# UZ-SLAMLab/DefSLAM

Measured on AMD Instinct MI355X. Metric: SfT GN iters/sec (500-node mesh, 1k matches), higher is better.
Workload: dtype f64

## Files before the change

### defslam_amd/_lib.py

```python
from __future__ import annotations

import ctypes as C
import os

_HERE = os.path.dirname(os.path.abspath(__file__))
LIB_PATH = os.path.join(_HERE, "lib", "libdefslam_hip.so")
LAB_LIB_PATH = os.path.join(_HERE, "lib", "libdefslam_hip_lab.so")

DSH_OK = 0
DSH_TRACE_STRIDE = 8
DSH_MAX_ITERS = 64

c_double_p = C.POINTER(C.c_double)
c_float_p = C.POINTER(C.c_float)
c_i32_p = C.POINTER(C.c_int32)
c_u8_p = C.POINTER(C.c_uint8)


class SftFrameC(C.Structure):
    _fields_ = [
        ("Tcw", c_float_p),
        ("K", C.c_double * 4),
        ("n_frame", C.c_int32),
        ("M", C.c_int32),
        ("obs_nodes", c_i32_p),
        ("obs_bary", c_double_p),
        ("obs_uv", c_double_p),
        ("obs_invsig2", c_double_p),
        ("xyz", c_double_p),
        ("reg_lap", C.c_double),
        ("reg_inex", C.c_double),
        ("reg_temp", C.c_double),
        ("neighbour_layers", C.c_int32),
        ("max_iters", C.c_int32),
    ]


class SftResultC(C.Structure):
    _fields_ = [
        ("Tcw", c_float_p),
        ("pose7", c_double_p),
        ("xyz", c_double_p),
        ("chi2_obs", c_double_p),
        ("outlier", c_u8_p),
        ("mappoint_xyz", c_float_p),
        ("rep_error", C.c_double),
        ("inliers", C.c_int32),
        ("iters", C.c_int32),
        ("trials", C.c_int32),
        ("dim", C.c_int32),
        ("half_bandwidth", C.c_int32),
        ("status", C.c_int32),
        ("trace", c_double_p),
    ]


class SchwarpProblemC(C.Structure):
    pass


class BbsC(C.Structure):
    _fields_ = [("umin", C.c_double), ("umax", C.c_double), ("nptsu", C.c_int32), ("vmin", C.c_double), ("vmax", C.c_double),
                ("nptsv", C.c_int32), ("valdim", C.c_int32)]


SchwarpProblemC._fields_ = [("bbs", BbsC), ("P", C.c_int32), ("kp1", C.c_void_p), ("kp2", C.c_void_p), ("invsig", C.c_void_p), ("fx_slot", C.c_double),
                            ("fy_slot", C.c_double), ("lam", C.c_double), ("fx", C.c_float), ("fy", C.c_float), ("max_iters", C.c_int32), ("x", C.c_void_p),
                            ("diff", C.c_void_p), ("drop", C.c_void_p), ("info", C.c_int32 * 2), ("costs", C.c_double * 2), ("init_lambda", C.c_double), ("init_ok", C.c_int32)]



class SchwarpStoreC(C.Structure):
    _fields_ = [("point_id", C.c_void_p), ("idx2", C.c_void_p), ("tag", C.c_int32)]


class TrackFrameC(C.Structure):
    _fields_ = [("Tcw", c_float_p), ("Ow", C.c_float * 3), ("K", C.c_float * 4), ("bounds", C.c_float * 4), ("grid_cols", C.c_int32),
                ("grid_rows", C.c_int32), ("levels", C.c_int32), ("scale_factors", c_float_p), ("log_scale_factor", C.c_float), ("N", C.c_int32),
                ("kp", c_float_p), ("octave", c_i32_p), ("desc", c_u8_p), ("state", c_u8_p)]


class TrackProblemC(C.Structure):
    _fields_ = [("frame", TrackFrameC), ("mode", C.c_int32), ("th", C.c_float), ("Q", C.c_int32), ("xyz", c_float_p), ("octave", c_i32_p),
                ("normal", c_float_p), ("max_distance", c_float_p), ("desc", c_u8_p), ("skip", c_u8_p), ("match", c_i32_p), ("in_view", c_u8_p),
                ("level", c_i32_p), ("uv", c_float_p), ("view_cos", c_float_p), ("nmatches", C.c_int32), ("rescans", C.c_int32)]


DSH_TRACK_FRAME = 0
DSH_TRACK_LOCAL = 1


class MpKeyFrameC(C.Structure):
    _fields_ = [("Ow", C.c_float * 3), ("N", C.c_int32), ("desc", c_u8_p), ("octave", c_i32_p), ("levels", C.c_int32),
                ("scale_factors", c_float_p), ("bad", C.c_int32)]


DSH_MP_DESCRIPTOR = 1
DSH_MP_NORMAL_DEPTH = 2
DSH_MP_NO_OBS = 1
DSH_MP_NO_GOOD_DESC = 2
DSH_MP_MAX_OBS = 65535


class MpdbDescC(C.Structure):
    _fields_ = [("ctx", C.c_void_p), ("point_capacity", C.c_int32), ("keyframe_capacity", C.c_int32), ("observation_capacity", C.c_int64)]


DSH_MPDB_POSITION = 1
DSH_MPDB_NORMAL_DEPTH = 2
DSH_MPDB_DESCRIPTOR = 4


class TrackCloseCountsC(C.Structure):
    _fields_ = [(n, C.c_int32) for n in ("matches_inliers", "matches_outliers", "to_match_local", "observed", "inliers", "outliers",
                                         "local_map_points", "n_moved")]


DIFFPROP_FIELDS = ["I1u", "I1v", "I2u", "I2v", "J12a", "J12b", "J12c", "J12d", "J21a", "J21b", "J21c", "J21d",
                   "H12uux", "H12uuy", "H12uvx", "H12uvy", "H12vvx", "H12vvy"]


EXPORTED_SYMBOLS = [
    "dsh_create", "dsh_destroy", "dsh_last_error", "dsh_stream", "dsh_synchronize",
    "dsh_template_build", "dsh_template_set", "dsh_template_dims", "dsh_template_get", "dsh_template_embed",
    "dsh_sft_solve", "dsh_sft_batch_upload", "dsh_sft_batch_run", "dsh_sft_batch_download",
    "dsh_sft_batch_counts", "dsh_sft_batch_problem_info",
    "dsh_bbs_eval", "dsh_bbs_coloc", "dsh_normals_estimate", "dsh_schwarp_eval", "dsh_schwarp_fit", "dsh_schwarp_fit_batch",
    "dsh_sfn_estimate", "dsh_bbs_bending", "dsh_warp_initialize", "dsh_search_by_schwarp",
    "dsh_template_embed_device", "dsh_scale_min_median", "dsh_optimize_horn", "dsh_surface_register",
    "dsh_comm_unique_id", "dsh_comm_create", "dsh_comm_destroy", "dsh_sft_shared_solve", "dsh_sft_shared_solve_group", "dsh_sft_connected_solve", "dsh_sft_connected_solve_group",
    "dsh_diffdb_create", "dsh_diffdb_destroy", "dsh_diffdb_clear", "dsh_diffdb_count", "dsh_diffdb_append", "dsh_schwarp_fit_batch_store",
    "dsh_normals_estimate_db", "dsh_sfn_estimate_db",
    "dsh_search_by_projection_batch", "dsh_search_by_projection_frame", "dsh_search_by_projection_local",
    "dsh_kfdb_create", "dsh_kfdb_destroy", "dsh_kfdb_clear", "dsh_kfdb_add", "dsh_kfdb_set_bad", "dsh_kfdb_count", "dsh_mappoint_update",
    "dsh_mpdb_create", "dsh_mpdb_destroy", "dsh_mpdb_clear", "dsh_mpdb_point_count", "dsh_mpdb_keyframe_count", "dsh_mpdb_add_points",
    "dsh_mpdb_update_points", "dsh_mpdb_set_points_bad", "dsh_mpdb_add_observations", "dsh_mpdb_erase_observations", "dsh_mpdb_add_keyframe",
    "dsh_mpdb_set_keyframe_point", "dsh_mpdb_set_keyframe_parent", "dsh_mpdb_set_keyframe_bad",
    "dsh_local_map_update", "dsh_local_map_points", "dsh_local_map_search",
    "dsh_trackstate_set_embedding", "dsh_trackstate_clear_embedding", "dsh_trackstate_set_counters", "dsh_trackstate_get",
    "dsh_trackstate_seed_local_points", "dsh_trackstate_repose", "dsh_trackstate_cull", "dsh_track_close_frame",
]
DSH_COMM_ID_BYTES = 128

LAB_SYMBOLS = ["dsh_lab_set_option", "dsh_lab_sft_run_timed", "dsh_lab_sft_assemble_timed", "dsh_lab_sft_phase_ms", "dsh_lab_sft_step_trace",
               "dsh_lab_sft_system", "dsh_lab_sft_solver_info", "dsh_lab_sft_wave_check", "dsh_lab_sft_dump", "dsh_lab_sft_rounds_timed",
               "dsh_lab_sft_factor_check"]

_lib = None
_lab = None


def load() -> C.CDLL:
    global _lib
    if _lib is None:
        _lib = _bind(LIB_PATH, lab=False)
    return _lib


def load_lab() -> C.CDLL:
    global _lab
    if _lab is None:
        _lab = _bind(LAB_LIB_PATH, lab=True)
    return _lab


def _bind(path: str, lab: bool) -> C.CDLL:
    if not os.path.exists(path):
        raise OSError(f"{path} is missing: run `python -c 'import __graft_entry__ as g; g.build()'` "
                      f"(or `make -C defslam_amd/csrc`). There is no CPU fallback.")
    L = C.CDLL(path)
    vp = C.c_void_p
    L.dsh_create.argtypes = [C.POINTER(vp), C.c_int]
    L.dsh_destroy.argtypes = [vp]
    L.dsh_last_error.argtypes = [vp]
    L.dsh_last_error.restype = C.c_char_p
    L.dsh_stream.argtypes = [vp]
    L.dsh_stream.restype = vp
    L.dsh_synchronize.argtypes = [vp]
    L.dsh_template_build.argtypes = [vp, C.c_int, c_double_p, C.c_int, c_i32_p]
    L.dsh_template_set.argtypes = [vp, C.c_int, c_double_p, c_u8_p, c_i32_p, c_i32_p, c_double_p, c_double_p, C.c_int, c_i32_p,
                                   c_double_p, C.c_double]
    L.dsh_template_dims.argtypes = [vp, c_i32_p, c_i32_p, c_i32_p]
    L.dsh_template_get.argtypes = [vp, c_u8_p, c_i32_p, c_i32_p, c_double_p, c_double_p, c_i32_p, c_double_p, c_double_p]
    L.dsh_template_embed.argtypes = [vp, C.c_int, c_float_p, c_i32_p, c_i32_p, c_float_p]
    L.dsh_sft_solve.argtypes = [vp, C.POINTER(SftFrameC), C.POINTER(SftResultC)]
    L.dsh_sft_batch_upload.argtypes = [vp, C.c_int, C.POINTER(SftFrameC)]
    L.dsh_sft_batch_run.argtypes = [vp]
    L.dsh_sft_batch_download.argtypes = [vp, C.c_int, C.POINTER(SftResultC)]
    L.dsh_sft_batch_counts.argtypes = [vp, C.POINTER(C.c_int64), C.POINTER(C.c_int64)]
    L.dsh_sft_batch_problem_info.argtypes = [vp, C.c_int, C.POINTER(C.c_int64), c_i32_p]
    L.dsh_bbs_eval.argtypes = [vp, C.POINTER(BbsC), c_double_p, c_double_p, c_double_p, C.c_int, C.c_int, C.c_int, c_double_p, c_u8_p]
    L.dsh_bbs_coloc.argtypes = [vp, C.POINTER(BbsC), c_double_p, c_double_p, C.c_int, C.c_int, C.c_int, c_i32_p, c_double_p, c_i32_p]
    L.dsh_normals_estimate.argtypes = [vp, C.c_int, c_i32_p, c_float_p, c_u8_p, c_float_p, c_u8_p, c_float_p, c_u8_p, c_float_p,
                                       c_double_p, c_double_p, c_i32_p, c_float_p, c_float_p, c_u8_p, c_i32_p]
    L.dsh_schwarp_eval.argtypes = [vp, C.POINTER(BbsC), C.c_int, c_float_p, c_float_p, c_float_p, C.c_double, C.c_double, C.c_double, c_double_p,
                                   c_double_p, c_double_p]
    L.dsh_schwarp_fit.argtypes = [vp, C.POINTER(BbsC), C.c_int, c_float_p, c_float_p, c_float_p, C.c_double, C.c_double, C.c_double, C.c_float,
                                  C.c_float, C.c_int, c_double_p, c_float_p, c_u8_p, c_i32_p, c_double_p]
    L.dsh_schwarp_fit_batch.argtypes = [vp, C.c_int, C.POINTER(SchwarpProblemC)]
    L.dsh_diffdb_create.argtypes = [vp, C.c_int64, C.POINTER(vp)]
    L.dsh_diffdb_destroy.argtypes = [vp]
    L.dsh_diffdb_clear.argtypes = [vp]
    L.dsh_diffdb_count.argtypes = [vp]
    L.dsh_diffdb_count.restype = C.c_int64
    L.dsh_diffdb_append.argtypes = [vp, C.c_int, c_float_p, c_i32_p, c_i32_p, c_i32_p]
    L.dsh_schwarp_fit_batch_store.argtypes = [vp, C.c_int, C.POINTER(SchwarpProblemC), C.POINTER(SchwarpStoreC), vp]
    L.dsh_normals_estimate_db.argtypes = [vp, vp, C.c_int, c_i32_p, c_float_p, c_u8_p, c_float_p, c_double_p, c_double_p, c_i32_p, c_float_p, c_i32_p,
                                          C.c_int32, c_i32_p, c_i32_p, c_i32_p, c_i32_p, c_float_p, c_u8_p]
    L.dsh_sfn_estimate.argtypes = [vp, C.POINTER(BbsC), C.c_int, c_double_p, c_double_p, c_float_p, C.c_double, C.c_double, C.c_int, c_double_p, c_double_p,
                                   c_double_p, c_double_p, c_float_p, c_i32_p]
    L.dsh_sfn_estimate_db.argtypes = [vp, C.POINTER(BbsC), vp, C.c_int, c_i32_p, c_double_p, c_double_p, C.c_double, C.c_double, C.c_int, c_double_p, c_double_p,
                                      c_double_p, c_double_p, c_float_p, c_i32_p]
    L.dsh_bbs_bending.argtypes = [C.POINTER(BbsC), C.c_double, c_double_p]
    L.dsh_search_by_schwarp.argtypes = [vp, C.POINTER(BbsC), c_double_p, C.c_int, c_float_p, c_u8_p, c_float_p, c_float_p, C.c_int, C.c_int, C.c_int, c_float_p,
                                        c_u8_p, c_u8_p, C.c_float, C.c_int, c_i32_p, c_i32_p]
    L.dsh_warp_initialize.argtypes = [vp, C.POINTER(BbsC), C.c_int, c_float_p, c_float_p, C.c_double, c_double_p, c_i32_p]
    c_i64_p = C.POINTER(C.c_int64)
    L.dsh_template_embed_device.argtypes = [vp, C.c_int, c_float_p, c_i32_p, c_i32_p, c_float_p]
    L.dsh_scale_min_median.argtypes = [vp, C.c_int, c_float_p, c_float_p, c_double_p, C.c_int64, c_float_p, c_i64_p, c_i32_p]
    L.dsh_optimize_horn.argtypes = [vp, C.c_int, c_float_p, c_float_p, c_double_p, C.c_double, C.c_double, c_i32_p, c_double_p]
    L.dsh_surface_register.argtypes = [vp, C.c_int, c_float_p, c_float_p, c_double_p, C.c_int64, c_float_p, C.c_double, C.c_int, c_i32_p, c_double_p,
                                       c_double_p, c_float_p, c_double_p]
    L.dsh_comm_unique_id.argtypes = [vp]
    L.dsh_comm_create.argtypes = [vp, C.c_int, C.c_int, vp, C.POINTER(vp)]
    L.dsh_comm_destroy.argtypes = [vp]
    L.dsh_sft_shared_solve.argtypes = [vp, vp, C.POINTER(SftFrameC), C.POINTER(SftResultC)]
    L.dsh_sft_shared_solve_group.argtypes = [C.c_int, C.POINTER(vp), C.POINTER(SftFrameC), C.POINTER(SftResultC)]
    L.dsh_sft_connected_solve.argtypes = [vp, vp, C.POINTER(SftFrameC), C.POINTER(SftResultC)]
    L.dsh_sft_connected_solve_group.argtypes = [vp, vp, C.POINTER(SftFrameC), C.POINTER(SftResultC)]
    L.dsh_search_by_projection_batch.argtypes = [vp, C.c_int, C.POINTER(TrackProblemC)]
    L.dsh_search_by_projection_frame.argtypes = [vp, C.POINTER(TrackFrameC), C.c_int, c_float_p, c_i32_p, c_u8_p, C.c_float, c_i32_p, c_i32_p]
    L.dsh_search_by_projection_local.argtypes = [vp, C.POINTER(TrackFrameC), C.c_int, c_float_p, c_float_p, c_float_p, c_u8_p, c_u8_p, C.c_float,
                                                 c_i32_p, c_u8_p, c_i32_p, c_i32_p]
    L.dsh_kfdb_create.argtypes = [vp, C.c_int32, C.POINTER(vp)]
    L.dsh_kfdb_destroy.argtypes = [vp]
    L.dsh_kfdb_clear.argtypes = [vp]
    L.dsh_kfdb_add.argtypes = [vp, C.POINTER(MpKeyFrameC), c_i32_p]
    L.dsh_kfdb_set_bad.argtypes = [vp, C.c_int32, C.c_int32]
    L.dsh_kfdb_count.argtypes = [vp]
    L.dsh_mappoint_update.argtypes = [vp, vp, C.c_int, c_float_p, c_i32_p, c_i32_p, c_i32_p, c_i32_p, C.c_int32, c_u8_p, c_i32_p, c_float_p,
                                      c_float_p, c_float_p, c_i32_p]
    i32 = C.c_int32
    L.dsh_mpdb_create.argtypes = [C.POINTER(MpdbDescC), C.POINTER(vp)]
    L.dsh_mpdb_destroy.argtypes = [vp]
    L.dsh_mpdb_clear.argtypes = [vp]
    L.dsh_mpdb_point_count.argtypes = [vp]
    L.dsh_mpdb_keyframe_count.argtypes = [vp]
    L.dsh_mpdb_add_points.argtypes = [vp, C.c_int, c_float_p, c_float_p, c_float_p, c_u8_p, c_u8_p, c_i32_p]
    L.dsh_mpdb_update_points.argtypes = [vp, C.c_int, c_i32_p, i32, c_float_p, c_float_p, c_float_p, c_u8_p]
    L.dsh_mpdb_set_points_bad.argtypes = [vp, C.c_int, c_i32_p, c_u8_p]
    L.dsh_mpdb_add_observations.argtypes = [vp, C.c_int, c_i32_p, c_i32_p]
    L.dsh_mpdb_erase_observations.argtypes = [vp, C.c_int, c_i32_p, c_i32_p]
    L.dsh_mpdb_add_keyframe.argtypes = [vp, i32, c_i32_p, i32, i32, c_i32_p]
    L.dsh_mpdb_set_keyframe_point.argtypes = [vp, i32, i32, i32]
    L.dsh_mpdb_set_keyframe_parent.argtypes = [vp, i32, i32]
    L.dsh_mpdb_set_keyframe_bad.argtypes = [vp, i32, i32]
    L.dsh_local_map_update.argtypes = [vp, C.c_int, c_i32_p, c_u8_p, i32, c_i32_p, c_i32_p, c_i32_p, c_i32_p, c_i32_p, c_i32_p]
    L.dsh_local_map_points.argtypes = [vp, i32, c_i32_p, c_i32_p]
    L.dsh_local_map_search.argtypes = [vp, C.POINTER(TrackFrameC), C.c_float, i32, c_i32_p, c_i32_p, c_u8_p, c_i32_p, c_float_p, c_float_p, c_i32_p]
    L.dsh_trackstate_set_embedding.argtypes = [vp, C.c_int, c_i32_p, c_i32_p, c_double_p]
    L.dsh_trackstate_clear_embedding.argtypes = [vp]
    L.dsh_trackstate_set_counters.argtypes = [vp, C.c_int, c_i32_p, c_i32_p, c_i32_p]
    L.dsh_trackstate_get.argtypes = [vp, C.c_int, c_i32_p, c_i32_p, c_i32_p, c_i32_p, c_float_p]
    L.dsh_trackstate_seed_local_points.argtypes = [vp, C.c_int, c_i32_p]
    L.dsh_trackstate_repose.argtypes = [vp, C.c_int, c_double_p, c_i32_p]
    L.dsh_trackstate_cull.argtypes = [vp, C.c_int, c_i32_p, c_i32_p, i32, c_u8_p]
    L.dsh_track_close_frame.argtypes = [vp, C.POINTER(TrackFrameC), C.c_int, c_i32_p, c_u8_p, C.c_int, c_double_p, i32, C.POINTER(TrackCloseCountsC)]
    for name in EXPORTED_SYMBOLS:
        fn = getattr(L, name)
        if name not in ("dsh_last_error", "dsh_stream"):
            fn.restype = C.c_int
    if lab:
        L.dsh_lab_set_option.argtypes = [vp, C.c_char_p, C.c_int]
        L.dsh_lab_sft_run_timed.argtypes = [vp, C.c_int, c_double_p]
        L.dsh_lab_sft_assemble_timed.argtypes = [vp, C.c_int, c_double_p]
        L.dsh_lab_sft_phase_ms.argtypes = [vp, C.c_int, c_double_p]
        L.dsh_lab_sft_step_trace.argtypes = [vp, C.c_int, c_double_p]
        L.dsh_lab_sft_system.argtypes = [vp, C.c_int, C.c_int32, c_double_p, c_double_p, c_double_p]
        L.dsh_lab_sft_solver_info.argtypes = [vp, C.c_int, c_i32_p]
        L.dsh_lab_sft_wave_check.argtypes = [vp, C.c_double, C.c_int, C.c_int, c_double_p, c_double_p, c_i32_p, c_double_p]
        L.dsh_lab_sft_dump.argtypes = [vp, C.c_int, C.c_int, C.c_int64, c_double_p]
        L.dsh_lab_sft_rounds_timed.argtypes = [vp, c_double_p, c_i32_p]
        L.dsh_lab_sft_factor_check.argtypes = [vp, c_double_p, c_u8_p, C.c_int, c_double_p, c_i32_p]
        for name in LAB_SYMBOLS:
            getattr(L, name).restype = C.c_int
    return L


class HipEvents:

    def __init__(self):
        self._hip = C.CDLL("libamdhip64.so")
        self._hip.hipEventCreate.argtypes = [C.POINTER(C.c_void_p)]
        self._hip.hipEventRecord.argtypes = [C.c_void_p, C.c_void_p]
        self._hip.hipEventSynchronize.argtypes = [C.c_void_p]
        self._hip.hipEventElapsedTime.argtypes = [C.POINTER(C.c_float), C.c_void_p, C.c_void_p]
        self._hip.hipEventDestroy.argtypes = [C.c_void_p]
        self.e0, self.e1 = C.c_void_p(), C.c_void_p()
        for e in (self.e0, self.e1):
            if self._hip.hipEventCreate(C.byref(e)) != 0:
                raise OSError("hipEventCreate failed")

    def start(self, stream: int):
        if self._hip.hipEventRecord(self.e0, C.c_void_p(stream)) != 0:
            raise OSError("hipEventRecord failed")

    def stop_ms(self, stream: int) -> float:
        ms = C.c_float()
        if (self._hip.hipEventRecord(self.e1, C.c_void_p(stream)) != 0 or self._hip.hipEventSynchronize(self.e1) != 0
                or self._hip.hipEventElapsedTime(C.byref(ms), self.e0, self.e1) != 0):
            raise OSError("HIP event timing failed")
        return float(ms.value)

    def close(self):
        for e in (self.e0, self.e1):
            if e:
                self._hip.hipEventDestroy(e)
        self.e0 = self.e1 = None


HIP_DEVICE_ATTRIBUTE_MULTIPROCESSOR_COUNT = 63


def device_cus(device: int = 0) -> int:
    hip = C.CDLL("libamdhip64.so")
    hip.hipDeviceGetAttribute.argtypes = [C.POINTER(C.c_int), C.c_int, C.c_int]
    n = C.c_int(0)
    if hip.hipDeviceGetAttribute(C.byref(n), HIP_DEVICE_ATTRIBUTE_MULTIPROCESSOR_COUNT, int(device)) != 0 or n.value <= 0:
        raise OSError("hipDeviceGetAttribute(hipDeviceAttributeMultiprocessorCount) failed")
    return int(n.value)
```

### defslam_amd/csrc/dsh_api.cpp

```cpp
#include <hip/hip_runtime.h>

#include <algorithm>
#include <cmath>
#include <cstdio>
#include <cstdlib>
#include <cstring>
#include <dlfcn.h>

#include <memory>
#include <mutex>
#include <string>
#include <vector>

#include "../../include/defslam_hip.h"
#include "dsh_ctx.h"
#include "dsh_template.h"
#include "sft_pack.h"
#include "sft_problem.h"

#include "mapping_launch.h"

#ifdef DSH_LAB
#include "../../include/defslam_hip_debug.h"
#endif

struct LdsMarks { size_t lm[2] = {0, 0}, sc = 0, spec[2] = {0, 0}, cn = 0, b[2] = {0, 0}, tail = 0; };
static LdsMarks g_lds_marks[64];
static std::mutex g_lds_mu;
#define LDS_MARKS(c) (g_lds_marks[(c)->device & 63])
#define LDS_LOCK() std::lock_guard<std::mutex> lds_lock__(g_lds_mu)

namespace {

constexpr int kNB = 32;
constexpr int kTS = 16, kBT = 8, kWB = 16;

using dsh::Tcw_from_pose7;

struct Packed {
  SftDev h{};
  dsh::SftGraph* g = nullptr;
  dsh::SftFramePack f;
};

}

struct dsh_ctx : dsh_ctx_base {
  dsh::TemplateHost tmpl;
  char* d_tmpl = nullptr;
  size_t d_tmpl_bytes = 0;
  struct {
    const double *xyz0, *nbr_w, *nbr_sumw, *k0;
    const int32_t *nbr_ptr, *nbr_idx;
  } dt{};
  std::vector<std::unique_ptr<dsh::SftGraph>> graphs;
  uint64_t upload_serial = 0;
  int B = 0;
  std::vector<Packed> packed;
  char* d_batch = nullptr;
  size_t d_batch_cap = 0;
  SftDev* d_probs = nullptr;
  std::vector<SftDev> h_probs;
  HostBuf stage;
  hipEvent_t stage_free = nullptr;
  bool stage_busy = false;
  HostBuf results;
  size_t ro_bytes = 0;
  size_t res_off = 0, res_bytes = 0;
  struct ResOffs { size_t xyz, chi2, trace, mp, outl; };
  std::vector<ResOffs> res_offs;
  int max_kd = 0;
  size_t jl_doubles = 0;
  size_t xyz_doubles = 0;
  int nw = 8;
  int spec_k = 1;
  int spec_nh = 0;
  char* d_sync = nullptr;
  size_t sync_bytes = 0;
  int spec_hint = 12;
  int max_iters_batch = 0;
  SftSpec* d_spec = nullptr;
  size_t spec_bytes = 0;
  HostBuf spec_done;
  SftSc* d_sc = nullptr;
  int force_waves = 0;
  bool force_split = false;
  bool rounds_mode = false;
  SftRun* d_runs = nullptr;
  int* d_counters = nullptr;
  int* d_linlist = nullptr;
  int rounds_hint = 24;
  static constexpr int kMaxSub = 4;
  hipStream_t sub_stream[kMaxSub] = {nullptr, nullptr, nullptr, nullptr};
  hipEvent_t sub_event[kMaxSub] = {nullptr, nullptr, nullptr, nullptr};
  int n_sub = 1;
  std::vector<hipEvent_t>* phase_events = nullptr;
  std::vector<int> phase_ids;
  int num_cus = 256;
  bool ran = false;
  struct { int waves = 0; int dataflow = 1; int wide_off = 0; int speculate = 0; int split = 2; int rounds = 1; int streams = 0; int helpers = -1; int tail = -1; int owner_waves = 8; int helpers_wbt = 12; } opt;
  bool any_split = false;
};

dsh_ctx_base* dsh_base(dsh_ctx* ctx) { return static_cast<dsh_ctx_base*>(ctx); }

namespace {

void drop_graphs(dsh_ctx* c) {
  if (!c->host_only && c->stream) (void)hipStreamSynchronize(c->stream);
  for (auto& g : c->graphs)
    if (g->d_base) (void)hipFree(g->d_base);
  c->graphs.clear();
  c->packed.clear();
}

int upload_template(dsh_ctx* c) {
  c->B = 0;
  c->ran = false;
  drop_graphs(c);
  if (c->host_only) return DSH_OK;
  const dsh::TemplateHost& t = c->tmpl;
  Arena a;
  const size_t o_xyz0 = a.take(sizeof(double) * 3 * t.n);
  const size_t o_ptr = a.take(sizeof(int32_t) * (t.n + 1));
  const size_t o_idx = a.take(sizeof(int32_t) * t.nbr_idx.size());
  const size_t o_w = a.take(sizeof(double) * t.nbr_w.size());
  const size_t o_sw = a.take(sizeof(double) * t.n);
  const size_t o_k0 = a.take(sizeof(double) * t.n);
  if (c->d_tmpl) { (void)hipFree(c->d_tmpl); c->d_tmpl = nullptr; }
  HIPCHK(c, hipMalloc((void**)&c->d_tmpl, a.size));
  c->d_tmpl_bytes = a.size;
  std::vector<char> st(a.size, 0);
  std::memcpy(&st[o_xyz0], t.xyz0.data(), sizeof(double) * 3 * t.n);
  std::memcpy(&st[o_ptr], t.nbr_ptr.data(), sizeof(int32_t) * (t.n + 1));
  std::memcpy(&st[o_idx], t.nbr_idx.data(), sizeof(int32_t) * t.nbr_idx.size());
  std::memcpy(&st[o_w], t.nbr_w.data(), sizeof(double) * t.nbr_w.size());
  std::memcpy(&st[o_sw], t.nbr_sumw.data(), sizeof(double) * t.n);
  std::memcpy(&st[o_k0], t.k0.data(), sizeof(double) * t.n);
  HIPCHK(c, hipMemcpy(c->d_tmpl, st.data(), a.size, hipMemcpyHostToDevice));
  c->dt.xyz0 = (const double*)(c->d_tmpl + o_xyz0);
  c->dt.nbr_ptr = (const int32_t*)(c->d_tmpl + o_ptr);
  c->dt.nbr_idx = (const int32_t*)(c->d_tmpl + o_idx);
  c->dt.nbr_w = (const double*)(c->d_tmpl + o_w);
  c->dt.nbr_sumw = (const double*)(c->d_tmpl + o_sw);
  c->dt.k0 = (const double*)(c->d_tmpl + o_k0);
  c->B = 0;
  c->ran = false;
  return DSH_OK;
}

template <class T>
size_t reserve(Arena& a, const std::vector<T>& v) { return a.take(sizeof(T) * v.size()); }
template <class T>
void put(char* st, size_t off, const std::vector<T>& v) {
  if (!v.empty()) std::memcpy(st + off, v.data(), sizeof(T) * v.size());
}

int graph_for(dsh_ctx* c, const std::vector<uint8_t>& opt, dsh::SftGraph** out, std::string& err) {
  uint64_t h = 1469598103934665603ull;
  for (uint8_t b : opt) { h ^= b; h *= 1099511628211ull; }
  for (auto& g : c->graphs)
    if (g->opt_hash == h && g->opt == opt) { g->last_use = c->upload_serial; *out = g.get(); return DSH_OK; }
  if (c->graphs.size() >= 64) {
    if (!c->host_only && c->stream) (void)hipStreamSynchronize(c->stream);
    auto& gs = c->graphs;
    for (size_t i = 0; i < gs.size();) {
      if (gs[i]->last_use != c->upload_serial) {
        if (gs[i]->d_base) (void)hipFree(gs[i]->d_base);
        gs.erase(gs.begin() + i);
      } else {
        i++;
      }
    }
  }
  std::unique_ptr<dsh::SftGraph> g(new dsh::SftGraph());
  const int rc = dsh::build_graph(c->tmpl, opt, *g, err);
  if (rc != DSH_OK) return rc;
  g->last_use = c->upload_serial;
  if (!c->host_only) {
    Arena a;
    auto& o = g->o;
    o.act = reserve(a, g->act); o.actnode = reserve(a, g->actnode); o.star_node = reserve(a, g->star_node); o.star_sL = reserve(a, g->star_sL);
    o.str_nodes = reserve(a, g->str_nodes); o.str_L0 = reserve(a, g->str_L0); o.off_ptr = reserve(a, g->off_ptr); o.off_rc = reserve(a, g->off_rc);
    o.sh_ptr = reserve(a, g->sh_ptr); o.sh_rec = reserve(a, g->sh_rec); o.sh_cf = reserve(a, g->sh_cf); o.tmask = reserve(a, g->tmask);
    o.hgather = reserve(a, g->hgather);
    o.hgatherT = reserve(a, g->hgatherT);
    std::vector<char> st(a.size, 0);
    put(st.data(), o.act, g->act); put(st.data(), o.actnode, g->actnode); put(st.data(), o.star_node, g->star_node); put(st.data(), o.star_sL, g->star_sL);
    put(st.data(), o.str_nodes, g->str_nodes); put(st.data(), o.str_L0, g->str_L0); put(st.data(), o.off_ptr, g->off_ptr); put(st.data(), o.off_rc, g->off_rc);
    put(st.data(), o.sh_ptr, g->sh_ptr); put(st.data(), o.sh_rec, g->sh_rec); put(st.data(), o.sh_cf, g->sh_cf); put(st.data(), o.tmask, g->tmask);
    put(st.data(), o.hgather, g->hgather);
    put(st.data(), o.hgatherT, g->hgatherT);
    if (hipMalloc((void**)&g->d_base, a.size) != hipSuccess) { err = "out of device memory (graph)"; return DSH_ERR_HIP; }
    g->d_bytes = a.size;
    if (hipMemcpy(g->d_base, st.data(), a.size, hipMemcpyHostToDevice) != hipSuccess) { (void)hipFree(g->d_base); err = "graph upload failed"; return DSH_ERR_HIP; }
  }
  *out = g.get();
  c->graphs.push_back(std::move(g));
  return DSH_OK;
}

int pack_problem(dsh_ctx* c, const dsh_sft_frame& f, bool wide_off, Packed& P, std::string& err) {
  const dsh::TemplateHost& t = c->tmpl;
  std::vector<uint8_t> viewed, opt;
  int rc = dsh::frame_active_set(t, f, viewed, opt, err);
  if (rc != DSH_OK) return rc;
  rc = graph_for(c, opt, &P.g, err);
  if (rc != DSH_OK) return rc;
  const dsh::SftGraph& g = *P.g;
  rc = dsh::pack_frame(t, g, f, viewed, P.f, err);
  if (rc != DSH_OK) return rc;
  SftDev& h = P.h;
  h = SftDev{};
  h.n = t.n; h.nA = g.nA; h.Dn = 3 * g.nA; h.kd = g.kd; h.ldh = h.kd + 1;
  h.tile_mode = (h.kd <= kTS * kBT) ? 1 : ((h.kd <= kTS * kWB && !wide_off) ? 2 : 0);
  h.wbt = h.tile_mode == 1 ? kBT : (h.tile_mode == 2 ? (h.kd + kTS - 1) / kTS : 0);
  h.tpr = h.tile_mode ? h.wbt + 1 : 0;
  h.M = f.M; h.V = P.f.V; h.S = g.S; h.Es = g.Es; h.noff = g.noff; h.max_iters = f.max_iters; h.mode = 0;
  h.fx = f.K[0]; h.fy = f.K[1]; h.cx = f.K[2]; h.cy = f.K[3];
  h.w_ref = f.reg_temp / std::pow(t.median_L, 2);
  h.w_curv = f.reg_lap / (double)g.nA;
  h.w_str = g.Es > 0 ? f.reg_inex / (double)g.Es : 0.0;
  const float deltaMono = (float)std::sqrt(5.991);
  h.hub_delta = (double)deltaMono;
  h.hub_dsqr = h.hub_delta * h.hub_delta;
  return DSH_OK;
}

int run_rounds_enqueue(dsh_ctx* c);
int run_rounds(dsh_ctx* c) {
  const int rc = run_rounds_enqueue(c);
  if (rc != DSH_OK)
    for (int s = 0; s < c->n_sub; s++) if (c->sub_stream[s]) (void)hipStreamSynchronize(c->sub_stream[s]);
  return rc;
}
int run_rounds_enqueue(dsh_ctx* c) {
  const int B = c->B, S = c->n_sub;
  int b0[dsh_ctx::kMaxSub + 1];
  for (int s = 0; s <= S; s++) b0[s] = (int)((long long)B * s / S);
  int tail_below = -1;
  if (S == 1 && c->opt.tail != 0) {
    if (c->opt.tail > 0) tail_below = c->opt.tail * c->num_cus;
    else tail_below = std::min(4 * c->num_cus, std::max(2 * c->num_cus, (int)((long long)3 * B / 4)));
  }
  auto launch = [&](int s, int phase) {
    const bool ev = c->phase_events && S == 1;
    if (ev) { hipEvent_t e; if (hipEventCreate(&e) == hipSuccess) { (void)hipEventRecord(e, c->stream); c->phase_events->push_back(e); c->phase_ids.push_back(phase); } }
    hipError_t r;
    {
      LDS_LOCK();
      if (phase == SFTB_PH_TAIL) r = sftb_tail_launch(c->d_probs + b0[s], c->d_runs + b0[s], c->d_counters + 16 * s, b0[s + 1] - b0[s], c->max_kd, c->jl_doubles, &LDS_MARKS(c).tail, c->num_cus, tail_below, c->sub_stream[s]);
      else r = sftb_launch(c->d_probs + b0[s], c->d_runs + b0[s], c->d_counters + 16 * s, c->d_linlist + b0[s], b0[s + 1] - b0[s], phase, c->jl_doubles, c->xyz_doubles, LDS_MARKS(c).b,
                           c->num_cus, tail_below, c->sub_stream[s]);
    }
    if (ev) { hipEvent_t e; if (hipEventCreate(&e) == hipSuccess) { (void)hipEventRecord(e, c->stream); c->phase_events->push_back(e); } }
    return r;
  };
  if (S > 1) {
    HIPCHK(c, hipEventRecord(c->sub_event[0], c->stream));
    for (int s = 1; s < S; s++) HIPCHK(c, hipStreamWaitEvent(c->sub_stream[s], c->sub_event[0], 0));
  }
  for (int s = 0; s < S; s++) HIPCHK(c, launch(s, SFTB_PH_INIT));
  const int worst = std::max(1, c->max_iters_batch) * 10 + 1;
  int rounds = 0, group = std::max(1, std::min(worst, c->rounds_hint));
  if (tail_below >= B) group = 0;
  HIPCHK(c, c->spec_done.ensure(64 * dsh_ctx::kMaxSub, true));
  int rc = DSH_OK;
  while (true) {
    for (int i = 0; i < group && rounds < worst; i++, rounds++)
      for (int s = 0; s < S; s++) {
        HIPCHK(c, launch(s, SFTB_PH_LIN));
        HIPCHK(c, launch(s, SFTB_PH_FACTOR));
        HIPCHK(c, launch(s, SFTB_PH_TRIAL));
      }
    if (tail_below >= 0) HIPCHK(c, launch(0, SFTB_PH_TAIL));
    for (int s = 0; s < S; s++) HIPCHK(c, hipMemcpyAsync(c->spec_done.p + 64 * s, c->d_counters + 16 * s, 8 * sizeof(int), hipMemcpyDeviceToHost, c->sub_stream[s]));
    for (int s = 0; s < S; s++) HIPCHK(c, hipStreamSynchronize(c->sub_stream[s]));
    int done = 0;
    for (int s = 0; s < S; s++) done += *reinterpret_cast<const int*>(c->spec_done.p + 64 * s);
    const int* c0 = reinterpret_cast<const int*>(c->spec_done.p);
    if (done >= B) { c->rounds_hint = (tail_below >= 0 && c0[6]) ? std::max(1, c0[7]) : rounds; break; }
    if (rounds >= worst) { rc = dsh_fail(c, DSH_ERR_STATE, "batched rounds: a problem did not terminate within its trial budget"); break; }
    group = 2;
  }
  return rc;
}

int run_once(dsh_ctx* c) {
  if (c->rounds_mode) return run_rounds(c);
  if (c->spec_k <= 1) {
    LDS_LOCK();
    HIPCHK(c, sft_lm_launch(c->d_probs, c->B, c->max_kd, c->jl_doubles, c->nw, LDS_MARKS(c).lm, c->stream));
    return DSH_OK;
  }
  const int K = c->spec_k, B = c->B;
  HIPCHK(c, hipMemsetAsync(c->d_spec, 0, c->spec_bytes, c->stream));
  const int rounds_per_iter = (10 + K - 1) / K;
  const int worst = c->max_iters_batch * rounds_per_iter;
  auto launch = [&](int phase) { LDS_LOCK(); return sft_spec_launch(c->d_probs, c->d_spec, B, K, phase, c->spec_nh, c->opt.owner_waves, c->max_kd, c->jl_doubles, LDS_MARKS(c).spec, c->stream); };
  if (c->spec_nh > 0) HIPCHK(c, hipMemsetAsync(c->d_sync, 0, c->sync_bytes, c->stream));
  HIPCHK(c, launch(SFT_SPEC_INIT));
  int rounds = 0, group = std::max(2, std::min(worst, c->spec_hint));
  HIPCHK(c, c->spec_done.ensure(sizeof(SftSpec) * (size_t)B, true));
  while (true) {
    for (int i = 0; i < group && rounds < worst; i++, rounds++) {
      HIPCHK(c, launch(SFT_SPEC_LIN));
      if (c->any_split) {
        HIPCHK(c, launch(SFT_SPEC_FACTOR));
        HIPCHK(c, launch(SFT_SPEC_SOLVE));
      }
      HIPCHK(c, launch(SFT_SPEC_TRIAL));
    }
    HIPCHK(c, launch(SFT_SPEC_LIN));
    HIPCHK(c, hipMemcpyAsync(c->spec_done.p, c->d_spec, sizeof(SftSpec) * (size_t)B, hipMemcpyDeviceToHost, c->stream));
    HIPCHK(c, hipStreamSynchronize(c->stream));
    const SftSpec* sp = reinterpret_cast<const SftSpec*>(c->spec_done.p);
    bool all_done = true;
    int needed = 0;
    for (int b = 0; b < B; b++) { all_done = all_done && sp[b].done; needed = std::max(needed, sp[b].launches); }
    if (all_done) { c->spec_hint = needed; break; }
    if (rounds >= worst) return dsh_fail(c, DSH_ERR_STATE, "speculative trials: a problem did not terminate within its launch budget");
    group = 2;
  }
  return DSH_OK;
}

}

extern "C" {

int dsh_create(dsh_ctx** out, int device) {
  if (!out) return DSH_ERR_ARG;
  *out = nullptr;
  if (device == -1) {
    dsh_ctx* hc = new dsh_ctx();
    hc->device = -1;
    hc->host_only = true;
    *out = hc;
    return DSH_OK;
  }
  int count = 0;
  if (hipGetDeviceCount(&count) != hipSuccess || count <= 0) return DSH_ERR_NO_DEVICE;
  if (device < 0 || device >= count) return DSH_ERR_ARG;
  dsh_ctx* c = new dsh_ctx();
  c->device = device;
  if (hipSetDevice(device) != hipSuccess || hipStreamCreateWithFlags(&c->stream, hipStreamNonBlocking) != hipSuccess) {
    delete c;
    return DSH_ERR_HIP;
  }
  if (hipEventCreateWithFlags(&c->stage_free, hipEventDisableTiming) != hipSuccess) {
    (void)hipStreamDestroy(c->stream);
    delete c;
    return DSH_ERR_HIP;
  }
  int cus = 0;
  if (hipDeviceGetAttribute(&cus, hipDeviceAttributeMultiprocessorCount, device) == hipSuccess && cus > 0) c->num_cus = cus;
  c->sub_stream[0] = c->stream;
  if (hipEventCreateWithFlags(&c->sub_event[0], hipEventDisableTiming) != hipSuccess) c->sub_event[0] = nullptr;
  *out = c;
  return DSH_OK;
}

int dsh_destroy(dsh_ctx* c) {
  if (!c) return DSH_ERR_ARG;
  dsh_detach_stores(c);
  if (c->host_only) { c->stage.release(); c->results.release(); delete c; return DSH_OK; }
  (void)hipSetDevice(c->device);
  drop_graphs(c);
  for (int i = 1; i < dsh_ctx::kMaxSub; i++) if (c->sub_stream[i]) { (void)hipStreamSynchronize(c->sub_stream[i]); (void)hipStreamDestroy(c->sub_stream[i]); }
  for (int i = 0; i < dsh_ctx::kMaxSub; i++) if (c->sub_event[i]) (void)hipEventDestroy(c->sub_event[i]);
  if (c->stream) { (void)hipStreamSynchronize(c->stream); (void)hipStreamDestroy(c->stream); }
  if (c->stage_free) (void)hipEventDestroy(c->stage_free);
  c->stage.release();
  c->results.release();
  c->spec_done.release();
  if (c->d_tmpl) (void)hipFree(c->d_tmpl);
  c->scratch.release();
  c->pin_in.release();
  c->pin_out.release();
  if (c->d_batch) (void)hipFree(c->d_batch);
  if (c->d_sc) (void)hipFree(c->d_sc);
  delete c;
  return DSH_OK;
}

const char* dsh_last_error(const dsh_ctx* c) { return c ? c->err.c_str() : "null context"; }
void* dsh_stream(dsh_ctx* c) { return c ? (void*)c->stream : nullptr; }
int dsh_synchronize(dsh_ctx* c) {
  if (const int rc = dsh_enter(c, "dsh_synchronize")) return rc;
  HIPCHK(c, hipStreamSynchronize(c->stream));
  return DSH_OK;
}

int dsh_template_build(dsh_ctx* c, int n, const double* xyz0, int F, const int32_t* facets) {
  if (!c || n <= 0 || F <= 0 || !xyz0 || !facets) return dsh_fail(c, DSH_ERR_ARG, "dsh_template_build: bad argument");
  for (int i = 0; i < 3 * F; i++)
    if (facets[i] < 0 || facets[i] >= n) return dsh_fail(c, DSH_ERR_ARG, "dsh_template_build: facet index out of range");
  if (!c->host_only) (void)hipSetDevice(c->device);
  c->tmpl.build(n, xyz0, F, facets);
  return upload_template(c);
}

int dsh_template_set(dsh_ctx* c, int n, const double* xyz0, const uint8_t* boundary, const int32_t* rp, const int32_t* col, const double* w,
                     const double* k0, int E, const int32_t* en, const double* eL, double median_L) {
  if (!c || n <= 0 || E < 0 || !xyz0 || !boundary || !rp || !col || !w || !k0 || !en || !eL) return dsh_fail(c, DSH_ERR_ARG, "dsh_template_set: bad argument");
  if (rp[0] != 0) return dsh_fail(c, DSH_ERR_ARG, "dsh_template_set: nbr_rowptr[0] != 0");
  for (int i = 0; i < n; i++)
    if (rp[i + 1] < rp[i]) return dsh_fail(c, DSH_ERR_ARG, "dsh_template_set: nbr_rowptr is not non-decreasing");
  for (int p = 0; p < rp[n]; p++)
    if (col[p] < 0 || col[p] >= n) return dsh_fail(c, DSH_ERR_ARG, "dsh_template_set: neighbour index out of range");
  for (int e = 0; e < E; e++) {
    if (en[2 * e] < 0 || en[2 * e] >= n || en[2 * e + 1] < 0 || en[2 * e + 1] >= n) return dsh_fail(c, DSH_ERR_ARG, "dsh_template_set: edge node out of range");
    if (!(eL[e] > 0.0)) return dsh_fail(c, DSH_ERR_ARG, "dsh_template_set: edge rest length must be positive");
  }
  if (!(median_L > 0.0)) return dsh_fail(c, DSH_ERR_ARG, "dsh_template_set: median edge length must be positive");
  if (!c->host_only) (void)hipSetDevice(c->device);
  c->tmpl.set(n, xyz0, boundary, rp, col, w, k0, E, en, eL, median_L);
  return upload_template(c);
}

int dsh_template_dims(const dsh_ctx* c, int32_t* n, int32_t* E, int32_t* nnz) {
  if (!c || !c->tmpl.valid) return DSH_ERR_STATE;
  if (n) *n = c->tmpl.n;
  if (E) *E = c->tmpl.E;
  if (nnz) *nnz = (int32_t)c->tmpl.nbr_idx.size();
  return DSH_OK;
}

int dsh_template_get(const dsh_ctx* c, uint8_t* boundary, int32_t* rp, int32_t* col, double* w, double* k0, int32_t* en, double* eL, double* med) {
  if (!c || !c->tmpl.valid) return DSH_ERR_STATE;
  const dsh::TemplateHost& t = c->tmpl;
  if (boundary) std::memcpy(boundary, t.boundary.data(), t.n);
  if (rp) std::memcpy(rp, t.nbr_ptr.data(), sizeof(int32_t) * (t.n + 1));
  if (col) std::memcpy(col, t.nbr_idx.data(), sizeof(int32_t) * t.nbr_idx.size());
  if (w) std::memcpy(w, t.nbr_w.data(), sizeof(double) * t.nbr_w.size());
  if (k0) std::memcpy(k0, t.k0.data(), sizeof(double) * t.n);
  if (en) std::memcpy(en, t.edge_nodes.data(), sizeof(int32_t) * 2 * t.E);
  if (eL) std::memcpy(eL, t.edge_L0.data(), sizeof(double) * t.E);
  if (med) *med = t.median_L;
  return DSH_OK;
}

int dsh_template_embed(const dsh_ctx* c, int P, const float* pts, int32_t* facet_id, int32_t* nodes, float* bary) {
  if (!c || !c->tmpl.valid || c->tmpl.F <= 0) return DSH_ERR_STATE;
  if (P < 0 || !pts || !facet_id || !nodes || !bary) return DSH_ERR_ARG;
  c->tmpl.embed(P, pts, facet_id, nodes, bary);
  return DSH_OK;
}

int dsh_template_embed_device(dsh_ctx* c, int P, const float* pts, int32_t* facet_id, int32_t* nodes, float* bary) {
  if (!c) return DSH_ERR_ARG;
  if (!c->tmpl.valid || c->tmpl.F <= 0) return dsh_fail(c, DSH_ERR_STATE, "dsh_template_embed_device: needs a template built from facets");
  if (P < 0 || (P > 0 && (!pts || !facet_id || !nodes || !bary))) return dsh_fail(c, DSH_ERR_ARG, "dsh_template_embed_device: bad argument");
  if (c->host_only) return dsh_fail(c, DSH_ERR_NO_DEVICE, "dsh_template_embed_device: host-only context, no GPU (dsh_template_embed is the host routine)");
  if (P == 0) return DSH_OK;
  if (const int rc = dsh_enter(c, "dsh_template_embed_device")) return rc;
  const dsh::TemplateHost& t = c->tmpl;
  hipStream_t st = c->stream;
  struct Item { const void* src; size_t bytes; void* dev; };
  Item in[5] = {{pts, 12 * (size_t)P, nullptr}, {t.xyz0.data(), 24 * (size_t)t.n, nullptr}, {t.facets.data(), 12 * (size_t)t.F, nullptr},
                {t.nf_ptr.data(), 4 * (size_t)(t.n + 1), nullptr}, {t.nf_idx.data(), 4 * t.nf_idx.size(), nullptr}};
  for (Item& it : in) {
    if (c->scratch.take(it.bytes, &it.dev) != hipSuccess) return dsh_fail(c, DSH_ERR_HIP, "dsh_template_embed_device: out of device memory");
    if (it.bytes && hipMemcpyAsync(it.dev, it.src, it.bytes, hipMemcpyHostToDevice, st) != hipSuccess)
      return dsh_fail(c, DSH_ERR_HIP, "dsh_template_embed_device: upload failed");
  }
  void *d_fid = nullptr, *d_nodes = nullptr, *d_bary = nullptr;
  if (c->scratch.take(4 * (size_t)P, &d_fid) != hipSuccess || c->scratch.take(12 * (size_t)P, &d_nodes) != hipSuccess ||
      c->scratch.take(12 * (size_t)P, &d_bary) != hipSuccess)
    return dsh_fail(c, DSH_ERR_HIP, "dsh_template_embed_device: out of device memory");
  hipError_t e = reg_embed(P, static_cast<const float*>(in[0].dev), t.n, static_cast<const double*>(in[1].dev), static_cast<const int32_t*>(in[2].dev),
                           static_cast<const int32_t*>(in[3].dev), static_cast<const int32_t*>(in[4].dev), static_cast<int32_t*>(d_fid),
                           static_cast<int32_t*>(d_nodes), static_cast<float*>(d_bary), st);
  if (e == hipSuccess) e = hipMemcpyAsync(facet_id, d_fid, 4 * (size_t)P, hipMemcpyDeviceToHost, st);
  if (e == hipSuccess) e = hipMemcpyAsync(nodes, d_nodes, 12 * (size_t)P, hipMemcpyDeviceToHost, st);
  if (e == hipSuccess) e = hipMemcpyAsync(bary, d_bary, 12 * (size_t)P, hipMemcpyDeviceToHost, st);
  if (e == hipSuccess) e = hipStreamSynchronize(st);
  if (e != hipSuccess) return dsh_fail(c, DSH_ERR_HIP, std::string("dsh_template_embed_device: ") + hipGetErrorString(e));
  return DSH_OK;
}

int dsh_sft_batch_upload(dsh_ctx* c, int B, const dsh_sft_frame* frames) {
  if (!c || B <= 0 || !frames) return dsh_fail(c, DSH_ERR_ARG, "dsh_sft_batch_upload: bad argument");
  if (!c->tmpl.valid) return dsh_fail(c, DSH_ERR_STATE, "dsh_sft_batch_upload: no template");
  if (!c->host_only) (void)hipSetDevice(c->device);
  c->B = 0;
  c->ran = false;
  c->upload_serial++;
  if ((int)c->packed.size() != B) c->packed.resize(B);
  for (int b = 0; b < B; b++) {
    std::string e;
    const int rc = pack_problem(c, frames[b], c->opt.wide_off != 0, c->packed[b], e);
    if (rc != DSH_OK) return dsh_fail(c, rc, "problem " + std::to_string(b) + ": " + e);
  }
  int nw = 8;
  {
    bool all_tiles = true;
    for (int b = 0; b < B; b++) all_tiles = all_tiles && c->packed[b].h.tile_mode == 1;
    if (all_tiles && 2 * B > c->num_cus) nw = 4;
    if ((c->opt.waves == 4 && all_tiles) || c->opt.waves == 8) nw = c->opt.waves;
    if (c->force_waves == 8) nw = 8;
    c->rounds_mode = all_tiles && nw == 4 && c->opt.waves == 0 && c->opt.rounds != 0 && !c->host_only;
    c->n_sub = 1;
    if (c->rounds_mode) {
      const int want = c->opt.streams > 0 ? c->opt.streams : 1;
      while (c->n_sub < want && c->n_sub < dsh_ctx::kMaxSub && B / (c->n_sub + 1) >= 16 * c->num_cus) c->n_sub++;
      if (c->opt.streams > 0) c->n_sub = std::min(std::min(c->opt.streams, (int)dsh_ctx::kMaxSub), std::max(1, B / 64));
      for (int i = 1; i < c->n_sub; i++)
        if (!c->sub_stream[i] && hipStreamCreateWithFlags(&c->sub_stream[i], hipStreamNonBlocking) != hipSuccess) c->sub_stream[i] = nullptr;
      for (int i = 0; i < c->n_sub; i++) if (!c->sub_stream[i] || !c->sub_event[0]) c->n_sub = 1;
    }
  }
  int K = 1;
  if (nw == 8 && !c->force_waves && !c->host_only) {
    K = (4 * B <= c->num_cus) ? 4 : ((3 * B <= c->num_cus) ? 3 : ((2 * B <= c->num_cus) ? 2 : 1));
    {
      bool wide = c->opt.split != 0 && c->opt.helpers != 0;
      for (int b = 0; b < B; b++) {
        const SftDev& hh = c->packed[b].h;
        const int sT = (hh.kd + kTS - 1) / kTS, sp = kTS * sT;
        const int c0 = ((hh.Dn - sp) / 2 / kTS) * kTS, n1 = hh.Dn - sp - c0;
        wide = wide && hh.tile_mode == 2 && sT >= c->opt.helpers_wbt && sT >= 2 && c0 >= 4 * kTS && n1 >= 4 * kTS;
      }
      if (wide && K == 4 && (long long)B * 4 * 2 * 3 > c->num_cus && (long long)B * 2 * 2 * 3 <= c->num_cus) K = 2;
    }
    if (c->opt.speculate >= 1 && c->opt.speculate <= SFT_SPEC_MAXK) K = c->opt.speculate;
    for (int b = 0; b < B; b++) if (c->packed[b].f.max_iters < 1) K = 1;
  }
  size_t jl_doubles = 0, xyz_doubles = 0;
  int max_kd = 0;
  const size_t lds_budget = ((((nw == 4 && !c->rounds_mode) || SFT_WAVES_PER_EU >= 4) ? 75 : 155) * 1024) / 8;
  for (int b = 0; b < B; b++) {
    SftDev& hh = c->packed[b].h;
    if ((c->force_split && hh.tile_mode == 1) ||
        (K > 1 && hh.tile_mode == 1 && c->opt.split >= 2 && 20 * B <= c->num_cus && hh.kd > kTS && hh.Dn >= 8 * kTS * ((hh.kd + kTS - 1) / kTS))) {
      hh.tile_mode = 2;
      hh.wbt = (hh.kd + kTS - 1) / kTS;
      hh.tpr = hh.wbt + 1;
    }
    hh.mode = (hh.mode & ~2) | ((hh.tile_mode == 1 && c->opt.dataflow) ? 2 : 0);
    hh.split = 0;
    if ((c->force_split || (K > 1 && c->opt.split)) && hh.tile_mode == 2) {
      const int sT = hh.wbt, sp = kTS * sT;
      const int c0 = ((hh.Dn - sp) / 2 / kTS) * kTS, n1 = hh.Dn - sp - c0;
      if (sT >= 2 && c0 >= 4 * kTS && n1 >= 4 * kTS) {
        const int n1p = ((n1 + kTS - 1) / kTS) * kTS;
        hh.split = 1; hh.sp_c0 = c0; hh.sp_s = sp; hh.sp_n1p = n1p; hh.sp_pad = n1p - n1;
        SftPart& p0 = hh.part[0]; SftPart& p1 = hh.part[1]; SftPart& p2 = hh.part[2];
        p0 = SftPart{}; p1 = SftPart{}; p2 = SftPart{};
        p0.nS = c0 / kTS; p0.nT = p0.nS + sT; p0.tpr = hh.tpr; p0.wbt = hh.wbt; p0.b_base = 0; p0.b_sign = 1; p0.b_lo = 0; p0.b_hi = c0 + sp;
        p1.nS = n1p / kTS; p1.nT = p1.nS + sT; p1.tpr = hh.tpr; p1.wbt = hh.wbt; p1.b_base = hh.Dn - 1 + hh.sp_pad; p1.b_sign = -1; p1.b_lo = hh.sp_pad; p1.b_hi = n1p;
        p2.nS = sT; p2.nT = sT; p2.wbt = sT - 1; p2.tpr = sT;
        hh.sp_xl = sT * p2.tpr * kTS * kTS + 8 * kTS * sT + 64;
        hh.part[3] = p2;
      }
    }
    size_t used = 0;
    const size_t need1 = ((3 * (size_t)hh.n + 1) & ~(size_t)1) + (((size_t)hh.M + 1) & ~(size_t)1) + 4 * (size_t)hh.S, need2 = need1 + 6 * (size_t)hh.nA + 4 * (size_t)hh.Es;
    const size_t need3 = need2 + 5 * (size_t)hh.M;
    hh.lds_class = (c->rounds_mode && used + need3 <= lds_budget) ? 3 : (used + need2 <= lds_budget) ? 2 : ((used + need1 <= lds_budget) ? 1 : 0);
    used += hh.lds_class == 3 ? need3 : hh.lds_class == 2 ? need2 : (hh.lds_class == 1 ? need1 : 0);
    jl_doubles = std::max(jl_doubles, used);
    if (hh.lds_class >= 1) xyz_doubles = std::max(xyz_doubles, ((3 * (size_t)hh.n + 1) & ~(size_t)1));
    max_kd = std::max(max_kd, hh.tile_mode == 2 ? std::max(hh.kd, kTS * kBT + 1) : hh.kd);
  }
  if (c->host_only) {
    c->h_probs.resize(B);
    for (int b = 0; b < B; b++) c->h_probs[b] = c->packed[b].h;
    c->B = B;
    c->nw = nw;
    return DSH_OK;
  }
  Arena a;
  const size_t o_tab = a.take(sizeof(SftDev) * B * K);
  struct Offs { size_t obs_nodes, obs_bary, obs_uv, obs_w, ob_ptr, ob_m, ob_c, viewed, xyz_init, pose_init; };
  std::vector<Offs> ro(B);
  for (int b = 0; b < B; b++) {
    dsh::SftFramePack& F = c->packed[b].f;
    Offs& o = ro[b];
    o.obs_nodes = reserve(a, F.obs_nodes); o.obs_bary = reserve(a, F.obs_bary); o.obs_uv = reserve(a, F.obs_uv); o.obs_w = reserve(a, F.obs_w);
    o.ob_ptr = reserve(a, F.ob_ptr); o.ob_m = reserve(a, F.ob_m); o.ob_c = reserve(a, F.ob_c); o.viewed = reserve(a, F.viewed);
    o.xyz_init = reserve(a, F.xyz_init);
    o.pose_init = a.take(8 * 8);
  }
  c->ro_bytes = a.size;
  c->res_off = a.size;
  (void)a.take(sizeof(SftResHdr) * (size_t)B);
  c->res_offs.resize(B);
  for (int b = 0; b < B; b++) {
    const SftDev& h = c->packed[b].h;
    dsh_ctx::ResOffs& r = c->res_offs[b];
    r.xyz = a.take(8 * 3 * (size_t)h.n) - c->res_off; r.chi2 = a.take(8 * (size_t)h.M) - c->res_off;
    r.trace = a.take(8 * DSH_TRACE_STRIDE * DSH_MAX_ITERS) - c->res_off;
    r.mp = a.take(4 * 3 * (size_t)h.M) - c->res_off; r.outl = a.take((size_t)h.M) - c->res_off;
  }
  c->res_bytes = a.size - c->res_off;
  struct POffs { size_t Hb, Lb, Lt, LbT, Lbord, Linv, x, xchg, Pf, PfB, sync; };
  struct WOffs { size_t bak, camrec, wtv, Anode, Jstar, Jstr, Hc, Hb, Hbord, Hcn, Lb, Lbord, Lc, Linv, Lt, LbT, x, dbg, sx0, sx1, shadow_xyz, shadow_chi2, shadow_hdr; POffs part[4]; };
  std::vector<WOffs> wo((size_t)B * K);
  const size_t ws_off = a.size;
  const size_t o_spec = a.take(sizeof(SftSpec) * (size_t)B * K);
  const size_t o_runs = a.take(c->rounds_mode ? sizeof(SftRun) * (size_t)B + 64 * dsh_ctx::kMaxSub + sizeof(int) * (size_t)B : 0);
  int nh = 0;
  {
    bool any = false;
    for (int b = 0; b < B; b++) any = any || (c->packed[b].h.split != 0 && c->packed[b].h.wbt >= c->opt.helpers_wbt);
    for (int b = 0; b < B; b++)
      if (c->packed[b].h.split && std::max(c->packed[b].h.part[0].nT, c->packed[b].h.part[1].nT) >= 60000) any = false;
    if (any && K > 1 && !c->force_split) {
      while (nh < 3 && (long long)B * K * 2 * (2 + nh) <= c->num_cus) nh++;
      if (nh == 1) nh = 0;
      if (c->opt.helpers >= 0) nh = c->opt.helpers;
    }
  }
  size_t sync_total = 0;
  if (nh > 0)
    for (int e = 0; e < B * K; e++) {
      const SftDev& h = c->packed[e % B].h;
      if (h.split) for (int g = 0; g < 2; g++) sync_total += Arena::round((size_t)4 * (16 + h.part[g].nT));
    }
  const size_t o_sync = a.take(sync_total);
  size_t sync_used = 0;
  for (int e = 0; e < B * K; e++) {
    const int b = e % B, lane = e / B;
    const SftDev& h = c->packed[b].h;
    const size_t Dnp = (size_t)((h.Dn + kNB - 1) / kNB) * kNB;
    WOffs& w = wo[e];
    w.sx0 = a.take(K > 1 ? 8 * 3 * (size_t)h.n : 0); w.sx1 = a.take(K > 1 ? 8 * 3 * (size_t)h.n : 0);
    w.shadow_xyz = a.take(lane ? 8 * 3 * (size_t)h.n : 0); w.shadow_chi2 = a.take(lane ? 8 * (size_t)h.M : 0); w.shadow_hdr = a.take(lane ? sizeof(SftResHdr) : 0);
    w.bak = a.take(8 * 3 * (size_t)h.n);
    w.camrec = a.take(8 * (size_t)h.M * SFT_CAM_STRIDE);
    w.wtv = a.take(h.lds_class >= 1 ? 0 : 8 * ((size_t)h.M + 1)); w.Jstar = a.take(h.lds_class >= 1 ? 0 : 8 * 4 * (size_t)h.S);
    w.Anode = a.take(h.lds_class >= 2 ? 0 : 8 * 6 * (size_t)h.nA); w.Jstr = a.take(h.lds_class >= 2 ? 0 : 8 * 4 * (size_t)h.Es);
    const size_t band_elems = h.tile_mode ? (Dnp / kTS + SFT_H_PAD_TILE_ROWS) * (size_t)h.tpr * kTS * kTS : Dnp * (size_t)h.ldh;
    const size_t bord_elems = (SFT_BORDER + 1) * Dnp + SFT_H_PAD_BORDER;
    w.Hc = a.take(h.tile_mode == 1 ? 8 * c->packed[b].g->hc_elems() : 0);
    w.Hb = a.take(h.tile_mode == 1 ? 0 : 8 * band_elems); w.Hbord = a.take(8 * bord_elems); w.Hcn = a.take(8 * 56);
    w.Lb = a.take(8 * band_elems); w.Lbord = a.take(8 * bord_elems); w.Lc = a.take(8 * 56);
    w.Linv = a.take(8 * (Dnp / kTS) * (size_t)kTS * kTS);
    w.Lt = a.take(h.tile_mode == 2 ? 8 * band_elems : 0); w.LbT = a.take(h.tile_mode == 2 ? 8 * (Dnp / kTS) * (size_t)kTS * kTS : 0);
    w.x = a.take(8 * (Dnp + 8)); w.dbg = a.take(1024);
    if (h.split)
      for (int g = 0; g < 4; g++) {
        const SftPart& q = h.part[g];
        const size_t tiles = 8 * (size_t)q.nT * q.tpr * kTS * kTS, col = 8 * (size_t)q.nT * kTS * kTS;
        POffs& po = w.part[g];
        po.Hb = a.take(g < 2 && lane == 0 ? tiles : 0);
        po.Lb = a.take(tiles); po.Lt = a.take(tiles); po.LbT = a.take(col); po.Linv = a.take(col);
        po.Lbord = a.take(8 * 8 * (size_t)kTS * q.nT); po.x = a.take(8 * ((size_t)kTS * q.nT + 8)); po.xchg = a.take(8 * (size_t)h.sp_xl);
        const bool helped = nh > 0 && g < 2;
        po.Pf = a.take(helped ? tiles : 0); po.PfB = a.take(helped ? col : 0);
        po.sync = o_sync + sync_used;
        if (helped) sync_used += Arena::round((size_t)4 * (16 + q.nT));
      }
  }
  if (sft_lm_kernel_lds_bytes(max_kd, jl_doubles) > 160 * 1024 || max_kd + kNB + SFT_BORDER > SFT_NT)
    return dsh_fail(c, DSH_ERR_ARG, "half-bandwidth too large for the LDS panel / workgroup");
  bool fresh_arena = false;
  if (a.size > c->d_batch_cap) {
    HIPCHK(c, hipStreamSynchronize(c->stream));
    if (c->d_batch) { (void)hipFree(c->d_batch); c->d_batch = nullptr; c->d_batch_cap = 0; }
    HIPCHK(c, hipMalloc((void**)&c->d_batch, a.size));
    c->d_batch_cap = a.size;
    fresh_arena = true;
  }
  if (c->stage_busy) { HIPCHK(c, hipEventSynchronize(c->stage_free)); c->stage_busy = false; }
  HIPCHK(c, c->stage.ensure(c->ro_bytes, true));
  char* st = c->stage.p;
  char* base = c->d_batch;
  c->h_probs.resize((size_t)B * K);
  SftResHdr* d_hdr = (SftResHdr*)(base + c->res_off);
  int max_iters = 0;
  for (int e = 0; e < B * K; e++) {
    const int b = e % B, lane = e / B;
    Packed& P = c->packed[b];
    const dsh::SftFramePack& F = P.f;
    const dsh::SftGraph& g = *P.g;
    const Offs& o = ro[b];
    if (lane == 0) {
      put(st, o.obs_nodes, F.obs_nodes); put(st, o.obs_bary, F.obs_bary); put(st, o.obs_uv, F.obs_uv); put(st, o.obs_w, F.obs_w);
      put(st, o.ob_ptr, F.ob_ptr); put(st, o.ob_m, F.ob_m); put(st, o.ob_c, F.ob_c); put(st, o.viewed, F.viewed); put(st, o.xyz_init, F.xyz_init);
      std::memcpy(st + o.pose_init, F.pose_init, 7 * sizeof(double));
    }
    SftDev h = P.h;
    const WOffs& w = wo[e];
    const dsh_ctx::ResOffs& r = c->res_offs[b];
    max_iters = std::max(max_iters, F.max_iters);
    char* rbase = base + c->res_off;
    const char* gb = g.d_base;
    h.xyz0 = c->dt.xyz0; h.nbr_ptr = c->dt.nbr_ptr; h.nbr_idx = c->dt.nbr_idx; h.nbr_w = c->dt.nbr_w; h.nbr_sumw = c->dt.nbr_sumw; h.k0 = c->dt.k0;
    h.act = (const int32_t*)(gb + g.o.act); h.actnode = (const int32_t*)(gb + g.o.actnode); h.star_node = (const int32_t*)(gb + g.o.star_node);
    h.star_sL = (const double*)(gb + g.o.star_sL); h.str_nodes = (const int32_t*)(gb + g.o.str_nodes); h.str_L0 = (const double*)(gb + g.o.str_L0);
    h.off_ptr = (const int32_t*)(gb + g.o.off_ptr); h.off_rc = (const int32_t*)(gb + g.o.off_rc); h.sh_ptr = (const int32_t*)(gb + g.o.sh_ptr);
    h.sh_rec = (const uint32_t*)(gb + g.o.sh_rec); h.sh_cf = (const double*)(gb + g.o.sh_cf); h.tmask = (const int32_t*)(gb + g.o.tmask);
    h.hgather = (const uint32_t*)(gb + g.o.hgather);
    h.hgatherT = (const uint32_t*)(gb + g.o.hgatherT);
    h.obs_nodes = (const int32_t*)(base + o.obs_nodes); h.obs_bary = (const double*)(base + o.obs_bary);
    h.obs_uv = (const double*)(base + o.obs_uv); h.obs_w = (const double*)(base + o.obs_w);
    h.ob_ptr = (const int32_t*)(base + o.ob_ptr); h.ob_m = (const int32_t*)(base + o.ob_m); h.ob_c = (const double*)(base + o.ob_c);
    h.viewed = (const uint8_t*)(base + o.viewed);
    h.xyz_init = (const double*)(base + o.xyz_init); h.pose_init = (const double*)(base + o.pose_init);
    h.res = d_hdr + b; h.pose = d_hdr[b].pose;
    h.xyz = (double*)(rbase + r.xyz); h.chi2_obs = (double*)(rbase + r.chi2); h.trace = (double*)(rbase + r.trace);
    h.mappoint = (float*)(rbase + r.mp); h.outlier = (uint8_t*)(rbase + r.outl);
    h.xyz_bak = (double*)(base + w.bak);
    h.camrec = (double*)(base + w.camrec); h.wtv = (double*)(base + w.wtv); h.Anode = (double*)(base + w.Anode);
    h.Jstar = (double*)(base + w.Jstar); h.Jstr = (double*)(base + w.Jstr);
    h.Hc = (double*)(base + w.Hc); h.Hb = (double*)(base + w.Hb); h.Hbord = (double*)(base + w.Hbord); h.Hcorner = (double*)(base + w.Hcn);
    h.Lb = (double*)(base + w.Lb); h.Lbord = (double*)(base + w.Lbord); h.Lcorner = (double*)(base + w.Lc); h.Linv = (double*)(base + w.Linv);
    h.Lt = (double*)(base + w.Lt); h.LbT = (double*)(base + w.LbT);
    h.x = (double*)(base + w.x); h.dbg = (double*)(base + w.dbg);
    h.spec_xyz[0] = (double*)(base + w.sx0); h.spec_xyz[1] = (double*)(base + w.sx1);
    if (h.split)
      for (int g = 0; g < 4; g++) {
        const POffs& po = w.part[g];
        SftPart& q = h.part[g];
        q.Hb = g < 2 ? (double*)(base + (lane ? wo[b].part[g].Hb : po.Hb)) : (double*)(base + po.xchg);
        q.Lb = (double*)(base + po.Lb); q.Lt = (double*)(base + po.Lt); q.LbT = (double*)(base + po.LbT); q.Linv = (double*)(base + po.Linv);
        q.Lbord = (double*)(base + po.Lbord); q.x = (double*)(base + po.x); q.xchg = (double*)(base + po.xchg);
        const bool helped = nh > 0 && g < 2;
        q.Pf = helped ? (double*)(base + po.Pf) : nullptr; q.PfB = helped ? (double*)(base + po.PfB) : nullptr;
        q.sync = helped ? (int32_t*)(base + po.sync) : nullptr;
      }
    if (lane) {
      h.xyz = (double*)(base + w.shadow_xyz); h.chi2_obs = (double*)(base + w.shadow_chi2);
      h.res = (SftResHdr*)(base + w.shadow_hdr); h.pose = ((SftResHdr*)(base + w.shadow_hdr))->pose;
      h.trace = nullptr; h.mappoint = nullptr; h.outlier = nullptr;
      if (h.tile_mode == 1 || h.split) {
        const SftDev& h0 = c->h_probs[b];
        h.Hc = h0.Hc; h.Hbord = h0.Hbord; h.Hcorner = h0.Hcorner;
      }
    }
    c->h_probs[e] = h;
  }
  std::memcpy(st + o_tab, c->h_probs.data(), sizeof(SftDev) * B * K);
  HIPCHK(c, hipMemcpyAsync(base, st, c->ro_bytes, hipMemcpyHostToDevice, c->stream));
  HIPCHK(c, hipEventRecord(c->stage_free, c->stream));
  c->stage_busy = true;
  if (fresh_arena) HIPCHK(c, hipMemsetAsync(base + ws_off, 0, a.size - ws_off, c->stream));
  HIPCHK(c, hipMemsetAsync(base + c->res_off, 0, c->res_bytes, c->stream));
  c->d_probs = (SftDev*)(base + o_tab);
  c->d_spec = (SftSpec*)(base + o_spec);
  c->d_runs = (SftRun*)(base + o_runs);
  c->d_counters = (int*)(base + o_runs + sizeof(SftRun) * (size_t)B);
  c->d_linlist = c->d_counters + 16 * dsh_ctx::kMaxSub;
  c->spec_bytes = sizeof(SftSpec) * (size_t)B * K;
  c->spec_k = K;
  c->spec_nh = nh;
  c->d_sync = base + o_sync;
  c->sync_bytes = sync_total;
  c->any_split = false;
  for (int b = 0; b < B; b++) c->any_split = c->any_split || c->packed[b].h.split != 0;
  c->max_iters_batch = max_iters;
  c->B = B;
  c->max_kd = max_kd;
  c->jl_doubles = jl_doubles;
  c->xyz_doubles = xyz_doubles;
  c->nw = nw;
  return DSH_OK;
}

int dsh_sft_batch_run(dsh_ctx* c) {
  if (!c) return DSH_ERR_ARG;
  if (const int rc = dsh_enter(c, "dsh_sft_batch_run")) return rc;
  if (c->B <= 0) return dsh_fail(c, DSH_ERR_STATE, "dsh_sft_batch_run: nothing uploaded");
  const int rc = run_once(c);
  if (rc != DSH_OK) return rc;
  c->ran = true;
  return DSH_OK;
}

int dsh_sft_batch_counts(dsh_ctx* c, int64_t* iters, int64_t* trials) {
  if (!c || c->B <= 0 || !c->ran) return DSH_ERR_STATE;
  if (const int rc = dsh_enter(c, "dsh_sft_batch_counts")) return rc;
  const size_t bytes = sizeof(SftResHdr) * (size_t)c->B;
  HIPCHK(c, c->results.ensure(std::max(bytes, c->results.cap), true));
  HIPCHK(c, hipMemcpyAsync(c->results.p, c->d_batch + c->res_off, bytes, hipMemcpyDeviceToHost, c->stream));
  HIPCHK(c, hipStreamSynchronize(c->stream));
  const SftResHdr* hd = reinterpret_cast<const SftResHdr*>(c->results.p);
  int64_t it = 0, tr = 0;
  for (int b = 0; b < c->B; b++) { it += hd[b].iters; tr += hd[b].trials; }
  if (iters) *iters = it;
  if (trials) *trials = tr;
  return DSH_OK;
}

int dsh_sft_batch_problem_info(dsh_ctx* c, int b, int64_t* bytes, int32_t* counts) {
  if (!c || b < 0 || b >= c->B) return DSH_ERR_ARG;
  const Packed& P = c->packed[b];
  const SftDev& h = P.h;
  const int64_t M = h.M, n = h.n, C = P.g->n_curv_ref, E = h.Es, V = h.V;
  const int64_t reads = 60 * M + 24 * n + 88 + 92 * C + 16 * E + 28 * V;
  const int64_t writes = 8 * (30 * M + 21 * C + 6 * E + 9 * V) + 8 * (2 * M + C + E + 3 * V) + 8 * M;
  if (bytes) *bytes = reads + writes;
  if (counts) { counts[0] = h.M; counts[1] = h.nA; counts[2] = P.g->n_curv_ref; counts[3] = h.Es; counts[4] = h.V; counts[5] = 6 + h.Dn; counts[6] = h.kd; counts[7] = c->rounds_mode ? 1 : c->nw; counts[8] = P.g->noff; }
  return DSH_OK;
}

int dsh_sft_batch_download(dsh_ctx* c, int B, dsh_sft_result* res) {
  if (!c || !res || B != c->B) return dsh_fail(c, DSH_ERR_ARG, "dsh_sft_batch_download: bad argument");
  if (const int rc = dsh_enter(c, "dsh_sft_batch_download")) return rc;
  if (!c->ran) return dsh_fail(c, DSH_ERR_STATE, "dsh_sft_batch_download: no run");
  HIPCHK(c, c->results.ensure(c->res_bytes, true));
  HIPCHK(c, hipMemcpyAsync(c->results.p, c->d_batch + c->res_off, c->res_bytes, hipMemcpyDeviceToHost, c->stream));
  HIPCHK(c, hipStreamSynchronize(c->stream));
  const char* rb = c->results.p;
  const SftResHdr* hd = reinterpret_cast<const SftResHdr*>(rb);
  for (int b = 0; b < B; b++) {
    const SftDev& h = c->h_probs[b];
    const Packed& P = c->packed[b];
    const dsh_ctx::ResOffs& o = c->res_offs[b];
    dsh_sft_result& r = res[b];
    r.rep_error = hd[b].rep_error;
    r.inliers = hd[b].inliers;
    r.iters = hd[b].iters;
    r.trials = hd[b].trials;
    r.status = hd[b].status;
    r.dim = 6 + h.Dn;
    r.half_bandwidth = h.kd;
    if (r.chi2_obs) std::memcpy(r.chi2_obs, rb + o.chi2, 8 * (size_t)h.M);
    if (r.outlier) std::memcpy(r.outlier, rb + o.outl, (size_t)h.M);
    if (r.xyz) std::memcpy(r.xyz, rb + o.xyz, 8 * 3 * (size_t)h.n);
    if (r.pose7) std::memcpy(r.pose7, hd[b].pose, 8 * 7);
    if (r.Tcw) Tcw_from_pose7(hd[b].pose, r.Tcw);
    if (r.mappoint_xyz) std::memcpy(r.mappoint_xyz, rb + o.mp, 4 * 3 * (size_t)h.M);
    if (r.trace) {
      const size_t rows = (size_t)std::max(P.f.max_iters, 0), done = std::min(rows, (size_t)std::max(hd[b].iters, 0));
      std::memcpy(r.trace, rb + o.trace, 8 * DSH_TRACE_STRIDE * done);
      std::memset(r.trace + DSH_TRACE_STRIDE * done, 0, 8 * DSH_TRACE_STRIDE * (rows - done));
    }
  }
  return DSH_OK;
}

int dsh_sft_solve(dsh_ctx* c, const dsh_sft_frame* frame, dsh_sft_result* result) {
  if (!c || !frame || !result) return dsh_fail(c, DSH_ERR_ARG, "dsh_sft_solve: bad argument");
  int rc = dsh_sft_batch_upload(c, 1, frame);
  if (rc != DSH_OK) return rc;
  rc = dsh_sft_batch_run(c);
  if (rc != DSH_OK) return rc;
  return dsh_sft_batch_download(c, 1, result);
}

namespace {
struct RcclUniqueId { char internal[128]; };
struct Rccl {
  void* lib = nullptr;
  int (*GetUniqueId)(RcclUniqueId*) = nullptr;
  int (*CommInitRank)(void**, int, RcclUniqueId, int) = nullptr;
  int (*AllReduce)(const void*, void*, size_t, int, int, void*, hipStream_t) = nullptr;
  int (*CommDestroy)(void*) = nullptr;
  const char* (*GetErrorString)(int) = nullptr;
  bool load(std::string& err) {
    if (lib) return true;
    for (const char* name : {"librccl.so.1", "librccl.so", "/opt/rocm/lib/librccl.so.1"}) {
      lib = dlopen(name, RTLD_NOW | RTLD_GLOBAL);
      if (lib) break;
    }
    if (!lib) { err = std::string("RCCL not found: ") + dlerror(); return false; }
    GetUniqueId = reinterpret_cast<decltype(GetUniqueId)>(dlsym(lib, "ncclGetUniqueId"));
    CommInitRank = reinterpret_cast<decltype(CommInitRank)>(dlsym(lib, "ncclCommInitRank"));
    AllReduce = reinterpret_cast<decltype(AllReduce)>(dlsym(lib, "ncclAllReduce"));
    CommDestroy = reinterpret_cast<decltype(CommDestroy)>(dlsym(lib, "ncclCommDestroy"));
    GetErrorString = reinterpret_cast<decltype(GetErrorString)>(dlsym(lib, "ncclGetErrorString"));
    if (!GetUniqueId || !CommInitRank || !AllReduce || !CommDestroy) { err = "RCCL symbols missing"; lib = nullptr; return false; }
    return true;
  }
};
Rccl g_rccl;
constexpr int kNcclDouble = 8, kNcclSum = 0;
}

struct dsh_comm {
  int nranks = 1, rank = 0;
  void* comm = nullptr;
  dsh_ctx* ctx = nullptr;
};

namespace {

struct ScRank { dsh_ctx* c; };

struct ScReducer {
  dsh_comm* comm = nullptr;
  SftSc** d_ptrs = nullptr;
  int reduce(std::vector<ScRank>& R, std::string& err) {
    if (comm) {
      dsh_ctx* c = R[0].c;
      const int rc = g_rccl.AllReduce(c->d_sc->send, c->d_sc->recv, SFT_SC_XCHG, kNcclDouble, kNcclSum, comm->comm, c->stream);
      if (rc != 0) { err = std::string("ncclAllReduce: ") + (g_rccl.GetErrorString ? g_rccl.GetErrorString(rc) : "error"); return DSH_ERR_HIP; }
      return DSH_OK;
    }
    for (auto& r : R)
      if (hipStreamSynchronize(r.c->stream) != hipSuccess) { err = "stream synchronise failed"; return DSH_ERR_HIP; }
    if (sft_sc_local_reduce(d_ptrs, (int)R.size(), R[0].c->stream) != hipSuccess || hipStreamSynchronize(R[0].c->stream) != hipSuccess) { err = "local reduce failed"; return DSH_ERR_HIP; }
    return DSH_OK;
  }
};

int sc_phase(std::vector<ScRank>& R, int phase, std::string& err) {
  for (auto& r : R) {
    dsh_ctx* c = r.c;
    (void)hipSetDevice(c->device);
    LDS_LOCK();
    if (sft_sc_launch(c->d_probs, c->d_sc, 1, phase, c->max_kd, c->jl_doubles, &LDS_MARKS(c).sc, c->stream) != hipSuccess) { err = "phase kernel launch failed"; return DSH_ERR_HIP; }
  }
  return DSH_OK;
}

int sc_solve(std::vector<ScRank>& R, ScReducer& red, int rank0, int nranks, const dsh_sft_frame* frames, dsh_sft_result* results, std::string& err) {
  const int G = (int)R.size();
  if (nranks > SFT_SC_XCHG - 13) { err = "too many ranks for the exchange vector"; return DSH_ERR_ARG; }
  int local_rc = DSH_OK;
  std::string local_err;
  for (int g = 0; g < G; g++) {
    dsh_ctx* c = R[g].c;
    if (c->host_only) { err = "host-only context, no GPU (there is no CPU fallback)"; return DSH_ERR_NO_DEVICE; }
    (void)hipSetDevice(c->device);
    if (!c->d_sc && hipMalloc((void**)&c->d_sc, sizeof(SftSc)) != hipSuccess) { err = "out of device memory"; return DSH_ERR_HIP; }
    SftSc init{};
    init.rank = rank0 + g;
    init.nranks = nranks;
    int rc = frames[g].max_iters < 1 ? DSH_ERR_ARG : DSH_OK;
    if (rc != DSH_OK && local_rc == DSH_OK) { local_rc = rc; local_err = "max_iters must be >= 1"; }
    if (rc == DSH_OK) {
      c->force_waves = 8;
      rc = dsh_sft_batch_upload(c, 1, &frames[g]);
      c->force_waves = 0;
      if (rc != DSH_OK && local_rc == DSH_OK) { local_rc = rc; local_err = c->err; }
    }
    if (rc == DSH_OK && c->packed[0].h.tile_mode != 1) {
      rc = DSH_ERR_ARG;
      if (local_rc == DSH_OK) { local_rc = rc; local_err = "the shared-camera mode needs a template with half-bandwidth <= 128 (register-window solver); dsh_sft_connected_solve takes wider ones"; }
    }
    if (rc == DSH_OK) {
      init.send[0] = (double)c->packed[0].h.nA;
      init.send[1] = (double)c->packed[0].h.Es;
    }
    init.send[2] = rc == DSH_OK ? 0.0 : 1.0;
    if (hipMemcpyAsync(c->d_sc, &init, sizeof(SftSc), hipMemcpyHostToDevice, c->stream) != hipSuccess) { err = "state upload failed"; return DSH_ERR_HIP; }
  }
  int rc = red.reduce(R, err);
  if (rc != DSH_OK) return rc;
  {
    double tot3[3];
    dsh_ctx* c = R[0].c;
    if (hipMemcpyAsync(tot3, c->d_sc->recv, sizeof(tot3), hipMemcpyDeviceToHost, c->stream) != hipSuccess || hipStreamSynchronize(c->stream) != hipSuccess) { err = "read-back failed"; return DSH_ERR_HIP; }
    if (tot3[2] != 0.0) {
      if (local_rc != DSH_OK) { err = local_err; return local_rc; }
      err = "another rank failed to set its patch up";
      return DSH_ERR_STATE;
    }
  }
  for (int g = 0; g < G; g++) {
    dsh_ctx* c = R[g].c;
    double tot[2];
    if (hipMemcpyAsync(tot, c->d_sc->recv, sizeof(tot), hipMemcpyDeviceToHost, c->stream) != hipSuccess || hipStreamSynchronize(c->stream) != hipSuccess) { err = "read-back failed"; return DSH_ERR_HIP; }
    SftDev& h = c->h_probs[0];
    h.w_curv = frames[g].reg_lap / tot[0];
    h.w_str = tot[1] > 0 ? frames[g].reg_inex / tot[1] : 0.0;
    if (hipMemcpyAsync(c->d_probs, &h, sizeof(SftDev), hipMemcpyHostToDevice, c->stream) != hipSuccess || hipStreamSynchronize(c->stream) != hipSuccess) { err = "problem record upload failed"; return DSH_ERR_HIP; }
  }
  for (int guard = 0; guard < DSH_MAX_ITERS + 1; guard++) {
    if ((rc = sc_phase(R, SFT_SC_LIN, err)) != DSH_OK || (rc = red.reduce(R, err)) != DSH_OK) return rc;
    int again = 0, done = 0;
    do {
      if ((rc = sc_phase(R, SFT_SC_FAC, err)) != DSH_OK || (rc = red.reduce(R, err)) != DSH_OK) return rc;
      if ((rc = sc_phase(R, SFT_SC_SOL, err)) != DSH_OK || (rc = red.reduce(R, err)) != DSH_OK) return rc;
      if ((rc = sc_phase(R, SFT_SC_CTL, err)) != DSH_OK) return rc;
      int32_t flags[2];
      dsh_ctx* c = R[0].c;
      if (hipMemcpyAsync(flags, &c->d_sc->again, sizeof(flags), hipMemcpyDeviceToHost, c->stream) != hipSuccess || hipStreamSynchronize(c->stream) != hipSuccess) { err = "flag read-back failed"; return DSH_ERR_HIP; }
      again = flags[0];
      done = flags[1];
    } while (again);
    if (done) break;
  }
  for (int g = 0; g < G; g++) {
    R[g].c->ran = true;
    rc = dsh_sft_batch_download(R[g].c, 1, &results[g]);
    if (rc != DSH_OK) { err = R[g].c->err; return rc; }
  }
  return DSH_OK;
}

}

int dsh_comm_unique_id(void* id) {
  std::string err;
  if (!id || !g_rccl.load(err)) return DSH_ERR_HIP;
  return g_rccl.GetUniqueId(static_cast<RcclUniqueId*>(id)) == 0 ? DSH_OK : DSH_ERR_HIP;
}

int dsh_comm_create(dsh_ctx* c, int nranks, int rank, const void* id, dsh_comm** out) {
  if (!c || !out || !id || nranks < 1 || rank < 0 || rank >= nranks) return dsh_fail(c, DSH_ERR_ARG, "dsh_comm_create: bad argument");
  *out = nullptr;
  if (const int rc = dsh_enter(c, "dsh_comm_create")) return rc;
  std::string err;
  if (!g_rccl.load(err)) return dsh_fail(c, DSH_ERR_HIP, "dsh_comm_create: " + err);
  RcclUniqueId uid;
  std::memcpy(&uid, id, sizeof(uid));
  std::unique_ptr<dsh_comm> cm(new dsh_comm());
  cm->nranks = nranks; cm->rank = rank; cm->ctx = c;
  const int rc = g_rccl.CommInitRank(&cm->comm, nranks, uid, rank);
  if (rc != 0) return dsh_fail(c, DSH_ERR_HIP, std::string("ncclCommInitRank: ") + (g_rccl.GetErrorString ? g_rccl.GetErrorString(rc) : "error"));
  *out = cm.release();
  return DSH_OK;
}

int dsh_comm_destroy(dsh_comm* cm) {
  if (!cm) return DSH_ERR_ARG;
  if (cm->comm && g_rccl.CommDestroy) (void)g_rccl.CommDestroy(cm->comm);
  delete cm;
  return DSH_OK;
}

int dsh_sft_shared_solve(dsh_ctx* c, dsh_comm* cm, const dsh_sft_frame* frame, dsh_sft_result* result) {
  if (!c || !cm || !frame || !result || cm->ctx != c) return dsh_fail(c, DSH_ERR_ARG, "dsh_sft_shared_solve: bad argument");
  std::vector<ScRank> R{ScRank{c}};
  ScReducer red;
  red.comm = cm;
  std::string err;
  const int rc = sc_solve(R, red, cm->rank, cm->nranks, frame, result, err);
  return rc == DSH_OK ? rc : dsh_fail(c, rc, "dsh_sft_shared_solve: " + err);
}

int dsh_sft_shared_solve_group(int G, dsh_ctx* const* ctxs, const dsh_sft_frame* frames, dsh_sft_result* results) {
  if (G < 1 || !ctxs || !frames || !results) return DSH_ERR_ARG;
  for (int g = 0; g < G; g++)
    if (!ctxs[g]) return DSH_ERR_ARG;
  dsh_ctx* c0 = ctxs[0];
  std::vector<ScRank> R;
  for (int g = 0; g < G; g++) R.push_back(ScRank{ctxs[g]});
  for (int g = 0; g < G; g++) {
    if (ctxs[g]->host_only) return dsh_fail(c0, DSH_ERR_NO_DEVICE, "dsh_sft_shared_solve_group: host-only context, no GPU (there is no CPU fallback)");
    (void)hipSetDevice(ctxs[g]->device);
    if (!ctxs[g]->d_sc && hipMalloc((void**)&ctxs[g]->d_sc, sizeof(SftSc)) != hipSuccess) return dsh_fail(c0, DSH_ERR_HIP, "dsh_sft_shared_solve_group: out of device memory");
  }
  std::vector<SftSc*> ptrs;
  for (int g = 0; g < G; g++) ptrs.push_back(ctxs[g]->d_sc);
  ScReducer red;
  (void)hipSetDevice(c0->device);
  if (hipMalloc((void**)&red.d_ptrs, sizeof(SftSc*) * G) != hipSuccess) return dsh_fail(c0, DSH_ERR_HIP, "dsh_sft_shared_solve_group: out of device memory");
  int rc = DSH_OK;
  std::string err;
  if (hipMemcpy(red.d_ptrs, ptrs.data(), sizeof(SftSc*) * G, hipMemcpyHostToDevice) != hipSuccess) { rc = DSH_ERR_HIP; err = "pointer table upload failed"; }
  if (rc == DSH_OK) rc = sc_solve(R, red, 0, G, frames, results, err);
  (void)hipFree(red.d_ptrs);
  return rc == DSH_OK ? rc : dsh_fail(c0, rc, "dsh_sft_shared_solve_group: " + err);
}


namespace {

int cn_allreduce(std::vector<ScRank>& R, dsh_comm* comm, double* const* send, double* const* recv, int n, std::string& err) {
  if (comm) {
    dsh_ctx* c = R[0].c;
    const int rc = g_rccl.AllReduce(send[0], recv[0], (size_t)n, kNcclDouble, kNcclSum, comm->comm, c->stream);
    if (rc != 0) { err = std::string("ncclAllReduce: ") + (g_rccl.GetErrorString ? g_rccl.GetErrorString(rc) : "error"); return DSH_ERR_HIP; }
    return DSH_OK;
  }
  for (auto& r : R)
    if (hipStreamSynchronize(r.c->stream) != hipSuccess) { err = "stream synchronise failed"; return DSH_ERR_HIP; }
  if (sft_vec_sum2(send[0], send[1], recv[0], recv[1], n, R[0].c->stream) != hipSuccess || hipStreamSynchronize(R[0].c->stream) != hipSuccess) { err = "local reduce failed"; return DSH_ERR_HIP; }
  return DSH_OK;
}

int cn_phase(std::vector<ScRank>& R, int phase, std::string& err) {
  for (auto& r : R) {
    dsh_ctx* c = r.c;
    (void)hipSetDevice(c->device);
    LDS_LOCK();
    if (sft_cn_launch(c->d_probs, c->d_sc, phase, c->max_kd, c->jl_doubles, &LDS_MARKS(c).cn, c->stream) != hipSuccess) { err = "phase kernel launch failed"; return DSH_ERR_HIP; }
  }
  return DSH_OK;
}

int cn_solve(std::vector<ScRank>& R, dsh_comm* comm, int rank0, const dsh_sft_frame* frame, dsh_sft_result* results, std::string& err) {
  const int G = (int)R.size();
  int local_rc = DSH_OK;
  std::string local_err;
  for (int g = 0; g < G; g++) {
    dsh_ctx* c = R[g].c;
    if (c->host_only) { err = "host-only context, no GPU (there is no CPU fallback)"; return DSH_ERR_NO_DEVICE; }
    (void)hipSetDevice(c->device);
    if (!c->d_sc && hipMalloc((void**)&c->d_sc, sizeof(SftSc)) != hipSuccess) { err = "out of device memory"; return DSH_ERR_HIP; }
    int rc = frame->max_iters < 1 ? DSH_ERR_ARG : DSH_OK;
    if (rc != DSH_OK && local_rc == DSH_OK) { local_rc = rc; local_err = "max_iters must be >= 1"; }
    if (rc == DSH_OK) {
      c->force_waves = 8;
      c->force_split = true;
      rc = dsh_sft_batch_upload(c, 1, frame);
      c->force_waves = 0;
      c->force_split = false;
      if (rc != DSH_OK && local_rc == DSH_OK) { local_rc = rc; local_err = c->err; }
    }
    if (rc == DSH_OK && !c->packed[0].h.split) {
      rc = DSH_ERR_ARG;
      if (local_rc == DSH_OK) { local_rc = rc; local_err = "the connected-mesh mode needs a band of at most 256 that is long enough to cut (two parts of four tile columns next to a separator of one bandwidth)"; }
    }
    SftSc init{};
    init.rank = rank0 + g;
    init.nranks = 2;
    init.send[0] = rc == DSH_OK ? 0.0 : 1.0;
    if (hipMemcpyAsync(c->d_sc, &init, sizeof(SftSc), hipMemcpyHostToDevice, c->stream) != hipSuccess) { err = "state upload failed"; return DSH_ERR_HIP; }
  }
  {
    double* snd[2]; double* rcv[2];
    for (int g = 0; g < G; g++) { snd[g] = R[g].c->d_sc->send; rcv[g] = R[g].c->d_sc->recv; }
    int rc = cn_allreduce(R, comm, snd, rcv, 4, err);
    if (rc != DSH_OK) return rc;
    double bad = 0.0;
    dsh_ctx* c = R[0].c;
    if (hipMemcpyAsync(&bad, c->d_sc->recv, sizeof(bad), hipMemcpyDeviceToHost, c->stream) != hipSuccess || hipStreamSynchronize(c->stream) != hipSuccess) { err = "read-back failed"; return DSH_ERR_HIP; }
    if (bad != 0.0) {
      if (local_rc != DSH_OK) { err = local_err; return local_rc; }
      err = "the other rank failed to set the problem up";
      return DSH_ERR_STATE;
    }
  }
  int rc;
  double* xs[2]; double* xr[2]; double* vx[2];
  int xl = 0, nx = 0;
  for (int g = 0; g < G; g++) {
    const SftDev& h = R[g].c->h_probs[0];
    xs[g] = h.part[rank0 + g].xchg; xr[g] = h.part[2].xchg; vx[g] = h.x;
    xl = h.sp_xl;
    nx = ((h.Dn + kNB - 1) / kNB) * kNB + 6;
  }
  for (int guard = 0; guard < DSH_MAX_ITERS + 1; guard++) {
    if ((rc = cn_phase(R, SFT_CN_LIN, err)) != DSH_OK) return rc;
    int again = 0, done = 0;
    do {
      if ((rc = cn_phase(R, SFT_CN_FAC, err)) != DSH_OK || (rc = cn_allreduce(R, comm, xs, xr, xl, err)) != DSH_OK) return rc;
      if ((rc = cn_phase(R, SFT_CN_SOL, err)) != DSH_OK || (rc = cn_allreduce(R, comm, vx, vx, nx, err)) != DSH_OK) return rc;
      if ((rc = cn_phase(R, SFT_CN_CTL, err)) != DSH_OK) return rc;
      int32_t flags[2];
      dsh_ctx* c = R[0].c;
      if (hipMemcpyAsync(flags, &c->d_sc->again, sizeof(flags), hipMemcpyDeviceToHost, c->stream) != hipSuccess || hipStreamSynchronize(c->stream) != hipSuccess) { err = "flag read-back failed"; return DSH_ERR_HIP; }
      again = flags[0];
      done = flags[1];
    } while (again);
    if (done) break;
  }
  for (int g = 0; g < G; g++) {
    R[g].c->ran = true;
    rc = dsh_sft_batch_download(R[g].c, 1, &results[g]);
    if (rc != DSH_OK) { err = R[g].c->err; return rc; }
  }
  return DSH_OK;
}

}

int dsh_sft_connected_solve(dsh_ctx* c, dsh_comm* cm, const dsh_sft_frame* frame, dsh_sft_result* result) {
  if (!c || !cm || !frame || !result || cm->ctx != c) return dsh_fail(c, DSH_ERR_ARG, "dsh_sft_connected_solve: bad argument");
  if (cm->nranks != 2) return dsh_fail(c, DSH_ERR_ARG, "dsh_sft_connected_solve: the cut has two parts: the communicator must have exactly two ranks");
  std::vector<ScRank> R{ScRank{c}};
  std::string err;
  const int rc = cn_solve(R, cm, cm->rank, frame, result, err);
  return rc == DSH_OK ? rc : dsh_fail(c, rc, "dsh_sft_connected_solve: " + err);
}

int dsh_sft_connected_solve_group(dsh_ctx* c0, dsh_ctx* c1, const dsh_sft_frame* frame, dsh_sft_result* results) {
  if (!c0 || !c1 || c0 == c1 || !frame || !results) return DSH_ERR_ARG;
  std::vector<ScRank> R{ScRank{c0}, ScRank{c1}};
  std::string err;
  const int rc = cn_solve(R, nullptr, 0, frame, results, err);
  return rc == DSH_OK ? rc : dsh_fail(c0, rc, "dsh_sft_connected_solve_group: " + err);
}

#ifdef DSH_LAB
namespace {
struct EventPair {
  hipEvent_t e0 = nullptr, e1 = nullptr;
  hipError_t create() { hipError_t e = hipEventCreate(&e0); return e != hipSuccess ? e : hipEventCreate(&e1); }
  ~EventPair() { if (e0) (void)hipEventDestroy(e0); if (e1) (void)hipEventDestroy(e1); }
};
}

int dsh_lab_set_option(dsh_ctx* c, const char* name, int value) {
  if (!c || !name) return DSH_ERR_ARG;
  const std::string k(name);
  if (k == "waves") { if (value != 0 && value != 4 && value != 8) return dsh_fail(c, DSH_ERR_ARG, "dsh_lab_set_option: waves is 0 (automatic), 4 or 8"); c->opt.waves = value; }
  else if (k == "dataflow") c->opt.dataflow = value != 0;
  else if (k == "wide_off") c->opt.wide_off = value != 0;
  else if (k == "rounds") c->opt.rounds = value != 0;
  else if (k == "streams") { if (value < 0 || value > dsh_ctx::kMaxSub) return dsh_fail(c, DSH_ERR_ARG, "dsh_lab_set_option: streams is 0 (automatic) or 1..4 sub-batches"); c->opt.streams = value; }
  else if (k == "split") { if (value < 0 || value > 2) return dsh_fail(c, DSH_ERR_ARG, "dsh_lab_set_option: split is 0 (off), 1 (wide bands only) or 2 (every band long enough)"); c->opt.split = value; }
  else if (k == "helpers_wbt") { if (value < 1 || value > 16) return dsh_fail(c, DSH_ERR_ARG, "dsh_lab_set_option: helpers_wbt is 1..16 (tiles of half-bandwidth from which parts get helper workgroups)"); c->opt.helpers_wbt = value; }
  else if (k == "owner_waves") { if (value != 8 && value != 16) return dsh_fail(c, DSH_ERR_ARG, "dsh_lab_set_option: owner_waves is 8 or 16 (wavefronts of a FACTOR workgroup with helpers)"); c->opt.owner_waves = value; }
  else if (k == "helpers") { if (value < -1 || value > 3) return dsh_fail(c, DSH_ERR_ARG, "dsh_lab_set_option: helpers is -1 (automatic) or 0..3 workgroups per part"); c->opt.helpers = value; }
  else if (k == "tail") { if (value < -1 || value > 8) return dsh_fail(c, DSH_ERR_ARG, "dsh_lab_set_option: tail is -1 (automatic), 0 (rounds to the end) or the number of problems per CU from which downwards the last problems go to the tail kernel"); c->opt.tail = value; }
  else if (k == "speculate") { if (value < 0 || value > SFT_SPEC_MAXK) return dsh_fail(c, DSH_ERR_ARG, "dsh_lab_set_option: speculate is 0 (automatic) or 1..4 lanes"); c->opt.speculate = value; }
  else return dsh_fail(c, DSH_ERR_ARG, "dsh_lab_set_option: unknown option " + k);
  return DSH_OK;
}

int dsh_lab_sft_solver_info(dsh_ctx* c, int b, int32_t* out8) {
  if (!c || !out8 || b < 0 || b >= c->B) return dsh_fail(c, DSH_ERR_ARG, "dsh_lab_sft_solver_info: bad argument");
  const SftDev& h = c->h_probs[b];
  out8[0] = h.split; out8[1] = h.sp_c0; out8[2] = h.sp_s; out8[3] = h.sp_n1p; out8[4] = h.sp_pad; out8[5] = c->spec_k; out8[6] = h.tile_mode; out8[7] = c->nw;
  return DSH_OK;
}

int dsh_lab_sft_run_timed(dsh_ctx* c, int launches, double* total_ms) {
  if (!c || launches <= 0 || !total_ms) return dsh_fail(c, DSH_ERR_ARG, "dsh_lab_sft_run_timed: bad argument");
  if (const int rc = dsh_enter(c, "dsh_lab_sft_run_timed")) return rc;
  if (c->B <= 0) return dsh_fail(c, DSH_ERR_STATE, "dsh_lab_sft_run_timed: nothing uploaded");
  EventPair ev;
  HIPCHK(c, ev.create());
  HIPCHK(c, hipEventRecord(ev.e0, c->stream));
  for (int i = 0; i < launches; i++) { const int rc = run_once(c); if (rc != DSH_OK) return rc; }
  HIPCHK(c, hipEventRecord(ev.e1, c->stream));
  HIPCHK(c, hipEventSynchronize(ev.e1));
  float ms = 0.f;
  HIPCHK(c, hipEventElapsedTime(&ms, ev.e0, ev.e1));
  *total_ms = (double)ms;
  c->ran = true;
  return DSH_OK;
}

int dsh_lab_sft_assemble_timed(dsh_ctx* c, int launches, double* total_ms) {
  if (!c || launches <= 0 || !total_ms) return dsh_fail(c, DSH_ERR_ARG, "dsh_lab_sft_assemble_timed: bad argument");
  if (const int rc = dsh_enter(c, "dsh_lab_sft_assemble_timed")) return rc;
  if (c->B <= 0 || !c->ran) return dsh_fail(c, DSH_ERR_STATE, "dsh_lab_sft_assemble_timed: needs an uploaded batch that has run once");
  EventPair ev;
  HIPCHK(c, ev.create());
  HIPCHK(c, hipEventRecord(ev.e0, c->stream));
  for (int i = 0; i < launches; i++) HIPCHK(c, sft_assembly_launch(c->d_probs, c->B, c->max_kd, c->jl_doubles, c->rounds_mode ? 8 : c->nw, c->stream));
  HIPCHK(c, hipEventRecord(ev.e1, c->stream));
  HIPCHK(c, hipEventSynchronize(ev.e1));
  float ms = 0.f;
  HIPCHK(c, hipEventElapsedTime(&ms, ev.e0, ev.e1));
  *total_ms = ms;
  c->ran = false;
  return DSH_OK;
}

int dsh_lab_sft_wave_check(dsh_ctx* c, double rel, int launches, int only, double* x_ref, double* x_new, int32_t* ok2, double* ms2) {
  if (!c || launches <= 0 || !ms2) return dsh_fail(c, DSH_ERR_ARG, "dsh_lab_sft_wave_check: bad argument");
  if (const int rc = dsh_enter(c, "dsh_lab_sft_wave_check")) return rc;
  if (c->B <= 0 || !c->ran) return dsh_fail(c, DSH_ERR_STATE, "dsh_lab_sft_wave_check: needs an uploaded batch that has run once");
  for (int b = 0; b < c->B; b++)
    if (c->h_probs[b].tile_mode != 1) return dsh_fail(c, DSH_ERR_STATE, "dsh_lab_sft_wave_check: register-window problems (half-bandwidth <= 128) only");
  HIPCHK(c, sft_assembly_launch(c->d_probs, c->B, c->max_kd, c->jl_doubles, c->rounds_mode ? 8 : c->nw, c->stream));
  EventPair ev;
  HIPCHK(c, ev.create());
  for (int which = 0; which < 2; which++) {
    if (only == 2 - which) continue;
    HIPCHK(c, sft_wave_lab_launch(c->d_probs, c->B, which, rel, c->max_kd, c->jl_doubles, c->stream));
    HIPCHK(c, hipEventRecord(ev.e0, c->stream));
    for (int i = 0; i < launches; i++) HIPCHK(c, sft_wave_lab_launch(c->d_probs, c->B, which, rel, c->max_kd, c->jl_doubles, c->stream));
    HIPCHK(c, hipEventRecord(ev.e1, c->stream));
    HIPCHK(c, hipEventSynchronize(ev.e1));
    float ms = 0.f;
    HIPCHK(c, hipEventElapsedTime(&ms, ev.e0, ev.e1));
    ms2[which] = (double)ms / launches;
    double* dst = which == 0 ? x_ref : x_new;
    size_t off = 0;
    for (int b = 0; b < c->B; b++) {
      const SftDev& h = c->h_probs[b];
      const size_t Dnp = (size_t)((h.Dn + kNB - 1) / kNB) * kNB;
      if (dst) HIPCHK(c, hipMemcpy(dst + off, h.x, 8 * (Dnp + 6), hipMemcpyDeviceToHost));
      off += Dnp + 6;
      double flag = 0.0;
      if (ok2) { HIPCHK(c, hipMemcpy(&flag, h.dbg + 2, 8, hipMemcpyDeviceToHost)); ok2[2 * b + which] = (int32_t)flag; }
    }
  }
  return DSH_OK;
}

int dsh_lab_sft_factor_check(dsh_ctx* c, const double* lambda, const uint8_t* factor, int grid, double* x, int32_t* ok) {
  if (!c || !lambda || grid < 0) return dsh_fail(c, DSH_ERR_ARG, "dsh_lab_sft_factor_check: bad argument");
  if (const int rc = dsh_enter(c, "dsh_lab_sft_factor_check")) return rc;
  if (c->B <= 0 || !c->ran) return dsh_fail(c, DSH_ERR_STATE, "dsh_lab_sft_factor_check: needs an uploaded batch that has run once");
  for (int b = 0; b < c->B; b++)
    if (c->h_probs[b].tile_mode != 1) return dsh_fail(c, DSH_ERR_STATE, "dsh_lab_sft_factor_check: register-window problems (half-bandwidth <= 128) only");
  const int B = c->B;
  struct OwnedDevBuf { void* p = nullptr; ~OwnedDevBuf() { if (p) (void)hipFree(p); } } runs, counters;
  HIPCHK(c, hipMalloc(&runs.p, sizeof(SftRun) * (size_t)B));
  HIPCHK(c, hipMalloc(&counters.p, 16 * sizeof(int)));
  std::vector<SftRun> h_runs(B);
  for (int b = 0; b < B; b++) {
    SftRun& R = h_runs[b];
    std::memset(&R, 0, sizeof(R));
    R.lambda = lambda[b];
    R.state = (!factor || factor[b]) ? SFTB_TRIAL : SFTB_DONE;
    R.fact_ok = -1;
  }
  HIPCHK(c, sft_assembly_launch(c->d_probs, B, c->max_kd, c->jl_doubles, c->rounds_mode ? 8 : c->nw, c->stream));
  for (int b = 0; b < B; b++) HIPCHK(c, hipMemcpyAsync(c->h_probs[b].dbg + 1, &lambda[b], sizeof(double), hipMemcpyHostToDevice, c->stream));
  HIPCHK(c, hipMemcpyAsync(runs.p, h_runs.data(), sizeof(SftRun) * (size_t)B, hipMemcpyHostToDevice, c->stream));
  HIPCHK(c, hipMemsetAsync(counters.p, 0, 16 * sizeof(int), c->stream));
  HIPCHK(c, sftb_factor_lab_launch(c->d_probs, (SftRun*)runs.p, (int*)counters.p, B, grid ? grid : std::min(B, 4 * c->num_cus), c->stream));
  HIPCHK(c, hipStreamSynchronize(c->stream));
  HIPCHK(c, hipMemcpy(h_runs.data(), runs.p, sizeof(SftRun) * (size_t)B, hipMemcpyDeviceToHost));
  size_t off = 0;
  for (int b = 0; b < B; b++) {
    const SftDev& h = c->h_probs[b];
    const size_t Dnp = (size_t)((h.Dn + kNB - 1) / kNB) * kNB;
    if (x) HIPCHK(c, hipMemcpy(x + off, h.x, 8 * (Dnp + 6), hipMemcpyDeviceToHost));
    off += Dnp + 6;
    if (ok) ok[b] = h_runs[b].fact_ok;
  }
  return DSH_OK;
}

int dsh_lab_sft_rounds_timed(dsh_ctx* c, double* ms4, int32_t* rounds) {
  if (!c || !ms4) return dsh_fail(c, DSH_ERR_ARG, "dsh_lab_sft_rounds_timed: bad argument");
  if (const int rc = dsh_enter(c, "dsh_lab_sft_rounds_timed")) return rc;
  if (c->B <= 0 || !c->rounds_mode) return dsh_fail(c, DSH_ERR_STATE, "dsh_lab_sft_rounds_timed: needs an uploaded batch that runs as rounds of phase kernels");
  std::vector<hipEvent_t> ev;
  c->phase_events = &ev;
  c->phase_ids.clear();
  const int rc = run_rounds(c);
  c->phase_events = nullptr;
  (void)hipStreamSynchronize(c->stream);
  for (int i = 0; i < 7; i++) ms4[i] = 0.0;
  { int32_t cnt[16] = {0}; if (hipMemcpy(cnt, c->d_counters, sizeof(cnt), hipMemcpyDeviceToHost) == hipSuccess) { ms4[5] = (double)cnt[8]; ms4[6] = (double)cnt[9]; } }
  int n_trial = 0;
  for (size_t i = 0; i + 1 < ev.size(); i += 2) {
    float ms = 0.f;
    (void)hipEventElapsedTime(&ms, ev[i], ev[i + 1]);
    const int ph = c->phase_ids[i / 2];
    ms4[ph == SFTB_PH_INIT ? 0 : ph == SFTB_PH_LIN ? 1 : ph == SFTB_PH_FACTOR ? 2 : ph == SFTB_PH_TRIAL ? 3 : 4] += ms;
    n_trial += ph == SFTB_PH_TRIAL;
  }
  if (rounds) *rounds = n_trial;
  for (hipEvent_t e : ev) (void)hipEventDestroy(e);
  if (rc == DSH_OK) c->ran = true;
  return rc;
}

int dsh_lab_sft_dump(dsh_ctx* c, int b, int what, int64_t n, double* out) {
  if (!c || !out || b < 0 || b >= c->B || n <= 0) return dsh_fail(c, DSH_ERR_ARG, "dsh_lab_sft_dump: bad argument");
  if (const int rc = dsh_enter(c, "dsh_lab_sft_dump")) return rc;
  const SftDev& h = c->h_probs[b];
  const double* src = what == 0 ? h.Lb : what == 1 ? h.Linv : what == 2 ? h.Lbord : what == 3 ? h.Hc : what == 4 ? h.Hbord : what == 5 ? h.x : what == 6 ? h.Hcorner :
                      (what == 8 || what == 9) ? (const double*)h.part[what - 8].sync : h.dbg;
  if (!src) return dsh_fail(c, DSH_ERR_STATE, "dsh_lab_sft_dump: the problem has no such buffer");
  HIPCHK(c, hipStreamSynchronize(c->stream));
  HIPCHK(c, hipMemcpy(out, src, 8 * (size_t)n, hipMemcpyDeviceToHost));
  return DSH_OK;
}

int dsh_lab_sft_phase_ms(dsh_ctx* c, int b, double* out8) {
  if (!c || !out8 || b < 0 || b >= c->B) return dsh_fail(c, DSH_ERR_ARG, "dsh_lab_sft_phase_ms: bad argument");
  if (const int rc = dsh_enter(c, "dsh_lab_sft_phase_ms")) return rc;
  if (!c->ran) return dsh_fail(c, DSH_ERR_STATE, "dsh_lab_sft_phase_ms: no run");
#ifndef SFT_PHASE_TIMERS
  return dsh_fail(c, DSH_ERR_STATE, "dsh_lab_sft_phase_ms: this build has no phase timers (make lab EXTRA=-DSFT_PHASE_TIMERS)");
#else
  HIPCHK(c, hipStreamSynchronize(c->stream));
  HIPCHK(c, hipMemcpy(out8, c->h_probs[b].dbg, 8 * sizeof(double), hipMemcpyDeviceToHost));
  for (int i = 0; i < 8; i++) out8[i] *= 1e-5;
  {
    double as[6];
    HIPCHK(c, hipMemcpy(as, c->h_probs[b].dbg + 32, sizeof(as), hipMemcpyDeviceToHost));
    std::fprintf(stderr, "[lab] assembly sections of problem %d, kcycles of wave 0: corner %.0f, diagonal gather %.0f, butterfly+finish %.0f, off-diagonal %.0f, round overhead %.0f; rounds %.0f\n",
                 b, as[0] * 1e-3, as[1] * 1e-3, as[2] * 1e-3, as[3] * 1e-3, as[4] * 1e-3, as[5]);
  }
  return DSH_OK;
#endif
}

int dsh_lab_sft_step_trace(dsh_ctx* c, int b, double* out64) {
  if (!c || !out64 || b < 0 || b >= c->B) return dsh_fail(c, DSH_ERR_ARG, "dsh_lab_sft_step_trace: bad argument");
  if (const int rc = dsh_enter(c, "dsh_lab_sft_step_trace")) return rc;
  if (!c->ran) return dsh_fail(c, DSH_ERR_STATE, "dsh_lab_sft_step_trace: no run");
#ifndef SFT_STEP_TRACE
  return dsh_fail(c, DSH_ERR_STATE, "dsh_lab_sft_step_trace: this build has no step trace (make lab EXTRA=-DSFT_STEP_TRACE)");
#else
  HIPCHK(c, hipStreamSynchronize(c->stream));
  HIPCHK(c, hipMemcpy(out64, c->h_probs[b].dbg + 16, 64 * sizeof(double), hipMemcpyDeviceToHost));
  return DSH_OK;
#endif
}

int dsh_lab_sft_system(dsh_ctx* c, int b, int32_t D, double* H, double* bvec, double* chi2) {
  if (!c || b < 0 || b >= c->B) return dsh_fail(c, DSH_ERR_ARG, "dsh_lab_sft_system: bad argument");
  if (const int rc = dsh_enter(c, "dsh_lab_sft_system")) return rc;
  HIPCHK(c, hipStreamSynchronize(c->stream));
  SftDev h = c->h_probs[b];
  if (D != 6 + h.Dn) return dsh_fail(c, DSH_ERR_ARG, "dsh_lab_sft_system: D mismatch");
  const int32_t mode_saved = h.mode, split_saved = h.split;
  h.mode = 1;
  h.split = 0;
  HIPCHK(c, hipMemcpy(c->d_probs + b, &h, sizeof(SftDev), hipMemcpyHostToDevice));
  { LDS_LOCK(); HIPCHK(c, sft_lm_launch(c->d_probs + b, 1, c->max_kd, c->jl_doubles, c->nw, LDS_MARKS(c).lm, c->stream)); }
  HIPCHK(c, hipStreamSynchronize(c->stream));
  c->ran = false;
  h.mode = mode_saved;
  h.split = split_saved;
  HIPCHK(c, hipMemcpy(c->d_probs + b, &h, sizeof(SftDev), hipMemcpyHostToDevice));
  const size_t Dnp = (size_t)((h.Dn + kNB - 1) / kNB) * kNB;
  const size_t band_elems = h.tile_mode ? (Dnp / kTS) * (size_t)h.tpr * kTS * kTS : Dnp * (size_t)h.ldh;
  std::vector<double> Hb(h.tile_mode == 1 ? 0 : band_elems), Hbord(SFT_BORDER * Dnp), Hc(56);
  auto hidx = [&](int r, int cc) -> size_t {
    const size_t tb = ((size_t)(r >> 4) * h.tpr + ((r >> 4) - (cc >> 4))) * (kTS * kTS);
    if (h.tile_mode == 1) return tb + ((((r & 15) & 3) << 4) + (cc & 15)) * 4 + ((r & 15) >> 2);
    if (h.tile_mode == 2) return tb + ((((cc & 15) & 3) << 4) + (r & 15)) * 4 + ((cc & 15) >> 2);
    return (size_t)r * h.ldh + (cc - r + h.kd);
  };
  const dsh::SftGraph& g = *c->packed[b].g;
  std::vector<double> Hcomp;
  if (h.tile_mode == 1) {
    Hcomp.resize(g.hc_elems());
    HIPCHK(c, hipMemcpy(Hcomp.data(), h.Hc, 8 * Hcomp.size(), hipMemcpyDeviceToHost));
  } else {
    HIPCHK(c, hipMemcpy(Hb.data(), h.Hb, 8 * Hb.size(), hipMemcpyDeviceToHost));
  }
  auto hval = [&](int r, int cc) -> double {
    if (h.tile_mode != 1) return Hb[hidx(r, cc)];
    const int I = r >> 4, d = I - (cc >> 4);
    if (d > kBT) return 0.0;
    const int lane = (((r & 15) & 3) << 4) + (cc & 15), q = (r & 15) >> 2;
    return Hcomp[g.hgather[(((size_t)I * (kBT + 1) + d) * 64 + lane) * 4 + q] / 8];
  };
  HIPCHK(c, hipMemcpy(Hbord.data(), h.Hbord, 8 * Hbord.size(), hipMemcpyDeviceToHost));
  HIPCHK(c, hipMemcpy(Hc.data(), h.Hcorner, 8 * 49, hipMemcpyDeviceToHost));
  if (chi2) HIPCHK(c, hipMemcpy(chi2, h.dbg, 8, hipMemcpyDeviceToHost));
  if (H) {
    std::fill(H, H + (size_t)D * D, 0.0);
    for (int r = 0; r < h.Dn; r++)
      for (int k = 0; k <= h.kd; k++) {
        const int cidx = r - h.kd + k;
        if (cidx < 0) continue;
        const double v = hval(r, cidx);
        H[(size_t)(6 + r) + (size_t)(6 + cidx) * D] = v;
        H[(size_t)(6 + cidx) + (size_t)(6 + r) * D] = v;
      }
    for (int k = 0; k < 6; k++)
      for (int r = 0; r < h.Dn; r++) {
        const double v = Hbord[(size_t)k * Dnp + r];
        H[(size_t)k + (size_t)(6 + r) * D] = v;
        H[(size_t)(6 + r) + (size_t)k * D] = v;
      }
    for (int r = 0; r < 6; r++)
      for (int k = 0; k <= r; k++) {
        H[(size_t)r + (size_t)k * D] = Hc[r * 7 + k];
        H[(size_t)k + (size_t)r * D] = Hc[r * 7 + k];
      }
  }
  if (bvec) {
    for (int r = 0; r < 6; r++) bvec[r] = Hc[42 + r];
    for (int r = 0; r < h.Dn; r++) bvec[6 + r] = Hbord[(size_t)6 * Dnp + r];
  }
  return DSH_OK;
}
#endif

}
```

### defslam_amd/csrc/sft_batch.h

```cpp
#pragma once

#define SFTB_NW 8
#ifndef SFTB_LIN_NW
#define SFTB_LIN_NW 8
#endif
#ifndef SFTB_LIN_WAVES
#define SFTB_LIN_WAVES 2
#endif
#ifndef SFTB_TRIAL_WAVES
#define SFTB_TRIAL_WAVES 2
#endif

__device__ __forceinline__ void sftb_ctl_lds(char* smem, Ctl*& ctl, double*& red, double*& out, double*& panel) {
  ctl = reinterpret_cast<Ctl*>(smem);
  red = reinterpret_cast<double*>(smem + 512);
  out = red + 16 * 27 + 5;
  panel = out + 32;
}

__global__ __launch_bounds__(64 * SFTB_NW, 2) void sftb_init_kernel(const SftDev* __restrict__ probs, SftRun* __restrict__ runs, int* __restrict__ counters, int* __restrict__ lin_list, int tail_below) {
  const SftDev& P = probs[blockIdx.x];
  if (blockIdx.x == 0 && threadIdx.x == 0 && (int)gridDim.x <= tail_below) counters[6] = 1;
  init_state<64 * SFTB_NW>(P);
  if (threadIdx.x == 0) {
    SftRun& R = runs[blockIdx.x];
    R.lambda = -1.0; R.ni = 2.0; R.chi_cur = 0.0; R.chi_ini = 0.0; R.rho = 0.0; R.lambda_start = 0.0;
    R.it = 0; R.qmax = 0; R.nbad = 0; R.accepted = 0; R.all_ok = 1; R.iters = 0; R.trials = 0; R.fact_ok = 1;
    R.state = P.max_iters > 0 ? SFTB_LIN : SFTB_FINISH;
    if (P.max_iters > 0) lin_list[atomicAdd(&counters[2], 1)] = blockIdx.x;
  }
}

template <int NW>
__device__ __forceinline__ void sftb_lin_problem(const SftDev& P, SftRun& R, Ctl* ctl, double* red, double* out, double* panel) {
  constexpr int NT = 64 * NW;
  const int tid = threadIdx.x;
  auto nothing = [] {};
  const double chi0 = linearise<NW, decltype(nothing), true>(P, ctl, red, out, panel, nothing);
  double lambda = R.lambda;
  if (R.it == 0) {
    double mx = 0.0;
    for (int r = tid; r < P.Dn; r += NT) mx = fmax(mx, fabs(h_diag(P, r)));
    if (tid < 6) mx = fmax(mx, fabs(P.Hcorner[tid * 8]));
    mx = block_max(mx, red);
    lambda = 1e-5 * mx;
  }
  if (tid == 0) {
    if (R.it == 0) { R.lambda = lambda; R.ni = 2.0; R.nbad = 0; }
    R.chi_cur = chi0; R.chi_ini = chi0; R.qmax = 0; R.rho = 0.0; R.accepted = 0; R.all_ok = 1; R.lambda_start = lambda;
    R.state = SFTB_TRIAL;
  }
}

__global__ __launch_bounds__(64 * SFTB_LIN_NW, SFTB_LIN_WAVES) void sftb_lin_kernel(const SftDev* __restrict__ probs, SftRun* __restrict__ runs, int* __restrict__ counters,
                                                                                  const int* __restrict__ lin_list, int B, int tail_below) {
  constexpr int NW = SFTB_LIN_NW, NT = 64 * NW;
  extern __shared__ __attribute__((aligned(16))) char smem[];
  __shared__ int next_b;
  Ctl* ctl; double *red, *out, *panel;
  sftb_ctl_lds(smem, ctl, red, out, panel);
  const int tid = threadIdx.x;
  if (counters[6] || B - counters[0] <= tail_below) {
    if (blockIdx.x == 0 && tid == 0) counters[6] = 1;
    return;
  }
  if (blockIdx.x == 0 && tid == 0) counters[7]++;
  auto fetch = [&]() { const int i = atomicAdd(&counters[3], 1); return i < counters[2] ? lin_list[i] : -1; };
  int nxt = -1;
  if (tid == 0) nxt = fetch();
  while (true) {
    if (tid == 0) next_b = nxt;
    __syncthreads();
    const int b = __builtin_amdgcn_readfirstlane(next_b);
    if (b < 0) break;
    if (tid == 0) { nxt = fetch(); atomicAdd(&counters[9], 1); }
    sftb_lin_problem<NW>(probs[b], runs[b], ctl, red, out, panel);
  }
}

__global__ __launch_bounds__(64, 1) void sftb_factor_kernel(const SftDev* __restrict__ probs, SftRun* __restrict__ runs, int* __restrict__ counters, int B) {
  extern __shared__ __attribute__((aligned(16))) char smem[];
  lds_double* lds = to_lds(reinterpret_cast<double*>(smem));
  const int lane = threadIdx.x;
  if (counters[6]) return;
  for (int i = lane; i < WV_LDS_DOUBLES; i += 64) lds[i] = 0.0;
  if (blockIdx.x == 0 && lane == 0) { counters[2] = 0; counters[3] = 0; }
  WvPrev Q;
  Q.Lg = nullptr; Q.Linv = nullptr; Q.x = nullptr; Q.nT = 0; Q.active = 0; Q.xb = 0.0;
  int n_done = 0;
  while (true) {
    int b = 0;
    if (lane == 0) b = atomicAdd(&counters[1], 1);
    b = __builtin_amdgcn_readfirstlane(b);
    if (b >= B) break;
    if (runs[b].state != SFTB_TRIAL) continue;
    const SftDev& P = probs[b];
    const double lambda = runs[b].lambda;
    double xcam;
    const int ok = wv_factor(P, lambda, lambda, lds, Q, xcam);
    if (lane == 0) runs[b].fact_ok = ok;
    Q = wv_prev_of(P, ok, xcam, lane);
    n_done++;
  }
  int lane_now;
  asm volatile("v_mbcnt_lo_u32_b32 %0, -1, 0\n\tv_mbcnt_hi_u32_b32 %0, -1, %0" : "=v"(lane_now));
  if (Q.active) wv_backsub_now(Q, lane_now);
  if (lane_now == 0 && n_done) atomicAdd(&counters[8], n_done);
}

template <int NW>
__device__ __forceinline__ int sftb_trial_problem(const SftDev& P, SftRun& R, Ctl* ctl, double* red, double* out, double* panel, int* counters, int* lin_list, int b) {
  constexpr int NT = 64 * NW;
  const int tid = threadIdx.x;
  const int Dn = P.Dn;
  const int Dnp = ((Dn + NB - 1) / NB) * NB;
  const int ok = R.fact_ok;
  const double lam = R.lambda;
  const bool in_lds = P.lds_class >= 1;
  if (!in_lds)
    for (int i = tid; i < 3 * P.n; i += NT) {
      const double v = P.xyz[i];
      P.xyz_bak[i] = v;
      const int a = P.act[i / 3];
      if (a >= 0) P.xyz[i] = v + P.x[3 * a + (i % 3)];
    }
  if (tid < 7) R.pose_bak[tid] = P.pose[tid];
  __syncthreads();
  if (tid == 0) pose_oplus(P.pose, P.x + Dnp);
  double sc = 0.0;
  for (int r = tid; r < Dn; r += NT) { const double xv = P.x[r]; sc += xv * (lam * xv + P.Hbord[(size_t)6 * Dnp + r]); }
  if (tid < 6) { const double xv = P.x[Dnp + tid]; sc += xv * (lam * xv + P.Hcorner[42 + tid]); }
  __syncthreads();
  block_sum<1>(&sc, red, out);
  const double scale = out[0];
  __syncthreads();
  const auto staged = asm_records<NW, 1>(P, panel);
  const double chi_new = in_lds ? eval_edges<false, 1>(P, ctl, red, out, staged, P.x)
                                : eval_edges<false, 0>(P, ctl, red, out, asm_records<NW, 0>(P, panel));
  if (tid == 0) {
    const double tempChi = ok ? chi_new : DBL_MAX;
    double rho = (R.chi_cur - tempChi);
    rho /= (scale + 1e-3);
    R.rho = rho;
    if (rho > 0 && isfinite(tempChi)) {
      double alpha = 1. - pow((2 * rho - 1), 3);
      alpha = fmin(alpha, 2. / 3.);
      const double sf = fmax(1. / 3., alpha);
      R.lambda = lam * sf; R.ni = 2.0; R.chi_cur = tempChi; R.accepted = 1;
      ctl->stop = 0;
    } else {
      R.lambda = lam * R.ni; R.ni *= 2.0;
      ctl->stop = 1;
    }
    R.qmax++;
    R.all_ok &= ok;
    ctl->qmax = R.qmax;
    ctl->rho = rho;
  }
  __syncthreads();
  if (ctl->stop) {
    if (!in_lds)
      for (int i = tid; i < 3 * P.n; i += NT) P.xyz[i] = P.xyz_bak[i];
    if (tid < 7) P.pose[tid] = R.pose_bak[tid];
  } else if (in_lds) {
    for (int i = tid; i < 3 * P.n; i += NT) P.xyz[i] = staged.xyz_l[i];
  }
  const bool again = (ctl->rho < 0) && (ctl->qmax < 10);
  if (again) return 0;
  __syncthreads();
  if (tid == 0) {
    const int qmax = R.qmax;
    R.trials += qmax;
    R.iters++;
    if (P.trace) {
      double* t = P.trace + R.it * 8;
      t[0] = R.chi_ini; t[1] = R.lambda_start; t[2] = qmax; t[3] = R.chi_cur; t[4] = R.lambda; t[5] = R.rho; t[6] = R.accepted; t[7] = R.all_ok;
    }
    if (!R.all_ok) P.res->status |= 1;
    bool term = (qmax == 10) || (R.rho == 0);
    if (!term) {
      if ((R.chi_ini - R.chi_cur) * 1e3 < R.chi_ini) R.nbad++; else R.nbad = 0;
      term = R.nbad >= 3;
    }
    R.it++;
    if (R.it >= P.max_iters) term = true;
    ctl->nbad = term ? 1 : 0;
    ctl->it = R.iters;
    ctl->accepted = R.trials;
    R.state = term ? SFTB_DONE : SFTB_LIN;
    if (!term && lin_list) lin_list[atomicAdd(&counters[2], 1)] = b;
  }
  __syncthreads();
  if (ctl->nbad) {
    const int iters = ctl->it, trials = ctl->accepted;
    __syncthreads();
    classify<NT>(P, ctl, panel, iters, trials);
    if (tid == 0) atomicAdd(&counters[0], 1);
    return 2;
  }
  return 1;
}

__global__ __launch_bounds__(64 * SFTB_NW, SFTB_TRIAL_WAVES) void sftb_trial_kernel(const SftDev* __restrict__ probs, SftRun* __restrict__ runs, int* __restrict__ counters, int* __restrict__ lin_list) {
  constexpr int NW = SFTB_NW, NT = 64 * NW;
  SftRun& R = runs[blockIdx.x];
  const int st = R.state;
  if (counters[6]) return;
  if (blockIdx.x == 0 && threadIdx.x == 0) counters[1] = 0;
  if (st != SFTB_TRIAL && st != SFTB_FINISH) return;
  extern __shared__ __attribute__((aligned(16))) char smem[];
  const SftDev& P = probs[blockIdx.x];
  Ctl* ctl; double *red, *out, *panel;
  sftb_ctl_lds(smem, ctl, red, out, panel);
  const int tid = threadIdx.x;
  if (st == SFTB_FINISH) {
    classify<NT>(P, ctl, panel, 0, 0);
    if (tid == 0) { R.state = SFTB_DONE; atomicAdd(&counters[0], 1); }
    return;
  }
  (void)sftb_trial_problem<NW>(P, R, ctl, red, out, panel, counters, lin_list, blockIdx.x);
}

__device__ __noinline__ void sftb_solve8(const SftDev& P, unsigned ctl_off, unsigned ws_off, double lambda) {
  typedef __attribute__((address_space(3))) char lds_char;
  Ctl* ctl = reinterpret_cast<Ctl*>((char*)(lds_char*)(size_t)__builtin_amdgcn_readfirstlane(ctl_off));
  double* ws = reinterpret_cast<double*>((char*)(lds_char*)(size_t)__builtin_amdgcn_readfirstlane(ws_off));
  factor_tiles_df8<1>(P, ctl, ws, lambda, true);
  backsub_tiles<8>(P, ctl, ws);
}

__global__ __launch_bounds__(64 * SFTB_NW, SFT_WAVES_PER_EU) void sftb_tail_kernel(const SftDev* __restrict__ probs, SftRun* __restrict__ runs, int* __restrict__ counters, int B, int tail_below) {
  constexpr int NW = SFTB_NW, NT = 64 * NW;
  extern __shared__ __attribute__((aligned(16))) char smem[];
  Ctl* ctl; double *red, *out, *panel;
  sftb_ctl_lds(smem, ctl, red, out, panel);
  const int tid = threadIdx.x;
  if (!counters[6]) {
    if (B - counters[0] > tail_below) return;
    if (blockIdx.x == 0 && tid == 0) counters[6] = 1;
  }
  while (true) {
    __syncthreads();
    if (tid == 0) ctl->it = atomicAdd(&counters[5], 1);
    __syncthreads();
    const int b = __builtin_amdgcn_readfirstlane(ctl->it);
    __syncthreads();
    if (b >= B) break;
    SftRun& R = runs[b];
    const SftDev& P = probs[b];
    int st = R.state;
    if (st == SFTB_FINISH) {
      classify<NT>(P, ctl, panel, 0, 0);
      if (tid == 0) { R.state = SFTB_DONE; atomicAdd(&counters[0], 1); }
      continue;
    }
    while (st == SFTB_LIN || st == SFTB_TRIAL) {
      if (st == SFTB_LIN) {
        sftb_lin_problem<NW>(P, R, ctl, red, out, panel);
        __syncthreads();
      }
      if (tid == 0) ctl->lambda = R.lambda;
      __syncthreads();
      sftb_solve8(P, (unsigned)(size_t)(__attribute__((address_space(3))) char*)(char*)ctl, (unsigned)(size_t)(__attribute__((address_space(3))) char*)(char*)panel, R.lambda);
      if (tid == 0) R.fact_ok = ctl->fact_ok;
      __syncthreads();
      const int r = sftb_trial_problem<NW>(P, R, ctl, red, out, panel, counters, nullptr, b);
      __syncthreads();
      st = r == 0 ? SFTB_TRIAL : (r == 1 ? SFTB_LIN : SFTB_DONE);
    }
  }
}
```

### defslam_amd/csrc/sft_kernels.hip

```cpp
#include <hip/hip_runtime.h>
#include <type_traits>
#include <utility>
#include <algorithm>
#include <cstdio>
#include <cstdlib>
#include <math.h>
#include <float.h>
#define SFT_KERNEL_SOURCE
#include "sft_problem.h"
#include "tile_chol.h"

#define NB 32

#if defined(SFT_PHASE_TIMERS) && defined(DSH_LAB)
#define PH_T0() long long ph_t0__ = wall_clock64()
#define PH_ADD(slot)                                                          \
  do {                                                                        \
    const long long t1__ = wall_clock64();                                    \
    if (threadIdx.x == 0) P.dbg[slot] += (double)(t1__ - ph_t0__);            \
    ph_t0__ = t1__;                                                           \
  } while (0)
#define PH_RESET() ph_t0__ = wall_clock64()
#define AS_T0() long long as_t0__ = clock64()
#define AS_ADD(slot) do { const long long t1__ = clock64(); if (threadIdx.x == 0) P.dbg[slot] += (double)(t1__ - as_t0__); as_t0__ = t1__; } while (0)
// ... 2773 lines not shown
    for (int i = tid; i < 3 * P.n; i += NT) {
      const int a = P.act[i / 3];
      if (a >= 0) P.xyz[i] += P.x[3 * a + (i % 3)];
    }
    if (tid == 0) pose_oplus(P.pose, P.x + Dnp);
    double sc = 0.0;
    const double lam = S.lambda;
    for (int r = tid; r < Dn; r += NT) { const double xv = P.x[r]; sc += xv * (lam * xv + P.Hbord[(size_t)6 * Dnp + r]); }
    if (tid < 6) { const double xv = P.x[Dnp + tid]; sc += xv * (lam * xv + P.Hcorner[42 + tid]); }
    __syncthreads();
    block_sum<1>(&sc, red, out);
    const double scale = out[0];
    __syncthreads();
    const double chi_new = eval_edges<false, 0>(P, ctl, red, out, asm_records<NW, 0>(P, panel));
    if (tid == 0) {
      const int ok = S.fact_ok;
      S.all_ok &= ok;
      const double tempChi = ok ? chi_new : DBL_MAX;
      double rho = (S.chi_cur - tempChi);
      rho /= (scale + 1e-3);
      S.rho = rho;
      if (rho > 0 && isfinite(tempChi)) {
        double alpha = 1. - pow((2 * rho - 1), 3);
        alpha = fmin(alpha, 2. / 3.);
        const double sf = fmax(1. / 3., alpha);
        S.lambda *= sf; S.ni = 2.0; S.chi_cur = tempChi; S.accepted = 1;
        ctl->stop = 0;
      } else {
        S.lambda *= S.ni; S.ni *= 2.0;
        ctl->stop = 1;
      }
      S.qmax++;
    }
    __syncthreads();
    if (ctl->stop) {
      for (int i = tid; i < 3 * P.n; i += NT) P.xyz[i] = P.xyz_bak[i];
      if (tid < 7) P.pose[tid] = S.pose_bak[tid];
    }
    __syncthreads();
    const bool again = (S.rho < 0) && (S.qmax < 10);
    bool finished = false;
    if (!again) {
      if (tid == 0) {
        S.trials += S.qmax;
        S.iters++;
        if (P.trace) {
          double* t = P.trace + S.it * 8;
          t[0] = S.chi_ini; t[1] = S.lambda_start; t[2] = S.qmax; t[3] = S.chi_cur; t[4] = S.lambda; t[5] = S.rho; t[6] = S.accepted; t[7] = S.all_ok;
        }
        if (!S.all_ok) P.res->status |= 1;
        bool term = (S.qmax == 10) || (S.rho == 0);
        if (!term) {
          if ((S.chi_ini - S.chi_cur) * 1e3 < S.chi_ini) S.nbad++; else S.nbad = 0;
          term = S.nbad >= 3;
        }
        S.it++;
        if (S.it >= P.max_iters) term = true;
        S.done = term ? 1 : 0;
        ctl->qmax = term ? 1 : 0;
      }
      __syncthreads();
      finished = ctl->qmax != 0;
    }
    if (tid == 0) S.again = again ? 1 : 0;
    if (finished) classify<NT>(P, ctl, panel, S.iters, S.trials);
  }
}

#include "sft_batch.h"

#ifdef DSH_LAB
template <int NW>
__global__ __launch_bounds__(64 * NW, SFT_WAVES_PER_EU) void sft_assembly_kernel(const SftDev* __restrict__ probs) {
  constexpr int NT = 64 * NW;
  extern __shared__ __attribute__((aligned(16))) char smem[];
  const SftDev& P = probs[blockIdx.x];
  Ctl* ctl = reinterpret_cast<Ctl*>(smem);
  double* red = reinterpret_cast<double*>(smem + 512);
  double* out = red + 16 * 27 + 5;
  double* panel = out + 32;
  const int tid = threadIdx.x;
  for (int i = tid; i < 3 * P.n; i += NT) P.xyz[i] = P.xyz_init[i];
  if (tid < 7) P.pose[tid] = P.pose_init[tid];
  __syncthreads();
  double chi = 0.0;
  switch (P.lds_class) {
    case 3: { const auto jp = asm_records<NW, 3>(P, panel); chi = eval_edges<true, 3>(P, ctl, red, out, jp); assemble<NW, 3>(P, red, out, jp); break; }
    case 2: { const auto jp = asm_records<NW, 2>(P, panel); chi = eval_edges<true, 2>(P, ctl, red, out, jp); assemble<NW, 2>(P, red, out, jp); break; }
    case 1: { const auto jp = asm_records<NW, 1>(P, panel); chi = eval_edges<true, 1>(P, ctl, red, out, jp); assemble<NW, 1>(P, red, out, jp); break; }
    default: { const auto jp = asm_records<NW, 0>(P, panel); chi = eval_edges<true, 0>(P, ctl, red, out, jp); assemble<NW, 0>(P, red, out, jp); break; }
  }
  if (tid == 0) P.dbg[0] = chi;
}

template <int NW>
__device__ __forceinline__ void ref_factor_solve(const SftDev& P, Ctl* ctl, double* panel) {
  tile_factor<NW>(P, ctl, panel);
  backsub_tiles<NW>(P, ctl, panel);
}
template <int NW>
__global__ __launch_bounds__(64 * NW, SFT_WAVES_PER_EU) void sft_ref_solve_kernel(const SftDev* __restrict__ probs, double rel) {
  constexpr int NT = 64 * NW;
  extern __shared__ __attribute__((aligned(16))) char smem[];
  const SftDev& P = probs[blockIdx.x];
  Ctl* ctl = reinterpret_cast<Ctl*>(smem);
  double* red = reinterpret_cast<double*>(smem + 512);
  double* out = red + 16 * 27 + 5;
  double* panel = out + 32;
  const int tid = threadIdx.x;
  double mx = 0.0;
  for (int r = tid; r < P.Dn; r += NT) mx = fmax(mx, fabs(h_diag(P, r)));
  if (tid < 6) mx = fmax(mx, fabs(P.Hcorner[tid * 8]));
  mx = block_max(mx, red);
  if (tid == 0) { ctl->lambda = rel * 1e-5 * mx; P.dbg[1] = ctl->lambda; }
  __syncthreads();
  ref_factor_solve<NW>(P, ctl, panel);
  if (tid == 0) P.dbg[2] = ctl->fact_ok;
}
__global__ __launch_bounds__(64, 1) void sft_wave_solve_kernel(const SftDev* __restrict__ probs) {
  extern __shared__ __attribute__((aligned(16))) char smem[];
  const SftDev& P = probs[blockIdx.x];
  const double lambda = P.dbg[1];
  const int ok = wv_factor_solve(P, lambda, lambda, to_lds(reinterpret_cast<double*>(smem)));
  int lane_now;
  asm volatile("v_mbcnt_lo_u32_b32 %0, -1, 0\n\tv_mbcnt_hi_u32_b32 %0, -1, %0" : "=v"(lane_now));
  if (lane_now == 0) P.dbg[2] = ok;
}
#endif

}


extern "C" size_t sft_lm_kernel_lds_bytes(int kd, size_t jl_doubles) {
  const size_t rows = NB + kd + SFT_BORDER;
  const size_t LDP = rows | 1;
  size_t panel = (size_t)NB * LDP + 2 * NB * NB;
  const size_t backsub = NB + (SFT_NT / NB) * NB + NB * NB;
  if (backsub > panel) panel = backsub;
  const size_t tiles = (size_t)(BT + 2 * (BT + 1) + 3) * TILE_LDS + 3 * SFT_BORDER * TS + 64 + 48 + 128 + 128;
  if (kd <= TS * BT) panel = tiles;
  else if (kd <= TS * WB) panel = std::max(panel, std::max((size_t)2 * WB * TS * TS + TILE_LDS + 704, (size_t)(SFT_WIDE_NEAR + 2) * SFT_WIDE_NEAR * TS * TS + 2 * TILE_LDS + 704 + (size_t)32 * TS * TS + (size_t)(WB - SFT_WIDE_NEAR + 1) * TS * TS));
  if (jl_doubles > panel) panel = jl_doubles;
  return 512 + (16 * 27 + 5 + 32 + panel) * sizeof(double) + 64;
}

#ifdef DSH_LAB
extern "C" hipError_t sft_assembly_launch(const SftDev* d_probs, int B, int max_kd, size_t jl_doubles, int nw, hipStream_t stream) {
  const size_t lds = sft_lm_kernel_lds_bytes(max_kd, jl_doubles);
  const void* fn = nw == 4 ? reinterpret_cast<const void*>(sft_assembly_kernel<4>) : reinterpret_cast<const void*>(sft_assembly_kernel<8>);
  hipError_t e = hipFuncSetAttribute(fn, hipFuncAttributeMaxDynamicSharedMemorySize, (int)lds);
  if (e != hipSuccess) return e;
  if (nw == 4) hipLaunchKernelGGL(sft_assembly_kernel<4>, dim3(B), dim3(256), lds, stream, d_probs);
  else hipLaunchKernelGGL(sft_assembly_kernel<8>, dim3(B), dim3(512), lds, stream, d_probs);
  return hipGetLastError();
}
#endif

extern "C" hipError_t sft_sc_launch(const SftDev* d_probs, SftSc* d_sc, int B, int phase, int max_kd, size_t jl_doubles, size_t* configured, hipStream_t stream) {
  const size_t lds = sft_lm_kernel_lds_bytes(max_kd, jl_doubles);
  if (lds > *configured) {
    hipError_t e = hipFuncSetAttribute(reinterpret_cast<const void*>(sft_sc_kernel<8>), hipFuncAttributeMaxDynamicSharedMemorySize, (int)lds);
    if (e != hipSuccess) return e;
    *configured = lds;
  }
  hipLaunchKernelGGL(sft_sc_kernel<8>, dim3(B), dim3(512), lds, stream, d_probs, d_sc, phase);
  return hipGetLastError();
}

extern "C" hipError_t sft_cn_launch(const SftDev* d_probs, SftSc* d_sc, int phase, int max_kd, size_t jl_doubles, size_t* configured, hipStream_t stream) {
  const size_t lds = sft_lm_kernel_lds_bytes(max_kd, jl_doubles);
  if (lds > *configured) {
    hipError_t e = hipFuncSetAttribute(reinterpret_cast<const void*>(sft_cn_kernel<8>), hipFuncAttributeMaxDynamicSharedMemorySize, (int)lds);
    if (e != hipSuccess) return e;
    *configured = lds;
  }
  hipLaunchKernelGGL(sft_cn_kernel<8>, dim3(1), dim3(512), lds, stream, d_probs, d_sc, phase);
  return hipGetLastError();
}

extern "C" hipError_t sftb_tail_launch(const SftDev* d_probs, SftRun* d_runs, int* d_counters, int B, int max_kd, size_t jl_doubles, size_t* configured, int num_cus, int tail_below, hipStream_t stream) {
  const size_t lds = sft_lm_kernel_lds_bytes(max_kd, jl_doubles);
  if (lds > *configured) {
    hipError_t e = hipFuncSetAttribute(reinterpret_cast<const void*>(sftb_tail_kernel), hipFuncAttributeMaxDynamicSharedMemorySize, (int)lds);
    if (e != hipSuccess) return e;
    *configured = lds;
  }
  hipLaunchKernelGGL(sftb_tail_kernel, dim3(std::min(B, num_cus)), dim3(64 * SFTB_NW), lds, stream, d_probs, d_runs, d_counters, B, tail_below);
  return hipGetLastError();
}

#ifdef DSH_LAB
__global__ __launch_bounds__(1024) void sft_part_factor_kernel(const SftDev* __restrict__ probs, SftSpec* __restrict__ specs, int K, int nh) {
  constexpr int NT = 1024;
  extern __shared__ __attribute__((aligned(16))) char smem[];
  const int roles = 1 + nh, per_role = gridDim.x / roles;
  const int role = blockIdx.x / per_role, bid = blockIdx.x % per_role;
  const int fpart = bid % 2, bx = bid / 2;
  const int B = per_role / (K * 2), b = bx / K, j = bx % K;
  const SftDev& P = probs[(size_t)j * B + b];
  const SftSpec& S = specs[(size_t)j * B + b];
  Ctl* ctl = reinterpret_cast<Ctl*>(smem);
  double* red = reinterpret_cast<double*>(smem + 512);
  double* panel = red + 16 * 27 + 5 + 32;
  const int tid = threadIdx.x;
  if (S.done) return;
  if (!(P.tile_mode == 2 && P.split) || S.need_lin == 1) return;
  if (S.qbase + j >= 10) return;
  const int epoch = S.launches + 1;
  if (role > 0) {
    factor_wide_helper<16>(P, fpart, role - 1, nh, epoch, ctl, panel);
    return;
  }
  double lam = S.lambda, ni = S.ni;
  if (S.need_lin == 2 && S.it == 0) {
    double mx = 0.0;
    for (int r = tid; r < P.Dn; r += NT) mx = fmax(mx, fabs(h_diag(P, r)));
    if (tid < 6) mx = fmax(mx, fabs(P.Hcorner[tid * 8]));
    mx = block_max(mx, red);
    lam = 1e-5 * mx; ni = 2.0;
  }
  for (int t = 0; t < j; t++) { lam *= ni; ni *= 2.0; }
  if (tid == 0) ctl->lambda = lam;
  __syncthreads();
  factor_part<SFT_WIDE_NEAR, 16>(P, fpart, ctl, panel, epoch, nh);
}
#endif

__global__ void sft_vec_sum2_kernel(const double* a, const double* b, double* out_a, double* out_b, int n) {
  for (int i = blockIdx.x * blockDim.x + threadIdx.x; i < n; i += gridDim.x * blockDim.x) {
    const double v = a[i] + b[i];
    out_a[i] = v;
    out_b[i] = v;
  }
}
extern "C" hipError_t sft_vec_sum2(const double* a, const double* b, double* out_a, double* out_b, int n, hipStream_t stream) {
  hipLaunchKernelGGL(sft_vec_sum2_kernel, dim3(64), dim3(256), 0, stream, a, b, out_a, out_b, n);
  return hipGetLastError();
}

extern "C" hipError_t sft_spec_launch(const SftDev* d_probs, SftSpec* d_spec, int B, int K, int phase, int nh, int owner_waves, int max_kd, size_t jl_doubles, size_t* configured, hipStream_t stream) {
  const size_t lds = sft_lm_kernel_lds_bytes(max_kd, jl_doubles);
#ifdef DSH_LAB
  if (phase == SFT_SPEC_FACTOR && nh > 0 && owner_waves == 16) {
    if (lds > configured[1]) {
      hipError_t e = hipFuncSetAttribute(reinterpret_cast<const void*>(sft_part_factor_kernel), hipFuncAttributeMaxDynamicSharedMemorySize, (int)lds);
      if (e != hipSuccess) return e;
      configured[1] = lds;
    }
    hipLaunchKernelGGL(sft_part_factor_kernel, dim3(B * K * 2 * (1 + nh)), dim3(1024), lds, stream, d_probs, d_spec, K, nh);
    return hipGetLastError();
  }
#endif
  if (lds > *configured) {
    hipError_t e = hipFuncSetAttribute(reinterpret_cast<const void*>(sft_spec_kernel<8>), hipFuncAttributeMaxDynamicSharedMemorySize, (int)lds);
    if (e != hipSuccess) return e;
    *configured = lds;
  }
  const int wgs = (phase == SFT_SPEC_FACTOR || phase == SFT_SPEC_SOLVE) ? 2 : 1, roles = phase == SFT_SPEC_FACTOR ? 1 + nh : 1;
  hipLaunchKernelGGL(sft_spec_kernel<8>, dim3(B * K * wgs * roles), dim3(512), lds, stream, d_probs, d_spec, K, phase, nh);
  return hipGetLastError();
}

__global__ void sft_sc_local_reduce_kernel(SftSc* const* scs, int G) {
  const int i = threadIdx.x;
  if (i >= SFT_SC_XCHG) return;
  double s = 0.0;
  for (int g = 0; g < G; g++) s += scs[g]->send[i];
  for (int g = 0; g < G; g++) scs[g]->recv[i] = s;
}
extern "C" hipError_t sft_sc_local_reduce(SftSc* const* d_ptrs, int G, hipStream_t stream) {
  hipLaunchKernelGGL(sft_sc_local_reduce_kernel, dim3(1), dim3(64), 0, stream, d_ptrs, G);
  return hipGetLastError();
}

extern "C" hipError_t sft_lm_launch(const SftDev* d_probs, int B, int max_kd, size_t jl_doubles, int nw, size_t* configured, hipStream_t stream) {
  const size_t lds = sft_lm_kernel_lds_bytes(max_kd, jl_doubles);
  const int slot = nw == 4 ? 0 : 1;
  if (lds > configured[slot]) {
    const void* fn = nw == 4 ? reinterpret_cast<const void*>(sft_lm_kernel<4>) : reinterpret_cast<const void*>(sft_lm_kernel<8>);
    hipError_t e = hipFuncSetAttribute(fn, hipFuncAttributeMaxDynamicSharedMemorySize, (int)lds);
    if (e != hipSuccess) return e;
    configured[slot] = lds;
  }
  if (nw == 4) hipLaunchKernelGGL(sft_lm_kernel<4>, dim3(B), dim3(256), lds, stream, d_probs);
  else hipLaunchKernelGGL(sft_lm_kernel<8>, dim3(B), dim3(512), lds, stream, d_probs);
  return hipGetLastError();
}

#ifdef DSH_LAB
extern "C" hipError_t sft_wave_lab_launch(const SftDev* d_probs, int B, int which, double rel, int max_kd, size_t jl_doubles, hipStream_t stream) {
  if (which == 0) {
    (void)jl_doubles;
    const size_t lds = sft_lm_kernel_lds_bytes(max_kd, 0);
    hipError_t e = hipFuncSetAttribute(reinterpret_cast<const void*>(sft_ref_solve_kernel<4>), hipFuncAttributeMaxDynamicSharedMemorySize, (int)lds);
    if (e != hipSuccess) return e;
    hipLaunchKernelGGL(sft_ref_solve_kernel<4>, dim3(B), dim3(256), lds, stream, d_probs, rel);
  } else {
    hipLaunchKernelGGL(sft_wave_solve_kernel, dim3(B), dim3(64), WV_LDS_DOUBLES * sizeof(double), stream, d_probs);
  }
  return hipGetLastError();
}
#endif

extern "C" hipError_t sftb_launch(const SftDev* d_probs, SftRun* d_runs, int* d_counters, int* d_list, int B, int phase, size_t jl_doubles, size_t xyz_doubles, size_t* configured, int num_cus, int tail_below, hipStream_t stream) {
  const size_t head = 512 + (16 * 27 + 5 + 32) * sizeof(double) + 64;
  if (phase == SFTB_PH_INIT) {
    hipError_t e = hipMemsetAsync(d_counters, 0, 16 * sizeof(int), stream);
    if (e != hipSuccess) return e;
    hipLaunchKernelGGL(sftb_init_kernel, dim3(B), dim3(64 * SFTB_NW), 0, stream, d_probs, d_runs, d_counters, d_list, tail_below);
  } else if (phase == SFTB_PH_LIN) {
    const size_t lds = head + jl_doubles * sizeof(double);
    if (lds > configured[0]) {
      hipError_t e = hipFuncSetAttribute(reinterpret_cast<const void*>(sftb_lin_kernel), hipFuncAttributeMaxDynamicSharedMemorySize, (int)lds);
      if (e != hipSuccess) return e;
      configured[0] = lds;
    }
    const int per_cu = lds > 80 * 1024 ? 1 : 2;
    hipLaunchKernelGGL(sftb_lin_kernel, dim3(std::min(B, per_cu * num_cus)), dim3(64 * SFTB_LIN_NW), lds, stream, d_probs, d_runs, d_counters, d_list, B, tail_below);
  } else if (phase == SFTB_PH_FACTOR) {
    hipLaunchKernelGGL(sftb_factor_kernel, dim3(std::min(B, 4 * num_cus)), dim3(64), WV_LDS_DOUBLES * sizeof(double), stream, d_probs, d_runs, d_counters, B);
  } else {
    const size_t lds = head + std::max<size_t>(2048, xyz_doubles) * sizeof(double);
    if (lds > configured[1]) {
      hipError_t e = hipFuncSetAttribute(reinterpret_cast<const void*>(sftb_trial_kernel), hipFuncAttributeMaxDynamicSharedMemorySize, (int)lds);
      if (e != hipSuccess) return e;
      configured[1] = lds;
    }
    hipLaunchKernelGGL(sftb_trial_kernel, dim3(B), dim3(64 * SFTB_NW), lds, stream, d_probs, d_runs, d_counters, d_list);
  }
  return hipGetLastError();
}

#ifdef DSH_LAB
extern "C" hipError_t sftb_factor_lab_launch(const SftDev* d_probs, SftRun* d_runs, int* d_counters, int B, int grid, hipStream_t stream) {
  hipLaunchKernelGGL(sftb_factor_kernel, dim3(grid), dim3(64), WV_LDS_DOUBLES * sizeof(double), stream, d_probs, d_runs, d_counters, B);
  return hipGetLastError();
}
#endif
```

### defslam_amd/csrc/sft_problem.h

```cpp
#pragma once
#include <stdint.h>

#define SFT_NT 512
#define SFT_CAM_STRIDE 16
#define SFT_BORDER 7
#define SFT_H_PAD_TILE_ROWS 9
#define SFT_H_PAD_BORDER 160

#define SFT_KIND_OBS 0u
#define SFT_KIND_REF 1u
#define SFT_KIND_STAR 2u
#define SFT_KIND_STR 3u
#define SFT_REC(kind, s, t, e) (((uint32_t)(kind) << 30) | ((uint32_t)(s) << 26) | ((uint32_t)(t) << 22) | (uint32_t)(e))

#if defined(__HIP_DEVICE_COMPILE__) && defined(SFT_KERNEL_SOURCE)
#define SFT_G __attribute__((address_space(1)))
#else
#define SFT_G
#endif

struct SftResHdr {
  int32_t iters, trials, status, inliers;
  double rep_error;
  double pose[8];
  double pad[5];
};

#define SFT_SC_XCHG 32
#define SFT_SC_LIN 0
#define SFT_SC_FAC 1
#define SFT_SC_SOL 2
#define SFT_SC_CTL 3
#define SFT_CN_LIN 0
#define SFT_CN_FAC 1
#define SFT_CN_SOL 2
#define SFT_CN_CTL 3
struct SftSc {
  double send[SFT_SC_XCHG], recv[SFT_SC_XCHG];
  double lambda, ni, chi_cur, chi_ini, rho, lambda_start;
  double bc[6];
  double pose_bak[8];
  int32_t it, qmax, nbad, accepted, again, done, all_ok, fact_ok, iters, trials, rank, nranks;
};

#define SFT_SPEC_MAXK 4
#define SFT_SPEC_INIT 0
#define SFT_SPEC_LIN 1
#define SFT_SPEC_TRIAL 2
#ifndef SFT_WAVES_PER_EU
#define SFT_WAVES_PER_EU 2
#endif
#define SFT_SPEC_FACTOR 3
#define SFT_SPEC_SOLVE 4
struct SftSpecRes { double chi_new, scale, lambda, ni, pose[8]; int32_t ok, valid; };
struct SftSpec {
  double lambda, ni, chi_cur, chi_ini, lambda_start, rho;
  double pose_bak[8];
  int32_t it, qbase, nbad, accepted, all_ok, iters, trials, done, launches, need_lin, last_lane, pad;
  SftSpecRes res[2];
};

#define SFTB_LIN 0
#define SFTB_TRIAL 1
#define SFTB_DONE 2
#define SFTB_FINISH 3
#define SFTB_PH_INIT 0
#define SFTB_PH_LIN 1
#define SFTB_PH_FACTOR 2
#define SFTB_PH_TRIAL 3
#define SFTB_PH_TAIL 4
struct SftRun {
  double lambda, ni, chi_cur, chi_ini, rho, lambda_start;
  double pose_bak[8];
  int32_t it, qmax, nbad, accepted, all_ok, iters, trials, state, fact_ok, pad[3];
};

struct SftPart {
  int32_t nT, nS, tpr, wbt;
  int32_t b_base, b_sign, b_lo, b_hi;
  SFT_G double* Hb;
  SFT_G double *Lb, *Lt, *LbT, *Lbord, *Linv, *x;
  SFT_G double* xchg;
  SFT_G double *Pf, *PfB;
  SFT_G int32_t* sync;
};

struct SftDev {
  int32_t n, nA, Dn, kd, ldh, M, V, S, Es, noff, max_iters, mode;
  int32_t tile_mode;
  int32_t pad1;
  int32_t lds_class;
  int32_t tpr, wbt;
  int32_t pad0;
  double fx, fy, cx, cy;
  double w_ref, w_curv, w_str, hub_delta, hub_dsqr;
  const SFT_G double* xyz0;
  const SFT_G int32_t* nbr_ptr;
  const SFT_G int32_t* nbr_idx;
  const SFT_G double* nbr_w;
  const SFT_G double* nbr_sumw;
  const SFT_G double* k0;
  const SFT_G int32_t* act;
  const SFT_G int32_t* actnode;
  const SFT_G int32_t* star_node;
  const SFT_G double* star_sL;
  const SFT_G int32_t* str_nodes;
  const SFT_G double* str_L0;
  const SFT_G int32_t* off_ptr;
  const SFT_G int32_t* off_rc;
  const SFT_G int32_t* sh_ptr;
  const SFT_G uint32_t* sh_rec;
  const SFT_G double* sh_cf;
  const SFT_G int32_t* tmask;
  const SFT_G uint32_t* hgatherT;
  const SFT_G uint32_t* hgather;
  const SFT_G int32_t* obs_nodes;
  const SFT_G double* obs_bary;
  const SFT_G double* obs_uv;
  const SFT_G double* obs_w;
  const SFT_G int32_t* ob_ptr;
  const SFT_G int32_t* ob_m;
  const SFT_G double* ob_c;
  const SFT_G uint8_t* viewed;
  const SFT_G double* xyz_init;
  const SFT_G double* pose_init;
  SFT_G double* xyz;
  SFT_G double* xyz_bak;
  SFT_G double* pose;
  SFT_G double* camrec;
  SFT_G double* wtv;
  SFT_G double* Anode;
  SFT_G double* Jstar;
  SFT_G double* Jstr;
  SFT_G double* Hc;
  SFT_G double* Hb;
  SFT_G double* Hbord;
  SFT_G double* Hcorner;
  SFT_G double* Lb;
  SFT_G double* Lbord;
  SFT_G double* Lcorner;
  SFT_G double* Linv;
  SFT_G double* Lt;
  SFT_G double* LbT;
  SFT_G double* x;
  SFT_G double* chi2_obs;
  SFT_G double* trace;
  SFT_G SftResHdr* res;
  SFT_G uint8_t* outlier;
  SFT_G float* mappoint;
  SFT_G double* dbg;
  SFT_G double* spec_xyz[2];
  int32_t split;
  int32_t sp_c0, sp_s, sp_n1p, sp_pad;
  int32_t sp_xl;
  int32_t pad2[2];
  SftPart part[4];
};

#include <hip/hip_runtime.h>
#include <stddef.h>
extern "C" size_t sft_lm_kernel_lds_bytes(int kd, size_t jl_doubles);
extern "C" hipError_t sft_lm_launch(const SftDev* d_probs, int B, int max_kd, size_t jl_doubles, int nw, size_t* configured, hipStream_t stream);
extern "C" hipError_t sftb_launch(const SftDev* d_probs, SftRun* d_runs, int* d_counters, int* d_list, int B, int phase, size_t jl_doubles, size_t xyz_doubles,
                                  size_t* configured, int num_cus, int tail_below, hipStream_t stream);
extern "C" hipError_t sftb_tail_launch(const SftDev* d_probs, SftRun* d_runs, int* d_counters, int B, int max_kd, size_t jl_doubles, size_t* configured, int num_cus,
                                       int tail_below, hipStream_t stream);
extern "C" hipError_t sft_spec_launch(const SftDev* d_probs, SftSpec* d_spec, int B, int K, int phase, int nh, int owner_waves, int max_kd, size_t jl_doubles,
                                      size_t* configured, hipStream_t stream);
extern "C" hipError_t sft_sc_launch(const SftDev* d_probs, SftSc* d_sc, int B, int phase, int max_kd, size_t jl_doubles, size_t* configured, hipStream_t stream);
extern "C" hipError_t sft_sc_local_reduce(SftSc* const* d_ptrs, int G, hipStream_t stream);
extern "C" hipError_t sft_cn_launch(const SftDev* d_probs, SftSc* d_sc, int phase, int max_kd, size_t jl_doubles, size_t* configured, hipStream_t stream);
extern "C" hipError_t sft_vec_sum2(const double* a, const double* b, double* out_a, double* out_b, int n, hipStream_t stream);
#ifdef DSH_LAB
extern "C" hipError_t sft_wave_lab_launch(const SftDev* d_probs, int B, int which, double rel, int max_kd, size_t jl_doubles, hipStream_t stream);
extern "C" hipError_t sft_assembly_launch(const SftDev* d_probs, int B, int max_kd, size_t jl_doubles, int nw, hipStream_t stream);
extern "C" hipError_t sftb_factor_lab_launch(const SftDev* d_probs, SftRun* d_runs, int* d_counters, int B, int grid, hipStream_t stream);
#endif
```

### defslam_amd/sft.py

```python
from __future__ import annotations

import ctypes as C
from dataclasses import dataclass, field
from typing import List, Optional, Sequence

import numpy as np

from . import _lib


class DshError(RuntimeError):
    pass


def _ptr(a: Optional[np.ndarray], ctype):
    if a is None:
        return None
    return a.ctypes.data_as(C.POINTER(ctype))


@dataclass
class Frame:
    Tcw: np.ndarray
    K: np.ndarray
    N: int
    obs_nodes: np.ndarray
    obs_bary: np.ndarray
    obs_uv: np.ndarray
    obs_invsig2: np.ndarray
    nodes_xyz: np.ndarray
    mvbOutlier: np.ndarray = field(default=None)
    repError: float = 0.0
    mappoints: np.ndarray = field(default=None)
    pose7: np.ndarray = field(default=None)
    chi2_obs: np.ndarray = field(default=None)
    iters: int = 0
    trials: int = 0
    dim: int = 0
    half_bandwidth: int = 0
    status: int = 0
    trace: np.ndarray = field(default=None)
    regs: Optional[tuple] = None


class Context:

    def __init__(self, device: int = 0, lab: bool = False):
        self.lab = bool(lab)
        self._L = _lib.load_lab() if lab else _lib.load()
        h = C.c_void_p()
        rc = self._L.dsh_create(C.byref(h), device)
        if rc != _lib.DSH_OK:
            raise DshError(f"dsh_create failed with status {rc} (no gfx950 device visible?)")
        self._h = h
        self.n = 0
        self._keep = None

    def close(self):
        if getattr(self, "_events", None) is not None:
            self._events.close()
            self._events = None
        if getattr(self, "_h", None):
            self._L.dsh_destroy(self._h)
            self._h = None

    def __del__(self):
        try:
            self.close()
        except Exception:
            pass

    def _check(self, rc: int, what: str):
        if rc != _lib.DSH_OK:
            raise DshError(f"{what}: status {rc}: {self._L.dsh_last_error(self._h).decode()}")

    def template_build(self, xyz0: np.ndarray, facets: np.ndarray):
        xyz0 = np.ascontiguousarray(xyz0, np.float64)
        facets = np.ascontiguousarray(facets, np.int32)
        self._check(self._L.dsh_template_build(self._h, xyz0.shape[0], _ptr(xyz0, C.c_double), facets.shape[0], _ptr(facets, C.c_int32)),
                    "dsh_template_build")
        self.n = xyz0.shape[0]

    def template_set(self, xyz0, boundary, nbr_ptr, nbr_idx, nbr_w, k0, edge_nodes, edge_L0, median_L):
        xyz0 = np.ascontiguousarray(xyz0, np.float64)
        boundary = np.ascontiguousarray(boundary, np.uint8)
        nbr_ptr = np.ascontiguousarray(nbr_ptr, np.int32)
        nbr_idx = np.ascontiguousarray(nbr_idx, np.int32)
        nbr_w = np.ascontiguousarray(nbr_w, np.float64)
        k0 = np.ascontiguousarray(k0, np.float64)
        edge_nodes = np.ascontiguousarray(edge_nodes, np.int32)
        edge_L0 = np.ascontiguousarray(edge_L0, np.float64)
        self._check(self._L.dsh_template_set(self._h, xyz0.shape[0], _ptr(xyz0, C.c_double), _ptr(boundary, C.c_uint8), _ptr(nbr_ptr, C.c_int32),
                                             _ptr(nbr_idx, C.c_int32), _ptr(nbr_w, C.c_double), _ptr(k0, C.c_double), edge_L0.shape[0],
                                             _ptr(edge_nodes, C.c_int32), _ptr(edge_L0, C.c_double), float(median_L)), "dsh_template_set")
        self.n = xyz0.shape[0]

    def template_get(self) -> dict:
        n, E, nnz = C.c_int32(), C.c_int32(), C.c_int32()
        self._check(self._L.dsh_template_dims(self._h, C.byref(n), C.byref(E), C.byref(nnz)), "dsh_template_dims")
        out = dict(boundary=np.zeros(n.value, np.uint8), nbr_ptr=np.zeros(n.value + 1, np.int32), nbr_idx=np.zeros(nnz.value, np.int32),
                   nbr_w=np.zeros(nnz.value), k0=np.zeros(n.value), edge_nodes=np.zeros((E.value, 2), np.int32), edge_L0=np.zeros(E.value))
        med = C.c_double()
        self._check(self._L.dsh_template_get(self._h, _ptr(out["boundary"], C.c_uint8), _ptr(out["nbr_ptr"], C.c_int32), _ptr(out["nbr_idx"], C.c_int32),
                                             _ptr(out["nbr_w"], C.c_double), _ptr(out["k0"], C.c_double), _ptr(out["edge_nodes"], C.c_int32),
                                             _ptr(out["edge_L0"], C.c_double), C.byref(med)), "dsh_template_get")
        out["median_L"] = med.value
        return out

    def template_embed(self, pts: np.ndarray):
        pts = np.ascontiguousarray(pts, np.float32)
        P = pts.shape[0]
        fid = np.zeros(P, np.int32)
        nodes = np.zeros((P, 3), np.int32)
        bary = np.zeros((P, 3), np.float32)
        self._check(self._L.dsh_template_embed(self._h, P, _ptr(pts, C.c_float), _ptr(fid, C.c_int32), _ptr(nodes, C.c_int32), _ptr(bary, C.c_float)),
                    "dsh_template_embed")
        return fid, nodes, bary

    def template_embed_device(self, pts: np.ndarray):
        pts = np.ascontiguousarray(pts, np.float32)
        P = pts.shape[0]
        fid = np.zeros(P, np.int32)
        nodes = np.zeros((P, 3), np.int32)
        bary = np.zeros((P, 3), np.float32)
        self._check(self._L.dsh_template_embed_device(self._h, P, _ptr(pts, C.c_float), _ptr(fid, C.c_int32), _ptr(nodes, C.c_int32), _ptr(bary, C.c_float)),
                    "dsh_template_embed_device")
        return fid, nodes, bary

    def _frame_c(self, f: Frame, reg_lap, reg_inex, reg_temp, layers, max_iters, keep: list) -> _lib.SftFrameC:
        Tcw = np.ascontiguousarray(f.Tcw, np.float32)
        nodes = np.ascontiguousarray(f.obs_nodes, np.int32)
        bary = np.ascontiguousarray(f.obs_bary, np.float64)
        uv = np.ascontiguousarray(f.obs_uv, np.float64)
        isg = np.ascontiguousarray(f.obs_invsig2, np.float64)
        xyz = np.ascontiguousarray(f.nodes_xyz, np.float64)
        keep += [Tcw, nodes, bary, uv, isg, xyz]
        fc = _lib.SftFrameC()
        fc.Tcw = _ptr(Tcw, C.c_float)
        for i in range(4):
            fc.K[i] = float(f.K[i])
        fc.n_frame = int(f.N)
        fc.M = int(nodes.shape[0])
        fc.obs_nodes = _ptr(nodes, C.c_int32)
        fc.obs_bary = _ptr(bary, C.c_double)
        fc.obs_uv = _ptr(uv, C.c_double)
        fc.obs_invsig2 = _ptr(isg, C.c_double)
        fc.xyz = _ptr(xyz, C.c_double)
        if f.regs is not None:
            reg_lap, reg_inex, reg_temp = f.regs
        fc.reg_lap, fc.reg_inex, fc.reg_temp = float(reg_lap), float(reg_inex), float(reg_temp)
        fc.neighbour_layers = int(layers)
        fc.max_iters = int(max_iters)
        return fc

    def batch_upload(self, frames: Sequence[Frame], RegLap=5000.0, RegInex=5000.0, RegTemp=0.0, NeighboursLayers=1, max_iters=50):
        keep: list = []
        arr = (_lib.SftFrameC * len(frames))()
        for i, f in enumerate(frames):
            arr[i] = self._frame_c(f, RegLap, RegInex, RegTemp, NeighboursLayers, max_iters, keep)
        self._check(self._L.dsh_sft_batch_upload(self._h, len(frames), arr), "dsh_sft_batch_upload")
        self._frames = list(frames)
        self._max_iters = max_iters

    def batch_run(self):
        self._check(self._L.dsh_sft_batch_run(self._h), "dsh_sft_batch_run")

    def batch_run_timed(self, launches: int = 1) -> float:
        if getattr(self, "_events", None) is None:
            self._events = _lib.HipEvents()
        st = self.stream()
        self._events.start(st)
        for _ in range(int(launches)):
            self.batch_run()
        return self._events.stop_ms(st)

    def _need_lab(self, what: str):
        if not self.lab:
            raise DshError(f"{what} is a lab entry point (include/defslam_hip_debug.h): create the context with Context(device, lab=True)")

    def set_option(self, name: str, value: int):
        self._need_lab("dsh_lab_set_option")
        self._check(self._L.dsh_lab_set_option(self._h, name.encode(), int(value)), "dsh_lab_set_option")

    def solver_info(self, b: int = 0) -> dict:
        self._need_lab("dsh_lab_sft_solver_info")
        o = (C.c_int32 * 8)()
        self._check(self._L.dsh_lab_sft_solver_info(self._h, int(b), o), "dsh_lab_sft_solver_info")
        return dict(split=int(o[0]), c0=int(o[1]), s=int(o[2]), n1p=int(o[3]), pad=int(o[4]), lanes=int(o[5]), tile_mode=int(o[6]), waves=int(o[7]))

    def lab_run_timed(self, launches: int = 1) -> float:
        self._need_lab("dsh_lab_sft_run_timed")
        ms = C.c_double()
        self._check(self._L.dsh_lab_sft_run_timed(self._h, int(launches), C.byref(ms)), "dsh_lab_sft_run_timed")
        return ms.value

    def batch_assemble_timed(self, launches: int = 1) -> float:
        self._need_lab("dsh_lab_sft_assemble_timed")
        ms = C.c_double()
        self._check(self._L.dsh_lab_sft_assemble_timed(self._h, int(launches), C.byref(ms)), "dsh_lab_sft_assemble_timed")
        return ms.value

    def wave_check(self, rel: float = 1.0, launches: int = 1, only: int = 0):
        self._need_lab("dsh_lab_sft_wave_check")
        B = len(self._frames)
        dims = []
        for b in range(B):
            _, counts = self.problem_info(b)
            Dn = int(counts[5]) - 6
            dims.append(((Dn + 31) // 32) * 32 + 6)
        tot = int(sum(dims))
        xr, xn = np.zeros(tot), np.zeros(tot)
        ok = np.zeros((B, 2), np.int32)
        ms = np.zeros(2)
        self._check(self._L.dsh_lab_sft_wave_check(self._h, C.c_double(rel), int(launches), int(only), _ptr(xr, C.c_double), _ptr(xn, C.c_double), _ptr(ok, C.c_int32),
                                                   _ptr(ms, C.c_double)), "dsh_lab_sft_wave_check")
        offs = np.concatenate([[0], np.cumsum(dims)])
        return [xr[offs[b]:offs[b + 1]] for b in range(B)], [xn[offs[b]:offs[b + 1]] for b in range(B)], ok, ms

    def factor_check(self, lam, factor=None, grid: int = 0):
        self._need_lab("dsh_lab_sft_factor_check")
        B = len(self._frames)
        lam = np.ascontiguousarray(lam, np.float64)
        if lam.shape != (B,):
            raise ValueError(f"factor_check: lam must have one damping per problem ({B})")
        fac = None if factor is None else np.ascontiguousarray(np.asarray(factor, bool).astype(np.uint8))
        if fac is not None and fac.shape != (B,):
            raise ValueError(f"factor_check: factor must have one flag per problem ({B})")
        dims = []
        for b in range(B):
            Dn = int(self.problem_info(b)[1][5]) - 6
            dims.append(((Dn + 31) // 32) * 32 + 6)
        x = np.zeros(int(sum(dims)))
        ok = np.zeros(B, np.int32)
        self._check(self._L.dsh_lab_sft_factor_check(self._h, _ptr(lam, C.c_double), _ptr(fac, C.c_uint8), int(grid), _ptr(x, C.c_double),
                                                     _ptr(ok, C.c_int32)), "dsh_lab_sft_factor_check")
        offs = np.concatenate([[0], np.cumsum(dims)])
        return [x[offs[b]:offs[b + 1]] for b in range(B)], ok

    def rounds_timed(self):
        self._need_lab("dsh_lab_sft_rounds_timed")
        ms = np.zeros(7)
        r = np.zeros(1, np.int32)
        self._check(self._L.dsh_lab_sft_rounds_timed(self._h, _ptr(ms, C.c_double), _ptr(r, C.c_int32)), "dsh_lab_sft_rounds_timed")
        return dict(init=float(ms[0]), lin=float(ms[1]), factor=float(ms[2]), trial=float(ms[3]), tail=float(ms[4]), factorisations_in_rounds=int(ms[5]), linearisations_in_rounds=int(ms[6])), int(r[0])

    def dump(self, b: int, what: int, n: int):
        self._need_lab("dsh_lab_sft_dump")
        out = np.zeros(int(n))
        self._check(self._L.dsh_lab_sft_dump(self._h, int(b), int(what), int(n), _ptr(out, C.c_double)), "dsh_lab_sft_dump")
        return out

    def phase_ms(self, b: int = 0):
        self._need_lab("dsh_lab_sft_phase_ms")
        out = np.zeros(8)
        self._check(self._L.dsh_lab_sft_phase_ms(self._h, b, _ptr(out, C.c_double)), "dsh_lab_sft_phase_ms")
        return dict(trsm=out[0], residuals=out[1], assembly=out[2], copy=out[3], panel=out[4], update=out[5], backsub=out[6], control=out[7])

    def step_trace(self, b: int = 0):
        self._need_lab("dsh_lab_sft_step_trace")
        out = np.zeros(64)
        self._check(self._L.dsh_lab_sft_step_trace(self._h, b, _ptr(out, C.c_double)), "dsh_lab_sft_step_trace")
        return out.reshape(8, 8)

    def synchronize(self):
        self._check(self._L.dsh_synchronize(self._h), "dsh_synchronize")

    def stream(self) -> int:
        return int(self._L.dsh_stream(self._h) or 0)

    def batch_counts(self):
        it, tr = C.c_int64(), C.c_int64()
        self._check(self._L.dsh_sft_batch_counts(self._h, C.byref(it), C.byref(tr)), "dsh_sft_batch_counts")
        return it.value, tr.value

    def problem_info(self, b: int):
        nbytes = C.c_int64()
        counts = np.zeros(9, np.int32)
        self._check(self._L.dsh_sft_batch_problem_info(self._h, b, C.byref(nbytes), _ptr(counts, C.c_int32)), "dsh_sft_batch_problem_info")
        return nbytes.value, counts

    def batch_download(self, only=None) -> List[int]:
        frames = self._frames
        res = (_lib.SftResultC * len(frames))()
        keep = []
        want = None if only is None else set(int(i) for i in only)
        for i, f in enumerate(frames):
            if want is not None and i not in want:
                keep.append(None)
                continue
            M, n = f.obs_nodes.shape[0], f.nodes_xyz.shape[0]
            bufs = dict(Tcw=np.zeros((4, 4), np.float32), pose7=np.zeros(7), xyz=np.zeros((n, 3)), chi2=np.zeros(M), outl=np.zeros(M, np.uint8),
                        mp=np.zeros((M, 3), np.float32), trace=np.zeros((max(self._max_iters, 1), _lib.DSH_TRACE_STRIDE)))
            keep.append(bufs)
            r = res[i]
            r.Tcw = _ptr(bufs["Tcw"], C.c_float)
            r.pose7 = _ptr(bufs["pose7"], C.c_double)
            r.xyz = _ptr(bufs["xyz"], C.c_double)
            r.chi2_obs = _ptr(bufs["chi2"], C.c_double)
            r.outlier = _ptr(bufs["outl"], C.c_uint8)
            r.mappoint_xyz = _ptr(bufs["mp"], C.c_float)
            r.trace = _ptr(bufs["trace"], C.c_double)
        self._check(self._L.dsh_sft_batch_download(self._h, len(frames), res), "dsh_sft_batch_download")
        out = []
        for i, f in enumerate(frames):
            b, r = keep[i], res[i]
            if b is None:
                f.iters, f.trials, f.dim, f.half_bandwidth, f.status = r.iters, r.trials, r.dim, r.half_bandwidth, r.status
                out.append(int(r.inliers))
                continue
            f.Tcw = b["Tcw"]
            f.pose7 = b["pose7"]
            f.nodes_xyz = b["xyz"]
            f.chi2_obs = b["chi2"]
            f.mvbOutlier = b["outl"].astype(bool)
            f.mappoints = b["mp"]
            f.repError = float(np.float32(r.rep_error))
            f.rep_error_f64 = r.rep_error
            f.iters, f.trials, f.dim, f.half_bandwidth, f.status = r.iters, r.trials, r.dim, r.half_bandwidth, r.status
            f.trace = b["trace"][:r.iters].copy()
            out.append(int(r.inliers))
        return out

    def prepare_solve(self, f: Frame, RegLap=5000.0, RegInex=5000.0, RegTemp=0.0, NeighboursLayers=1, max_iters=50):
        keep: list = []
        fc = self._frame_c(f, RegLap, RegInex, RegTemp, NeighboursLayers, max_iters, keep)
        M, n = f.obs_nodes.shape[0], f.nodes_xyz.shape[0]
        b = dict(Tcw=np.zeros((4, 4), np.float32), pose7=np.zeros(7), xyz=np.zeros((n, 3)), chi2=np.zeros(M), outl=np.zeros(M, np.uint8),
                 mp=np.zeros((M, 3), np.float32), trace=np.zeros((max(max_iters, 1), _lib.DSH_TRACE_STRIDE)))
        r = _lib.SftResultC()
        r.Tcw = _ptr(b["Tcw"], C.c_float)
        r.pose7 = _ptr(b["pose7"], C.c_double)
        r.xyz = _ptr(b["xyz"], C.c_double)
        r.chi2_obs = _ptr(b["chi2"], C.c_double)
        r.outlier = _ptr(b["outl"], C.c_uint8)
        r.mappoint_xyz = _ptr(b["mp"], C.c_float)
        r.trace = _ptr(b["trace"], C.c_double)
        ctx = self

        class _Call:
            frame = f

            def __call__(self_inner) -> int:
                rc = ctx._L.dsh_sft_solve(ctx._h, C.byref(fc), C.byref(r))
                if rc != _lib.DSH_OK:
                    ctx._check(rc, "dsh_sft_solve")
                f.Tcw, f.pose7, f.nodes_xyz, f.chi2_obs, f.mappoints = b["Tcw"], b["pose7"], b["xyz"], b["chi2"], b["mp"]
                f.mvbOutlier = b["outl"].view(np.bool_)
                f.repError = float(np.float32(r.rep_error))
                f.rep_error_f64 = r.rep_error
                f.iters, f.trials, f.dim, f.half_bandwidth, f.status = r.iters, r.trials, r.dim, r.half_bandwidth, r.status
                f.trace = b["trace"][:r.iters]
                return int(r.inliers)

        call = _Call()
        call._keep = (keep, b, fc, r)
        return call

    def debug_system(self, b: int, D: int):
        self._need_lab("dsh_lab_sft_system")
        H = np.zeros((D, D), order="F")
        bv = np.zeros(D)
        chi = C.c_double()
        self._check(self._L.dsh_lab_sft_system(self._h, b, D, _ptr(H, C.c_double), _ptr(bv, C.c_double), C.byref(chi)), "dsh_lab_sft_system")
        return H, bv, chi.value


def DefPoseOptimization(ctx: Context, pFrame: Frame, RegLap: float = 5000, RegInex: float = 5000, RegTemp: float = 0,
                        NeighboursLayers: int = 1, max_iters: int = 50) -> int:
    ctx.batch_upload([pFrame], RegLap, RegInex, RegTemp, NeighboursLayers, max_iters)
    ctx.batch_run()
    return ctx.batch_download()[0]


def DefPoseOptimizationBatch(ctx: Context, frames: Sequence[Frame], RegLap: float = 5000, RegInex: float = 5000, RegTemp: float = 0,
                             NeighboursLayers: int = 1, max_iters: int = 50) -> List[int]:
    ctx.batch_upload(frames, RegLap, RegInex, RegTemp, NeighboursLayers, max_iters)
    ctx.batch_run()
    return ctx.batch_download()


def _result_buffers(f: Frame, max_iters: int):
    M, n = f.obs_nodes.shape[0], f.nodes_xyz.shape[0]
    b = dict(Tcw=np.zeros((4, 4), np.float32), pose7=np.zeros(7), xyz=np.zeros((n, 3)), chi2=np.zeros(M), outl=np.zeros(M, np.uint8),
             mp=np.zeros((M, 3), np.float32), trace=np.zeros((max(max_iters, 1), _lib.DSH_TRACE_STRIDE)))
    r = _lib.SftResultC()
    r.Tcw = _ptr(b["Tcw"], C.c_float)
    r.pose7 = _ptr(b["pose7"], C.c_double)
    r.xyz = _ptr(b["xyz"], C.c_double)
    r.chi2_obs = _ptr(b["chi2"], C.c_double)
    r.outlier = _ptr(b["outl"], C.c_uint8)
    r.mappoint_xyz = _ptr(b["mp"], C.c_float)
    r.trace = _ptr(b["trace"], C.c_double)
    return b, r


def _write_back(f: Frame, b: dict, r) -> int:
    f.Tcw, f.pose7, f.nodes_xyz, f.chi2_obs, f.mappoints = b["Tcw"], b["pose7"], b["xyz"], b["chi2"], b["mp"]
    f.mvbOutlier = b["outl"].astype(bool)
    f.repError = float(np.float32(r.rep_error))
    f.rep_error_f64 = r.rep_error
    f.iters, f.trials, f.dim, f.half_bandwidth, f.status = r.iters, r.trials, r.dim, r.half_bandwidth, r.status
    f.trace = b["trace"][:r.iters].copy()
    return int(r.inliers)


def comm_unique_id() -> bytes:
    buf = C.create_string_buffer(_lib.DSH_COMM_ID_BYTES)
    if _lib.load().dsh_comm_unique_id(buf) != _lib.DSH_OK:
        raise DshError("dsh_comm_unique_id failed (RCCL not available?)")
    return buf.raw


class Comm:

    def __init__(self, ctx: Context, nranks: int, rank: int, unique_id: bytes):
        self._ctx = ctx
        h = C.c_void_p()
        buf = C.create_string_buffer(bytes(unique_id), _lib.DSH_COMM_ID_BYTES)
        ctx._check(ctx._L.dsh_comm_create(ctx._h, int(nranks), int(rank), buf, C.byref(h)), "dsh_comm_create")
        self._h = h
        self.nranks, self.rank = int(nranks), int(rank)

    def close(self):
        if getattr(self, "_h", None):
            self._ctx._L.dsh_comm_destroy(self._h)
            self._h = None


def SharedCameraPoseOptimization(ctx: Context, comm: Comm, pFrame: Frame, RegLap: float = 5000, RegInex: float = 5000, RegTemp: float = 0,
                                 NeighboursLayers: int = 1, max_iters: int = 50) -> int:
    keep: list = []
    fc = ctx._frame_c(pFrame, RegLap, RegInex, RegTemp, NeighboursLayers, max_iters, keep)
    b, r = _result_buffers(pFrame, max_iters)
    ctx._check(ctx._L.dsh_sft_shared_solve(ctx._h, comm._h, C.byref(fc), C.byref(r)), "dsh_sft_shared_solve")
    return _write_back(pFrame, b, r)


def SharedCameraPoseOptimizationGroup(ctxs: Sequence[Context], frames: Sequence[Frame], RegLap: float = 5000, RegInex: float = 5000, RegTemp: float = 0,
                                      NeighboursLayers: int = 1, max_iters: int = 50) -> List[int]:
    G = len(ctxs)
    keep: list = []
    fcs = (_lib.SftFrameC * G)()
    res = (_lib.SftResultC * G)()
    bufs = []
    for g in range(G):
        fcs[g] = ctxs[g]._frame_c(frames[g], RegLap, RegInex, RegTemp, NeighboursLayers, max_iters, keep)
        b, r = _result_buffers(frames[g], max_iters)
        bufs.append(b)
        res[g] = r
    hs = (C.c_void_p * G)(*[c._h for c in ctxs])
    ctxs[0]._check(ctxs[0]._L.dsh_sft_shared_solve_group(G, hs, fcs, res), "dsh_sft_shared_solve_group")
    return [_write_back(frames[g], bufs[g], res[g]) for g in range(G)]


def ConnectedPoseOptimization(ctx: Context, comm: Comm, pFrame: Frame, RegLap: float = 5000, RegInex: float = 5000, RegTemp: float = 0,
                              NeighboursLayers: int = 1, max_iters: int = 50) -> int:
    keep: list = []
    fc = ctx._frame_c(pFrame, RegLap, RegInex, RegTemp, NeighboursLayers, max_iters, keep)
    b, r = _result_buffers(pFrame, max_iters)
    ctx._check(ctx._L.dsh_sft_connected_solve(ctx._h, comm._h, C.byref(fc), C.byref(r)), "dsh_sft_connected_solve")
    return _write_back(pFrame, b, r)


def ConnectedPoseOptimizationGroup(ctx0: Context, ctx1: Context, frames: Sequence[Frame], RegLap: float = 5000, RegInex: float = 5000, RegTemp: float = 0,
                                   NeighboursLayers: int = 1, max_iters: int = 50) -> List[int]:
    keep: list = []
    fc = ctx0._frame_c(frames[0], RegLap, RegInex, RegTemp, NeighboursLayers, max_iters, keep)
    res = (_lib.SftResultC * 2)()
    bufs = []
    for g in range(2):
        b, r = _result_buffers(frames[g], max_iters)
        bufs.append(b)
        res[g] = r
    ctx0._check(ctx0._L.dsh_sft_connected_solve_group(ctx0._h, ctx1._h, C.byref(fc), res), "dsh_sft_connected_solve_group")
    return [_write_back(frames[g], bufs[g], res[g]) for g in range(2)]


def two_sided_cut(Dn: int, kd: int):
    sT = -(-kd // 16)
    s = 16 * sT
    c0 = ((Dn - s) // 2 // 16) * 16
    n1 = Dn - s - c0
    if sT < 2 or c0 < 64 or n1 < 64:
        return None
    n1p = -(-n1 // 16) * 16
    return c0, s, n1p, n1p - n1


def frame_from_synth(fr) -> Frame:
    return Frame(Tcw=fr.Tcw.copy(), K=fr.K.copy(), N=fr.n_frame, obs_nodes=fr.obs_nodes, obs_bary=fr.obs_bary, obs_uv=fr.obs_uv,
                 obs_invsig2=fr.obs_invsig2, nodes_xyz=fr.xyz.copy())
```

### include/defslam_hip_debug.h

```cpp
#ifndef DEFSLAM_HIP_DEBUG_H
#define DEFSLAM_HIP_DEBUG_H

#include "defslam_hip.h"

#ifdef __cplusplus
extern "C" {
#endif
#if defined(__GNUC__)
#pragma GCC visibility push(default)
#endif

int dsh_lab_set_option(dsh_ctx* ctx, const char* name, int value);
int dsh_lab_sft_solver_info(dsh_ctx* ctx, int b, int32_t* out8);

int dsh_lab_sft_run_timed(dsh_ctx* ctx, int launches, double* total_ms);
int dsh_lab_sft_assemble_timed(dsh_ctx* ctx, int launches, double* total_ms);
int dsh_lab_sft_wave_check(dsh_ctx* ctx, double rel, int launches, int only, double* x_ref, double* x_new, int32_t* ok2, double* ms2);
int dsh_lab_sft_factor_check(dsh_ctx* ctx, const double* lambda, const uint8_t* factor, int grid, double* x, int32_t* ok);
int dsh_lab_sft_rounds_timed(dsh_ctx* ctx, double* ms7, int32_t* rounds);
int dsh_lab_sft_dump(dsh_ctx* ctx, int b, int what, int64_t n, double* out);
int dsh_lab_sft_phase_ms(dsh_ctx* ctx, int b, double* out8);
int dsh_lab_sft_step_trace(dsh_ctx* ctx, int b, double* out64);
int dsh_lab_sft_system(dsh_ctx* ctx, int b, int32_t D, double* H, double* bvec, double* chi2);

#if defined(__GNUC__)
#pragma GCC visibility pop
#endif
#ifdef __cplusplus
}
#endif
#endif
```

Measured before the change: 420,500.

## Add plan kernel and carry-over pending factorisations across rounds

Adds a single-workgroup PLAN kernel that builds a rotated, compacted list of problems awaiting factorisation. The FACTOR kernel now walks that list instead of atomically scanning every problem, and can optionally leave the last wave set's factors pending, finished at the start of the next round or in a RESOLVE pass before the tail. Carry is off by default, so the default path only gains the extra plan launch per round in exchange for a denser factor queue. The risk is added launch overhead and more rounds when carry is enabled.

```diff
diff --git a/defslam_amd/_lib.py b/defslam_amd/_lib.py
--- a/defslam_amd/_lib.py
+++ b/defslam_amd/_lib.py
@@ -144,7 +144,7 @@
 
 LAB_SYMBOLS = ["dsh_lab_set_option", "dsh_lab_sft_run_timed", "dsh_lab_sft_assemble_timed", "dsh_lab_sft_phase_ms", "dsh_lab_sft_step_trace",
                "dsh_lab_sft_system", "dsh_lab_sft_solver_info", "dsh_lab_sft_wave_check", "dsh_lab_sft_dump", "dsh_lab_sft_rounds_timed",
-               "dsh_lab_sft_factor_check"]
+               "dsh_lab_sft_factor_check", "dsh_lab_sft_plan_host"]
 
 _lib = None
 _lab = None
@@ -283,7 +283,11 @@
         L.dsh_lab_sft_rounds_timed.argtypes = [vp, c_double_p, c_i32_p]
         L.dsh_lab_sft_factor_check.argtypes = [vp, c_double_p, c_u8_p, C.c_int, c_double_p, c_i32_p]
         for name in LAB_SYMBOLS:
+            if name == "dsh_lab_sft_plan_host" and not hasattr(L, name):
+                continue
             getattr(L, name).restype = C.c_int
+        if hasattr(L, "dsh_lab_sft_plan_host"):
+            L.dsh_lab_sft_plan_host.argtypes = [c_i32_p, i32, i32, i32, i32, c_i32_p, c_i32_p]
     return L
 
 
diff --git a/defslam_amd/csrc/dsh_api.cpp b/defslam_amd/csrc/dsh_api.cpp
--- a/defslam_amd/csrc/dsh_api.cpp
+++ b/defslam_amd/csrc/dsh_api.cpp
@@ -98,7 +98,7 @@
   std::vector<int> phase_ids;
   int num_cus = 256;
   bool ran = false;
-  struct { int waves = 0; int dataflow = 1; int wide_off = 0; int speculate = 0; int split = 2; int rounds = 1; int streams = 0; int helpers = -1; int tail = -1; int owner_waves = 8; int helpers_wbt = 12; } opt;
+  struct { int waves = 0; int dataflow = 1; int wide_off = 0; int speculate = 0; int split = 2; int rounds = 1; int streams = 0; int helpers = -1; int tail = -1; int owner_waves = 8; int helpers_wbt = 12; int carry = SFTB_CARRY_OFF; int factor_waves = 0; } opt;
   bool any_split = false;
 };
 
@@ -243,6 +243,11 @@
     if (c->opt.tail > 0) tail_below = c->opt.tail * c->num_cus;
     else tail_below = std::min(4 * c->num_cus, std::max(2 * c->num_cus, (int)((long long)3 * B / 4)));
   }
+  int factor_waves = 4 * c->num_cus, carry = SFTB_CARRY_OFF;
+#ifdef DSH_LAB
+  if (c->opt.factor_waves > 0) factor_waves = std::min(factor_waves, c->opt.factor_waves);
+  if (S == 1) carry = c->opt.carry;
+#endif
   auto launch = [&](int s, int phase) {
     const bool ev = c->phase_events && S == 1;
     if (ev) { hipEvent_t e; if (hipEventCreate(&e) == hipSuccess) { (void)hipEventRecord(e, c->stream); c->phase_events->push_back(e); c->phase_ids.push_back(phase); } }
@@ -250,8 +255,8 @@
     {
       LDS_LOCK();
       if (phase == SFTB_PH_TAIL) r = sftb_tail_launch(c->d_probs + b0[s], c->d_runs + b0[s], c->d_counters + 16 * s, b0[s + 1] - b0[s], c->max_kd, c->jl_doubles, &LDS_MARKS(c).tail, c->num_cus, tail_below, c->sub_stream[s]);
-      else r = sftb_launch(c->d_probs + b0[s], c->d_runs + b0[s], c->d_counters + 16 * s, c->d_linlist + b0[s], b0[s + 1] - b0[s], phase, c->jl_doubles, c->xyz_doubles, LDS_MARKS(c).b,
-                           c->num_cus, tail_below, c->sub_stream[s]);
+      else r = sftb_launch(c->d_probs + b0[s], c->d_runs + b0[s], c->d_counters + 16 * s, c->d_linlist + 3 * (size_t)b0[s], b0[s + 1] - b0[s], phase, c->jl_doubles, c->xyz_doubles, LDS_MARKS(c).b,
+                           c->num_cus, tail_below, std::min(b0[s + 1] - b0[s], factor_waves), carry, c->sub_stream[s]);
     }
     if (ev) { hipEvent_t e; if (hipEventCreate(&e) == hipSuccess) { (void)hipEventRecord(e, c->stream); c->phase_events->push_back(e); } }
     return r;
@@ -261,7 +266,7 @@
     for (int s = 1; s < S; s++) HIPCHK(c, hipStreamWaitEvent(c->sub_stream[s], c->sub_event[0], 0));
   }
   for (int s = 0; s < S; s++) HIPCHK(c, launch(s, SFTB_PH_INIT));
-  const int worst = std::max(1, c->max_iters_batch) * 10 + 1;
+  const int worst = (std::max(1, c->max_iters_batch) * 10 + 1) * (carry == SFTB_CARRY_OFF ? 1 : carry == SFTB_CARRY_AUTO ? 3 : 3 + (B + factor_waves - 1) / factor_waves);
   int rounds = 0, group = std::max(1, std::min(worst, c->rounds_hint));
   if (tail_below >= B) group = 0;
   HIPCHK(c, c->spec_done.ensure(64 * dsh_ctx::kMaxSub, true));
@@ -270,10 +275,14 @@
     for (int i = 0; i < group && rounds < worst; i++, rounds++)
       for (int s = 0; s < S; s++) {
         HIPCHK(c, launch(s, SFTB_PH_LIN));
+        HIPCHK(c, launch(s, SFTB_PH_PLAN));
         HIPCHK(c, launch(s, SFTB_PH_FACTOR));
         HIPCHK(c, launch(s, SFTB_PH_TRIAL));
       }
-    if (tail_below >= 0) HIPCHK(c, launch(0, SFTB_PH_TAIL));
+    if (tail_below >= 0) {
+      if (carry != SFTB_CARRY_OFF) HIPCHK(c, launch(0, SFTB_PH_RESOLVE));
+      HIPCHK(c, launch(0, SFTB_PH_TAIL));
+    }
     for (int s = 0; s < S; s++) HIPCHK(c, hipMemcpyAsync(c->spec_done.p + 64 * s, c->d_counters + 16 * s, 8 * sizeof(int), hipMemcpyDeviceToHost, c->sub_stream[s]));
     for (int s = 0; s < S; s++) HIPCHK(c, hipStreamSynchronize(c->sub_stream[s]));
     int done = 0;
@@ -497,7 +506,7 @@
   {
     bool all_tiles = true;
     for (int b = 0; b < B; b++) all_tiles = all_tiles && c->packed[b].h.tile_mode == 1;
-    if (all_tiles && 2 * B > c->num_cus) nw = 4;
+    if (all_tiles && (2 * B > c->num_cus || c->opt.rounds == 2)) nw = 4;
     if ((c->opt.waves == 4 && all_tiles) || c->opt.waves == 8) nw = c->opt.waves;
     if (c->force_waves == 8) nw = 8;
     c->rounds_mode = all_tiles && nw == 4 && c->opt.waves == 0 && c->opt.rounds != 0 && !c->host_only;
@@ -600,7 +609,7 @@
   std::vector<WOffs> wo((size_t)B * K);
   const size_t ws_off = a.size;
   const size_t o_spec = a.take(sizeof(SftSpec) * (size_t)B * K);
-  const size_t o_runs = a.take(c->rounds_mode ? sizeof(SftRun) * (size_t)B + 64 * dsh_ctx::kMaxSub + sizeof(int) * (size_t)B : 0);
+  const size_t o_runs = a.take(c->rounds_mode ? sizeof(SftRun) * (size_t)B + 64 * dsh_ctx::kMaxSub + 3 * sizeof(int) * (size_t)B : 0);
   int nh = 0;
   {
     bool any = false;
@@ -1185,13 +1194,15 @@
   if (k == "waves") { if (value != 0 && value != 4 && value != 8) return dsh_fail(c, DSH_ERR_ARG, "dsh_lab_set_option: waves is 0 (automatic), 4 or 8"); c->opt.waves = value; }
   else if (k == "dataflow") c->opt.dataflow = value != 0;
   else if (k == "wide_off") c->opt.wide_off = value != 0;
-  else if (k == "rounds") c->opt.rounds = value != 0;
+  else if (k == "rounds") c->opt.rounds = value == 2 ? 2 : value != 0;
   else if (k == "streams") { if (value < 0 || value > dsh_ctx::kMaxSub) return dsh_fail(c, DSH_ERR_ARG, "dsh_lab_set_option: streams is 0 (automatic) or 1..4 sub-batches"); c->opt.streams = value; }
   else if (k == "split") { if (value < 0 || value > 2) return dsh_fail(c, DSH_ERR_ARG, "dsh_lab_set_option: split is 0 (off), 1 (wide bands only) or 2 (every band long enough)"); c->opt.split = value; }
   else if (k == "helpers_wbt") { if (value < 1 || value > 16) return dsh_fail(c, DSH_ERR_ARG, "dsh_lab_set_option: helpers_wbt is 1..16 (tiles of half-bandwidth from which parts get helper workgroups)"); c->opt.helpers_wbt = value; }
   else if (k == "owner_waves") { if (value != 8 && value != 16) return dsh_fail(c, DSH_ERR_ARG, "dsh_lab_set_option: owner_waves is 8 or 16 (wavefronts of a FACTOR workgroup with helpers)"); c->opt.owner_waves = value; }
   else if (k == "helpers") { if (value < -1 || value > 3) return dsh_fail(c, DSH_ERR_ARG, "dsh_lab_set_option: helpers is -1 (automatic) or 0..3 workgroups per part"); c->opt.helpers = value; }
   else if (k == "tail") { if (value < -1 || value > 8) return dsh_fail(c, DSH_ERR_ARG, "dsh_lab_set_option: tail is -1 (automatic), 0 (rounds to the end) or the number of problems per CU from which downwards the last problems go to the tail kernel"); c->opt.tail = value; }
+  else if (k == "carry") { if (value < -1 || value > 1) return dsh_fail(c, DSH_ERR_ARG, "dsh_lab_set_option: carry is 0 (off, the default), -1 (whole wave sets from two sets upwards, the last set left pending) or 1 (from one set and one problem upwards)"); c->opt.carry = value; }
+  else if (k == "factor_waves") { if (value < 0) return dsh_fail(c, DSH_ERR_ARG, "dsh_lab_set_option: factor_waves is 0 (one per SIMD) or a cap on the wavefronts of a FACTOR launch"); c->opt.factor_waves = value; }
   else if (k == "speculate") { if (value < 0 || value > SFT_SPEC_MAXK) return dsh_fail(c, DSH_ERR_ARG, "dsh_lab_set_option: speculate is 0 (automatic) or 1..4 lanes"); c->opt.speculate = value; }
   else return dsh_fail(c, DSH_ERR_ARG, "dsh_lab_set_option: unknown option " + k);
   return DSH_OK;
@@ -1278,8 +1289,9 @@
   for (int b = 0; b < c->B; b++)
     if (c->h_probs[b].tile_mode != 1) return dsh_fail(c, DSH_ERR_STATE, "dsh_lab_sft_factor_check: register-window problems (half-bandwidth <= 128) only");
   const int B = c->B;
-  struct OwnedDevBuf { void* p = nullptr; ~OwnedDevBuf() { if (p) (void)hipFree(p); } } runs, counters;
+  struct OwnedDevBuf { void* p = nullptr; ~OwnedDevBuf() { if (p) (void)hipFree(p); } } runs, counters, lists;
   HIPCHK(c, hipMalloc(&runs.p, sizeof(SftRun) * (size_t)B));
+  HIPCHK(c, hipMalloc(&lists.p, 2 * sizeof(int) * (size_t)B));
   HIPCHK(c, hipMalloc(&counters.p, 16 * sizeof(int)));
   std::vector<SftRun> h_runs(B);
   for (int b = 0; b < B; b++) {
@@ -1293,7 +1305,8 @@
   for (int b = 0; b < B; b++) HIPCHK(c, hipMemcpyAsync(c->h_probs[b].dbg + 1, &lambda[b], sizeof(double), hipMemcpyHostToDevice, c->stream));
   HIPCHK(c, hipMemcpyAsync(runs.p, h_runs.data(), sizeof(SftRun) * (size_t)B, hipMemcpyHostToDevice, c->stream));
   HIPCHK(c, hipMemsetAsync(counters.p, 0, 16 * sizeof(int), c->stream));
-  HIPCHK(c, sftb_factor_lab_launch(c->d_probs, (SftRun*)runs.p, (int*)counters.p, B, grid ? grid : std::min(B, 4 * c->num_cus), c->stream));
+  HIPCHK(c, hipMemsetAsync(lists.p, 0xff, 2 * sizeof(int) * (size_t)B, c->stream));
+  HIPCHK(c, sftb_factor_lab_launch(c->d_probs, (SftRun*)runs.p, (int*)counters.p, (int*)lists.p, B, grid ? grid : std::min(B, 4 * c->num_cus), c->stream));
   HIPCHK(c, hipStreamSynchronize(c->stream));
   HIPCHK(c, hipMemcpy(h_runs.data(), runs.p, sizeof(SftRun) * (size_t)B, hipMemcpyDeviceToHost));
   size_t off = 0;
@@ -1304,6 +1317,16 @@
     off += Dnp + 6;
     if (ok) ok[b] = h_runs[b].fact_ok;
   }
+  return DSH_OK;
+}
+
+int dsh_lab_sft_plan_host(const int32_t* states, int32_t B, int32_t W, int32_t carry, int32_t rot, int32_t* list, int32_t* out4) {
+  if (!states || !list || !out4 || B <= 0 || W <= 0 || rot < 0 || rot >= B || carry < -1 || carry > 1) return DSH_ERR_ARG;
+  int n = 0;
+  for (int p = 0; p < B; p++) { const int b = (rot + p) % B; if (states[b] == SFTB_TRIAL) list[n++] = b; }
+  int n_admit, n_dyn;
+  sftb_plan_budget(n, W, carry, &n_admit, &n_dyn);
+  out4[0] = n; out4[1] = n_admit; out4[2] = n_dyn; out4[3] = sftb_plan_rotate(rot, n_admit > 0 ? list[n_admit - 1] : -1, B);
   return DSH_OK;
 }
 
@@ -1317,14 +1340,14 @@
   const int rc = run_rounds(c);
   c->phase_events = nullptr;
   (void)hipStreamSynchronize(c->stream);
-  for (int i = 0; i < 7; i++) ms4[i] = 0.0;
+  for (int i = 0; i < 9; i++) ms4[i] = 0.0;
   { int32_t cnt[16] = {0}; if (hipMemcpy(cnt, c->d_counters, sizeof(cnt), hipMemcpyDeviceToHost) == hipSuccess) { ms4[5] = (double)cnt[8]; ms4[6] = (double)cnt[9]; } }
   int n_trial = 0;
   for (size_t i = 0; i + 1 < ev.size(); i += 2) {
     float ms = 0.f;
     (void)hipEventElapsedTime(&ms, ev[i], ev[i + 1]);
     const int ph = c->phase_ids[i / 2];
-    ms4[ph == SFTB_PH_INIT ? 0 : ph == SFTB_PH_LIN ? 1 : ph == SFTB_PH_FACTOR ? 2 : ph == SFTB_PH_TRIAL ? 3 : 4] += ms;
+    ms4[ph == SFTB_PH_INIT ? 0 : ph == SFTB_PH_LIN ? 1 : ph == SFTB_PH_FACTOR ? 2 : ph == SFTB_PH_TRIAL ? 3 : ph == SFTB_PH_PLAN ? 7 : ph == SFTB_PH_RESOLVE ? 8 : 4] += ms;
     n_trial += ph == SFTB_PH_TRIAL;
   }
   if (rounds) *rounds = n_trial;
diff --git a/defslam_amd/csrc/sft_batch.h b/defslam_amd/csrc/sft_batch.h
--- a/defslam_amd/csrc/sft_batch.h
+++ b/defslam_amd/csrc/sft_batch.h
@@ -18,8 +18,9 @@
   panel = out + 32;
 }
 
-__global__ __launch_bounds__(64 * SFTB_NW, 2) void sftb_init_kernel(const SftDev* __restrict__ probs, SftRun* __restrict__ runs, int* __restrict__ counters, int* __restrict__ lin_list, int tail_below) {
+__global__ __launch_bounds__(64 * SFTB_NW, 2) void sftb_init_kernel(const SftDev* __restrict__ probs, SftRun* __restrict__ runs, int* __restrict__ counters, int* __restrict__ lin_list, int* __restrict__ pend, int tail_below) {
   const SftDev& P = probs[blockIdx.x];
+  if (threadIdx.x == 0) pend[blockIdx.x] = -1;
   if (blockIdx.x == 0 && threadIdx.x == 0 && (int)gridDim.x <= tail_below) counters[6] = 1;
   init_state<64 * SFTB_NW>(P);
   if (threadIdx.x == 0) {
@@ -78,29 +79,76 @@
   }
 }
 
-__global__ __launch_bounds__(64, 1) void sftb_factor_kernel(const SftDev* __restrict__ probs, SftRun* __restrict__ runs, int* __restrict__ counters, int B) {
+#define SFTB_PLAN_NT 1024
+__global__ __launch_bounds__(SFTB_PLAN_NT, 1) void sftb_plan_kernel(const SftRun* __restrict__ runs, int* __restrict__ counters, int* __restrict__ fac_list, int B, int W, int carry) {
+  __shared__ int wave_sum[SFTB_PLAN_NT / 64];
+  if (counters[6]) return;
+  const int tid = threadIdx.x;
+  const int rot = counters[15];
+  const int C = (B + SFTB_PLAN_NT - 1) / SFTB_PLAN_NT;
+  const int p0 = min(B, tid * C), p1 = min(B, p0 + C);
+  int cnt = 0;
+  for (int p = p0; p < p1; p++) { int b = rot + p; if (b >= B) b -= B; cnt += runs[b].state == SFTB_TRIAL; }
+  int incl = cnt;
+  for (int d = 1; d < 64; d <<= 1) { const int o = __shfl_up(incl, d, 64); if ((tid & 63) >= d) incl += o; }
+  if ((tid & 63) == 63) wave_sum[tid >> 6] = incl;
+  __syncthreads();
+  int base = incl - cnt, n = 0;
+  for (int w = 0; w < SFTB_PLAN_NT / 64; w++) { const int v = wave_sum[w]; if (w < (tid >> 6)) base += v; n += v; }
+  for (int p = p0; p < p1; p++) { int b = rot + p; if (b >= B) b -= B; if (runs[b].state == SFTB_TRIAL) fac_list[base++] = b; }
+  __syncthreads();
+  if (tid == 0) {
+    int n_admit, n_dyn;
+    sftb_plan_budget(n, W, carry, &n_admit, &n_dyn);
+    counters[10] = n; counters[11] = n_admit; counters[12] = n_dyn;
+    counters[15] = sftb_plan_rotate(rot, n_admit > 0 ? fac_list[n_admit - 1] : -1, B);
+    counters[1] = 0; counters[2] = 0; counters[3] = 0;
+  }
+}
+
+__device__ __forceinline__ WvPrev sftb_prev_of_pending(const SftDev& P) {
+  int lane;
+  asm volatile("v_mbcnt_lo_u32_b32 %0, -1, 0\n\tv_mbcnt_hi_u32_b32 %0, -1, %0" : "=v"(lane));
+  const int c = lane & 15;
+  const int Dn = uni(P.Dn), Dnp = ((Dn + NB - 1) / NB) * NB;
+  const double xcam = c < 6 ? P.x[Dnp + c] : 0.0;
+  return wv_prev_of(P, 1, xcam, lane);
+}
+
+__global__ __launch_bounds__(64, 1) void sftb_factor_kernel(const SftDev* __restrict__ probs, SftRun* __restrict__ runs, int* __restrict__ counters,
+                                                            const int* __restrict__ fac_list, int* __restrict__ pend, int B, int resolve) {
   extern __shared__ __attribute__((aligned(16))) char smem[];
   lds_double* lds = to_lds(reinterpret_cast<double*>(smem));
   const int lane = threadIdx.x;
-  if (counters[6]) return;
-  for (int i = lane; i < WV_LDS_DOUBLES; i += 64) lds[i] = 0.0;
-  if (blockIdx.x == 0 && lane == 0) { counters[2] = 0; counters[3] = 0; }
+  const int tail_mode = counters[6] || (resolve >= 0 && B - counters[0] <= resolve);
+  if (resolve >= 0 && !tail_mode) return;
   WvPrev Q;
   Q.Lg = nullptr; Q.Linv = nullptr; Q.x = nullptr; Q.nT = 0; Q.active = 0; Q.xb = 0.0;
+  const int pb = __builtin_amdgcn_readfirstlane(pend[blockIdx.x]);
+  if (pb >= 0) {
+    Q = sftb_prev_of_pending(probs[pb]);
+    if (lane == 0) { runs[pb].state = SFTB_SOLVED; pend[blockIdx.x] = -1; }
+  }
   int n_done = 0;
-  while (true) {
-    int b = 0;
-    if (lane == 0) b = atomicAdd(&counters[1], 1);
-    b = __builtin_amdgcn_readfirstlane(b);
-    if (b >= B) break;
-    if (runs[b].state != SFTB_TRIAL) continue;
-    const SftDev& P = probs[b];
-    const double lambda = runs[b].lambda;
-    double xcam;
-    const int ok = wv_factor(P, lambda, lambda, lds, Q, xcam);
-    if (lane == 0) runs[b].fact_ok = ok;
-    Q = wv_prev_of(P, ok, xcam, lane);
-    n_done++;
+  if (!tail_mode) {
+    for (int i = lane; i < WV_LDS_DOUBLES; i += 64) lds[i] = 0.0;
+    while (true) {
+      int i = 0;
+      if (lane == 0) i = atomicAdd(&counters[1], 1);
+      i = __builtin_amdgcn_readfirstlane(i);
+      const int n_dyn = counters[12], last = i >= n_dyn;
+      if (last && n_dyn >= counters[11]) break;
+      const int b = __builtin_amdgcn_readfirstlane(fac_list[last ? n_dyn + (int)blockIdx.x : i]);
+      const SftDev& P = probs[b];
+      const double lambda = runs[b].lambda;
+      double xcam;
+      const int ok = wv_factor(P, lambda, lambda, lds, Q, xcam);
+      Q = wv_prev_of(P, ok, xcam, lane);
+      n_done++;
+      const int pending = last && ok;
+      if (lane == 0) { runs[b].fact_ok = ok; runs[b].state = pending ? SFTB_PENDING : SFTB_SOLVED; if (pending) pend[blockIdx.x] = b; }
+      if (last) { Q.active = 0; break; }
+    }
   }
   int lane_now;
   asm volatile("v_mbcnt_lo_u32_b32 %0, -1, 0\n\tv_mbcnt_hi_u32_b32 %0, -1, %0" : "=v"(lane_now));
@@ -206,8 +254,7 @@
   SftRun& R = runs[blockIdx.x];
   const int st = R.state;
   if (counters[6]) return;
-  if (blockIdx.x == 0 && threadIdx.x == 0) counters[1] = 0;
-  if (st != SFTB_TRIAL && st != SFTB_FINISH) return;
+  if (st != SFTB_SOLVED && st != SFTB_FINISH) return;
   extern __shared__ __attribute__((aligned(16))) char smem[];
   const SftDev& P = probs[blockIdx.x];
   Ctl* ctl; double *red, *out, *panel;
@@ -218,7 +265,8 @@
     if (tid == 0) { R.state = SFTB_DONE; atomicAdd(&counters[0], 1); }
     return;
   }
-  (void)sftb_trial_problem<NW>(P, R, ctl, red, out, panel, counters, lin_list, blockIdx.x);
+  const int r = sftb_trial_problem<NW>(P, R, ctl, red, out, panel, counters, lin_list, blockIdx.x);
+  if (r == 0 && tid == 0) R.state = SFTB_TRIAL;
 }
 
 __device__ __noinline__ void sftb_solve8(const SftDev& P, unsigned ctl_off, unsigned ws_off, double lambda) {
@@ -254,16 +302,18 @@
       if (tid == 0) { R.state = SFTB_DONE; atomicAdd(&counters[0], 1); }
       continue;
     }
-    while (st == SFTB_LIN || st == SFTB_TRIAL) {
+    while (st == SFTB_LIN || st == SFTB_TRIAL || st == SFTB_SOLVED) {
       if (st == SFTB_LIN) {
         sftb_lin_problem<NW>(P, R, ctl, red, out, panel);
         __syncthreads();
       }
-      if (tid == 0) ctl->lambda = R.lambda;
-      __syncthreads();
-      sftb_solve8(P, (unsigned)(size_t)(__attribute__((address_space(3))) char*)(char*)ctl, (unsigned)(size_t)(__attribute__((address_space(3))) char*)(char*)panel, R.lambda);
-      if (tid == 0) R.fact_ok = ctl->fact_ok;
-      __syncthreads();
+      if (st != SFTB_SOLVED) {
+        if (tid == 0) ctl->lambda = R.lambda;
+        __syncthreads();
+        sftb_solve8(P, (unsigned)(size_t)(__attribute__((address_space(3))) char*)(char*)ctl, (unsigned)(size_t)(__attribute__((address_space(3))) char*)(char*)panel, R.lambda);
+        if (tid == 0) R.fact_ok = ctl->fact_ok;
+        __syncthreads();
+      }
       const int r = sftb_trial_problem<NW>(P, R, ctl, red, out, panel, counters, nullptr, b);
       __syncthreads();
       st = r == 0 ? SFTB_TRIAL : (r == 1 ? SFTB_LIN : SFTB_DONE);
diff --git a/defslam_amd/csrc/sft_kernels.hip b/defslam_amd/csrc/sft_kernels.hip
--- a/defslam_amd/csrc/sft_kernels.hip
+++ b/defslam_amd/csrc/sft_kernels.hip
@@ -3099,12 +3099,15 @@
 }
 #endif
 
-extern "C" hipError_t sftb_launch(const SftDev* d_probs, SftRun* d_runs, int* d_counters, int* d_list, int B, int phase, size_t jl_doubles, size_t xyz_doubles, size_t* configured, int num_cus, int tail_below, hipStream_t stream) {
+extern "C" hipError_t sftb_launch(const SftDev* d_probs, SftRun* d_runs, int* d_counters, int* d_list, int B, int phase, size_t jl_doubles, size_t xyz_doubles, size_t* configured, int num_cus, int tail_below,
+                                  int factor_waves, int carry, hipStream_t stream) {
   const size_t head = 512 + (16 * 27 + 5 + 32) * sizeof(double) + 64;
+  int* d_fac = d_list + B;
+  int* d_pend = d_list + 2 * (size_t)B;
   if (phase == SFTB_PH_INIT) {
     hipError_t e = hipMemsetAsync(d_counters, 0, 16 * sizeof(int), stream);
     if (e != hipSuccess) return e;
-    hipLaunchKernelGGL(sftb_init_kernel, dim3(B), dim3(64 * SFTB_NW), 0, stream, d_probs, d_runs, d_counters, d_list, tail_below);
+    hipLaunchKernelGGL(sftb_init_kernel, dim3(B), dim3(64 * SFTB_NW), 0, stream, d_probs, d_runs, d_counters, d_list, d_pend, tail_below);
   } else if (phase == SFTB_PH_LIN) {
     const size_t lds = head + jl_doubles * sizeof(double);
     if (lds > configured[0]) {
@@ -3114,8 +3117,11 @@
     }
     const int per_cu = lds > 80 * 1024 ? 1 : 2;
     hipLaunchKernelGGL(sftb_lin_kernel, dim3(std::min(B, per_cu * num_cus)), dim3(64 * SFTB_LIN_NW), lds, stream, d_probs, d_runs, d_counters, d_list, B, tail_below);
-  } else if (phase == SFTB_PH_FACTOR) {
-    hipLaunchKernelGGL(sftb_factor_kernel, dim3(std::min(B, 4 * num_cus)), dim3(64), WV_LDS_DOUBLES * sizeof(double), stream, d_probs, d_runs, d_counters, B);
+  } else if (phase == SFTB_PH_PLAN) {
+    hipLaunchKernelGGL(sftb_plan_kernel, dim3(1), dim3(SFTB_PLAN_NT), 0, stream, d_runs, d_counters, d_fac, B, factor_waves, carry);
+  } else if (phase == SFTB_PH_FACTOR || phase == SFTB_PH_RESOLVE) {
+    hipLaunchKernelGGL(sftb_factor_kernel, dim3(factor_waves), dim3(64), WV_LDS_DOUBLES * sizeof(double), stream, d_probs, d_runs, d_counters, d_fac, d_pend, B,
+                       phase == SFTB_PH_RESOLVE ? std::max(0, tail_below) : -1);
   } else {
     const size_t lds = head + std::max<size_t>(2048, xyz_doubles) * sizeof(double);
     if (lds > configured[1]) {
@@ -3129,8 +3135,9 @@
 }
 
 #ifdef DSH_LAB
-extern "C" hipError_t sftb_factor_lab_launch(const SftDev* d_probs, SftRun* d_runs, int* d_counters, int B, int grid, hipStream_t stream) {
-  hipLaunchKernelGGL(sftb_factor_kernel, dim3(grid), dim3(64), WV_LDS_DOUBLES * sizeof(double), stream, d_probs, d_runs, d_counters, B);
+extern "C" hipError_t sftb_factor_lab_launch(const SftDev* d_probs, SftRun* d_runs, int* d_counters, int* d_list, int B, int grid, hipStream_t stream) {
+  hipLaunchKernelGGL(sftb_plan_kernel, dim3(1), dim3(SFTB_PLAN_NT), 0, stream, d_runs, d_counters, d_list, B, grid, SFTB_CARRY_OFF);
+  hipLaunchKernelGGL(sftb_factor_kernel, dim3(grid), dim3(64), WV_LDS_DOUBLES * sizeof(double), stream, d_probs, d_runs, d_counters, d_list, d_list + B, B, -1);
   return hipGetLastError();
 }
 #endif
diff --git a/defslam_amd/csrc/sft_problem.h b/defslam_amd/csrc/sft_problem.h
--- a/defslam_amd/csrc/sft_problem.h
+++ b/defslam_amd/csrc/sft_problem.h
@@ -64,11 +64,30 @@
 #define SFTB_TRIAL 1
 #define SFTB_DONE 2
 #define SFTB_FINISH 3
+#define SFTB_PENDING 4
+#define SFTB_SOLVED 5
 #define SFTB_PH_INIT 0
 #define SFTB_PH_LIN 1
 #define SFTB_PH_FACTOR 2
 #define SFTB_PH_TRIAL 3
 #define SFTB_PH_TAIL 4
+#define SFTB_PH_PLAN 5
+#define SFTB_PH_RESOLVE 6
+#define SFTB_CARRY_OFF 0
+#define SFTB_CARRY_AUTO -1
+#define SFTB_CARRY_ALWAYS 1
+#if defined(__HIPCC__) || defined(__CUDACC__)
+__host__ __device__
+#endif
+static inline void sftb_plan_budget(int n, int W, int carry, int* n_admit, int* n_dyn) {
+  *n_admit = n; *n_dyn = n;
+  if (carry == SFTB_CARRY_OFF || W <= 0) return;
+  if (n >= (carry == SFTB_CARRY_ALWAYS ? W + 1 : 2 * W)) { *n_admit = (n / W) * W; *n_dyn = *n_admit - W; }
+}
+#if defined(__HIPCC__) || defined(__CUDACC__)
+__host__ __device__
+#endif
+static inline int sftb_plan_rotate(int rot, int last_admitted, int B) { return last_admitted < 0 ? rot : (last_admitted + 1) % B; }
 struct SftRun {
   double lambda, ni, chi_cur, chi_ini, rho, lambda_start;
   double pose_bak[8];
@@ -162,7 +181,7 @@
 extern "C" size_t sft_lm_kernel_lds_bytes(int kd, size_t jl_doubles);
 extern "C" hipError_t sft_lm_launch(const SftDev* d_probs, int B, int max_kd, size_t jl_doubles, int nw, size_t* configured, hipStream_t stream);
 extern "C" hipError_t sftb_launch(const SftDev* d_probs, SftRun* d_runs, int* d_counters, int* d_list, int B, int phase, size_t jl_doubles, size_t xyz_doubles,
-                                  size_t* configured, int num_cus, int tail_below, hipStream_t stream);
+                                  size_t* configured, int num_cus, int tail_below, int factor_waves, int carry, hipStream_t stream);
 extern "C" hipError_t sftb_tail_launch(const SftDev* d_probs, SftRun* d_runs, int* d_counters, int B, int max_kd, size_t jl_doubles, size_t* configured, int num_cus,
                                        int tail_below, hipStream_t stream);
 extern "C" hipError_t sft_spec_launch(const SftDev* d_probs, SftSpec* d_spec, int B, int K, int phase, int nh, int owner_waves, int max_kd, size_t jl_doubles,
@@ -174,5 +193,5 @@
 #ifdef DSH_LAB
 extern "C" hipError_t sft_wave_lab_launch(const SftDev* d_probs, int B, int which, double rel, int max_kd, size_t jl_doubles, hipStream_t stream);
 extern "C" hipError_t sft_assembly_launch(const SftDev* d_probs, int B, int max_kd, size_t jl_doubles, int nw, hipStream_t stream);
-extern "C" hipError_t sftb_factor_lab_launch(const SftDev* d_probs, SftRun* d_runs, int* d_counters, int B, int grid, hipStream_t stream);
+extern "C" hipError_t sftb_factor_lab_launch(const SftDev* d_probs, SftRun* d_runs, int* d_counters, int* d_list, int B, int grid, hipStream_t stream);
 #endif
diff --git a/defslam_amd/sft.py b/defslam_amd/sft.py
--- a/defslam_amd/sft.py
+++ b/defslam_amd/sft.py
@@ -41,6 +41,7 @@
     status: int = 0
     trace: np.ndarray = field(default=None)
     regs: Optional[tuple] = None
+    max_iters: Optional[int] = None
 
 
 class Context:
@@ -150,7 +151,7 @@
             reg_lap, reg_inex, reg_temp = f.regs
         fc.reg_lap, fc.reg_inex, fc.reg_temp = float(reg_lap), float(reg_inex), float(reg_temp)
         fc.neighbour_layers = int(layers)
-        fc.max_iters = int(max_iters)
+        fc.max_iters = int(max_iters if f.max_iters is None else min(f.max_iters, max_iters))
         return fc
 
     def batch_upload(self, frames: Sequence[Frame], RegLap=5000.0, RegInex=5000.0, RegTemp=0.0, NeighboursLayers=1, max_iters=50):
@@ -237,12 +238,24 @@
         offs = np.concatenate([[0], np.cumsum(dims)])
         return [x[offs[b]:offs[b + 1]] for b in range(B)], ok
 
+    @staticmethod
+    def plan_host(states, W: int, carry: int, rot: int):
+        L = _lib.load_lab()
+        st = np.ascontiguousarray(states, np.int32)
+        lst = np.zeros(st.size, np.int32)
+        o = np.zeros(4, np.int32)
+        rc = L.dsh_lab_sft_plan_host(_ptr(st, C.c_int32), st.size, int(W), int(carry), int(rot), _ptr(lst, C.c_int32), _ptr(o, C.c_int32))
+        if rc != 0:
+            raise ValueError(f"dsh_lab_sft_plan_host: error {rc}")
+        return lst[:int(o[0])].copy(), int(o[1]), int(o[2]), int(o[3])
+
     def rounds_timed(self):
         self._need_lab("dsh_lab_sft_rounds_timed")
-        ms = np.zeros(7)
+        ms = np.zeros(9)
         r = np.zeros(1, np.int32)
         self._check(self._L.dsh_lab_sft_rounds_timed(self._h, _ptr(ms, C.c_double), _ptr(r, C.c_int32)), "dsh_lab_sft_rounds_timed")
-        return dict(init=float(ms[0]), lin=float(ms[1]), factor=float(ms[2]), trial=float(ms[3]), tail=float(ms[4]), factorisations_in_rounds=int(ms[5]), linearisations_in_rounds=int(ms[6])), int(r[0])
+        return dict(init=float(ms[0]), lin=float(ms[1]), plan=float(ms[7]), factor=float(ms[2]), trial=float(ms[3]), resolve=float(ms[8]), tail=float(ms[4]),
+                    factorisations_in_rounds=int(ms[5]), linearisations_in_rounds=int(ms[6])), int(r[0])
 
     def dump(self, b: int, what: int, n: int):
         self._need_lab("dsh_lab_sft_dump")
diff --git a/include/defslam_hip_debug.h b/include/defslam_hip_debug.h
--- a/include/defslam_hip_debug.h
+++ b/include/defslam_hip_debug.h
@@ -17,7 +17,8 @@
 int dsh_lab_sft_assemble_timed(dsh_ctx* ctx, int launches, double* total_ms);
 int dsh_lab_sft_wave_check(dsh_ctx* ctx, double rel, int launches, int only, double* x_ref, double* x_new, int32_t* ok2, double* ms2);
 int dsh_lab_sft_factor_check(dsh_ctx* ctx, const double* lambda, const uint8_t* factor, int grid, double* x, int32_t* ok);
-int dsh_lab_sft_rounds_timed(dsh_ctx* ctx, double* ms7, int32_t* rounds);
+int dsh_lab_sft_plan_host(const int32_t* states, int32_t B, int32_t W, int32_t carry, int32_t rot, int32_t* list, int32_t* out4);
+int dsh_lab_sft_rounds_timed(dsh_ctx* ctx, double* ms9, int32_t* rounds);
 int dsh_lab_sft_dump(dsh_ctx* ctx, int b, int what, int64_t n, double* out);
 int dsh_lab_sft_phase_ms(dsh_ctx* ctx, int b, double* out8);
 int dsh_lab_sft_step_trace(dsh_ctx* ctx, int b, double* out64);
```

Result: no change. 417,500 (-0.7%).
